# sotelo/parrot

Measured on AMD Instinct MI355X. Metric: acoustic feature frames/sec (train fwd+bwd+allreduce+clip/Adam), higher is better.
Workload: dtype f32; 1 GPU; BASELINE configs[1]: 2-layer attention-GRU decoder, h=1024, batch=64 per GPU, T_enc=200, T_dec=800, fp32; cell=gru, layers=2, hidden=1024, batch_per_gpu=64, global_batch=64, T_enc=200, T_dec=800, parallelism=dp1, params=13919212

## Files before the change

include/parrot_hip.h:

```cpp
#ifndef PARROT_HIP_H
#define PARROT_HIP_H

#include <stddef.h>
#include <stdint.h>

#ifdef __cplusplus
extern "C" {
#endif

#define PARROT_ERR_BADARG 10001
#define PARROT_ERR_UNSUPPORTED 10002

#define PARROT_NORM_EPS 1e-5f
#define PARROT_MAX_LAYERS 3

const char* parrot_hip_version(void);

int parrot_profile_begin(void);
long long parrot_profile_end(double* total_us, double* flops, double* bytes);
long long parrot_profile_end2(double* total_us, double* flops, double* bytes, double* plain4);

#define PARROT_PRECISION_F32 0
#define PARROT_PRECISION_BF16 1
#define PARROT_PRECISION_BF16X3 2
int parrot_set_gemm_precision(int mode);
int parrot_get_gemm_precision(void);
int parrot_gemm(const float* A, int lda, int transA, const float* B, int ldb, int transB, float* C, int ldc,
                int M, int N, int K, const float* bias, float alpha, int accumulate, int act, int nbatch,
                long long strideA, long long strideB, long long strideC, int split_k, void* stream);

int parrot_gemm_gated(const float* A, int lda, int transA, const float* B, int ldb, int transB, float* C, int ldc,
                      int M, int N, int K, const float* gate, int ldg, void* stream);

#define PARROT_GEMM_ROUTE_STEP 0
#define PARROT_GEMM_ROUTE_F32 1
#define PARROT_GEMM_ROUTE_BF16 2
#define PARROT_GEMM_ROUTE_BF16X3 3
int parrot_gemm_route(const float* A, int lda, int transA, const float* B, int ldb, int transB, int M, int N, int K,
                      float alpha, int act, int nbatch, long long strideA, long long strideB, int split_k, int has_gate,
                      int* kernel, int* slices);

int parrot_step_launch_mode(int njobs, const int* M, const int* N, const int* K, const int* lstm_H, int* info);

int parrot_to_bf16(const float* x, void* y, long long n, void* stream);
int parrot_gemm_bf16in(const void* A, int lda, const void* B, int ldb, float* C, int ldc, int M, int N, int K,
                       int accumulate, int split_k, void* stream);
int parrot_gemm_bf16in_ex(const void* A, int lda, int transA, const void* B, int ldb, int transB, float* C, int ldc, int M,
                          int N, int K, const float* bias, int accumulate, int split_k, void* stream);

int parrot_colsum(const float* x, long long M, int N, int ld, float* out, int accumulate, void* stream);
int parrot_colsum_route(const float* x, long long M, int N, int ld, const float* out, int* info2);

int parrot_gru_step_fwd(const float* h, const float* inputs, const float* gate_inputs, const float* mask,
                        const float* Wg, const float* Wc, float* h_out, float* z, float* r, float* rh,
                        float* c, int B, int H, void* stream);

int parrot_gru_step_bwd(const float* dh_out, const float* h, const float* mask, const float* Wg,
                        const float* Wc, const float* z, const float* r, const float* c, float* dh,
                        float* d_inputs, float* d_gate_inputs, int B, int H, void* stream);

typedef struct ParrotGruSeqDesc {
    int T, B, H, nchain, use_graph, reserved;
    int reverse[4];
    const float* Wg[4];
    const float* Wc[4];
    const float* inputs[4];
    const float* gate_inputs[4];
    const float* mask;
    float* h[4];
    float* z[4]; float* r[4]; float* rh[4]; float* c[4];
    float* dh[4];
    float* dG[4];
    float* dC[4];
} ParrotGruSeqDesc;

int parrot_gru_seq_create(const ParrotGruSeqDesc* desc, void** plan);
int parrot_gru_seq_fwd(void* plan, void* stream);
int parrot_gru_seq_bwd(void* plan, void* stream);
int parrot_gru_seq_destroy(void* plan);

#define PARROT_GRU_ROUTE_ROWWISE 0
#define PARROT_GRU_ROUTE_SHAPE 1
#define PARROT_GRU_ROUTE_SWITCH 2
#define PARROT_GRU_ROUTE_UNALIGNED 3
#define PARROT_GRU_ROUTE_ALLOC 4
int parrot_gru_seq_route(void* plan, int* info4);
int parrot_gru_seq_rowwise_supported(int T, int B, int H, int nchain);

typedef struct ParrotLstmSeqDesc {
    int T, B, H, use_graph;
    const float* W;
    const float* pre_in;
    float* s; float* c;
    float* gates;
    float* dS;
    float* dc;
    float* dP;
} ParrotLstmSeqDesc;

int parrot_lstm_seq_create(const ParrotLstmSeqDesc* desc, void** plan);
int parrot_lstm_seq_fwd(void* plan, void* stream);
int parrot_lstm_seq_bwd(void* plan, void* stream);
int parrot_lstm_seq_destroy(void* plan);

int parrot_gmm_attention_fwd(const float* h1, const float* WattT, const float* batt, const float* kappa_prev,
                             const float* ctx, float* a, float* b, float* kappa, float* phi, float* w, int B,
                             int H, int A, int U, int E, int att_type, float eps, float alignment,
                             float sharpening, float timing, void* stream);

int parrot_gmm_attention_bwd(const float* dw, const float* ctx, const float* a, const float* b,
                             const float* kappa, const float* kappa_prev, const float* WattT, float* dkappa,
                             float* dp, float* dh1, int B, int H, int A, int U, int E, int att_type, float eps,
                             void* stream);

typedef struct ParrotDecoderDesc {
    int T, B, H, E, A, U, L, att_type, use_graph;
    int reserved;
    float eps, alignment, sharpening, timing;
    const float* Wg[PARROT_MAX_LAYERS];
    const float* Wc[PARROT_MAX_LAYERS];
    const float* bg[PARROT_MAX_LAYERS];
    const float* bc[PARROT_MAX_LAYERS];
    const float* WattT;
    const float* batt;
    const float* ctx;
    float* seq_c[PARROT_MAX_LAYERS];
    float* seq_g[PARROT_MAX_LAYERS];
    float* h[PARROT_MAX_LAYERS];
    float* w;
    float* kappa;
    float* z[PARROT_MAX_LAYERS]; float* r[PARROT_MAX_LAYERS];
    float* rh[PARROT_MAX_LAYERS]; float* c[PARROT_MAX_LAYERS];
    float* a; float* b;
    float* phi;
    float* dh[PARROT_MAX_LAYERS];
    float* dw;
    float* dw0;
    float* dhup[PARROT_MAX_LAYERS];
    float* dkappa;
    float* dG[PARROT_MAX_LAYERS];
    float* dC[PARROT_MAX_LAYERS];
    float* dp;
    int cell;
    int seq_init;
    float* cst[PARROT_MAX_LAYERS];
    float* gate4[PARROT_MAX_LAYERS];
    float* dcell[PARROT_MAX_LAYERS];
    int layer_norm, bf16;
    const float* ln_bg[PARROT_MAX_LAYERS * PARROT_MAX_LAYERS];
    const float* ln_bc[PARROT_MAX_LAYERS * PARROT_MAX_LAYERS];
    float* ln_yg[PARROT_MAX_LAYERS * PARROT_MAX_LAYERS];
    float* ln_yc[PARROT_MAX_LAYERS * PARROT_MAX_LAYERS];
    float* ln_sg[PARROT_MAX_LAYERS * PARROT_MAX_LAYERS];
    float* ln_sc[PARROT_MAX_LAYERS * PARROT_MAX_LAYERS];
    const float* Wg_f[PARROT_MAX_LAYERS];
    const float* Wc_f[PARROT_MAX_LAYERS];
    const float* Wg_r[PARROT_MAX_LAYERS];
    const float* Wc_r[PARROT_MAX_LAYERS];
    int* att_sup;
    float* persist_ws;
    long long persist_ws_floats;
    float* dh_b[PARROT_MAX_LAYERS];
    float* dhup_b[PARROT_MAX_LAYERS];
    float* dw_b;
    float* dw0_b;
    float* dhup_c[PARROT_MAX_LAYERS];
    float* dw_c;
    float* dw0_c;
    void* dG16[PARROT_MAX_LAYERS];
} ParrotDecoderDesc;

long long parrot_decoder_persist_floats(const ParrotDecoderDesc* desc);
int parrot_decoder_is_persistent(void* plan);
int parrot_decoder_schedule(void* plan);
int parrot_decoder_backward_tick(void* plan);
long long parrot_decoder_trace(void* plan, int which, long long* out, long long cap);
long long parrot_decoder_trace_jobs(void* plan, int which, long long* out, long long cap);
int parrot_decoder_status(void* plan);

int parrot_decoder_create(const ParrotDecoderDesc* desc, void** plan);
int parrot_decoder_writes_bf16_grads(void* plan);
int parrot_decoder_seq_fwd(void* plan, void* stream);
int parrot_decoder_seq_bwd(void* plan, void* stream);
int parrot_decoder_destroy(void* plan);

#define PARROT_READOUT_MAX_SEG 4
typedef struct ParrotReadoutComposedDesc {
    long long M;
    long long ws_floats;
    int nseg, R, O, zero_rows;
    int slice_rows, nbias;
    int K[PARROT_READOUT_MAX_SEG];
    int ldx[PARROT_READOUT_MAX_SEG];
// ... 196 lines not shown
```

parrot_amd/_lib.py:

```python
from __future__ import annotations

import ctypes as C
import os

from .utils import env_str

_HERE = os.path.dirname(os.path.abspath(__file__))
LIB_PATH = os.path.join(_HERE, "libparrot_hip.so")

MAX_LAYERS = 3

c_float_p = C.c_void_p


class HipLibraryMissing(RuntimeError):
    pass


class HipCallError(RuntimeError):
    pass


class GruSeqDesc(C.Structure):
    _fields_ = [
        ("T", C.c_int), ("B", C.c_int), ("H", C.c_int), ("nchain", C.c_int),
        ("use_graph", C.c_int), ("reserved", C.c_int),
        ("reverse", C.c_int * 4),
        ("Wg", C.c_void_p * 4), ("Wc", C.c_void_p * 4),
        ("inputs", C.c_void_p * 4), ("gate_inputs", C.c_void_p * 4),
        ("mask", C.c_void_p),
        ("h", C.c_void_p * 4),
        ("z", C.c_void_p * 4), ("r", C.c_void_p * 4), ("rh", C.c_void_p * 4), ("c", C.c_void_p * 4),
        ("dh", C.c_void_p * 4), ("dG", C.c_void_p * 4), ("dC", C.c_void_p * 4),
    ]


class LabelTablesDesc(C.Structure):
    _fields_ = [
        ("N", C.c_longlong), ("Q", C.c_int), ("nseg", C.c_int),
        ("labels", C.c_void_p),
        ("tbl", C.c_void_p * 4), ("rows", C.c_void_p * 4), ("sums", C.c_void_p * 4),
        ("D", C.c_int * 4),
    ]


class LstmSeqDesc(C.Structure):
    _fields_ = [(n, C.c_int) for n in ("T", "B", "H", "use_graph")] + \
               [(n, C.c_void_p) for n in ("W", "pre_in", "s", "c", "gates", "dS", "dc", "dP")]


class DecoderDesc(C.Structure):
    _fields_ = [
        ("T", C.c_int), ("B", C.c_int), ("H", C.c_int), ("E", C.c_int), ("A", C.c_int),
        ("U", C.c_int), ("L", C.c_int), ("att_type", C.c_int), ("use_graph", C.c_int),
        ("reserved", C.c_int),
        ("eps", C.c_float), ("alignment", C.c_float), ("sharpening", C.c_float), ("timing", C.c_float),
        ("Wg", C.c_void_p * MAX_LAYERS), ("Wc", C.c_void_p * MAX_LAYERS),
        ("bg", C.c_void_p * MAX_LAYERS), ("bc", C.c_void_p * MAX_LAYERS),
        ("WattT", C.c_void_p), ("batt", C.c_void_p), ("ctx", C.c_void_p),
        ("seq_c", C.c_void_p * MAX_LAYERS), ("seq_g", C.c_void_p * MAX_LAYERS),
        ("h", C.c_void_p * MAX_LAYERS), ("w", C.c_void_p), ("kappa", C.c_void_p),
        ("z", C.c_void_p * MAX_LAYERS), ("r", C.c_void_p * MAX_LAYERS),
        ("rh", C.c_void_p * MAX_LAYERS), ("c", C.c_void_p * MAX_LAYERS),
        ("a", C.c_void_p), ("b", C.c_void_p), ("phi", C.c_void_p),
        ("dh", C.c_void_p * MAX_LAYERS), ("dw", C.c_void_p), ("dw0", C.c_void_p), ("dhup", C.c_void_p * MAX_LAYERS),
        ("dkappa", C.c_void_p),
        ("dG", C.c_void_p * MAX_LAYERS), ("dC", C.c_void_p * MAX_LAYERS), ("dp", C.c_void_p),
        ("cell", C.c_int), ("seq_init", C.c_int),
        ("cst", C.c_void_p * MAX_LAYERS), ("gate4", C.c_void_p * MAX_LAYERS), ("dcell", C.c_void_p * MAX_LAYERS),
        ("layer_norm", C.c_int), ("bf16", C.c_int),
        ("ln_bg", C.c_void_p * (MAX_LAYERS * MAX_LAYERS)), ("ln_bc", C.c_void_p * (MAX_LAYERS * MAX_LAYERS)),
        ("ln_yg", C.c_void_p * (MAX_LAYERS * MAX_LAYERS)), ("ln_yc", C.c_void_p * (MAX_LAYERS * MAX_LAYERS)),
        ("ln_sg", C.c_void_p * (MAX_LAYERS * MAX_LAYERS)), ("ln_sc", C.c_void_p * (MAX_LAYERS * MAX_LAYERS)),
        ("Wg_f", C.c_void_p * MAX_LAYERS), ("Wc_f", C.c_void_p * MAX_LAYERS),
        ("Wg_r", C.c_void_p * MAX_LAYERS), ("Wc_r", C.c_void_p * MAX_LAYERS),
        ("att_sup", C.c_void_p),
        ("persist_ws", C.c_void_p), ("persist_ws_floats", C.c_longlong),
        ("dh_b", C.c_void_p * MAX_LAYERS), ("dhup_b", C.c_void_p * MAX_LAYERS), ("dw_b", C.c_void_p), ("dw0_b", C.c_void_p),
        ("dhup_c", C.c_void_p * MAX_LAYERS), ("dw_c", C.c_void_p), ("dw0_c", C.c_void_p),
        ("dG16", C.c_void_p * MAX_LAYERS),
    ]


READOUT_MAX_SEG = 4


class ReadoutComposedDesc(C.Structure):
    _fields_ = [
        ("M", C.c_longlong), ("ws_floats", C.c_longlong),
        ("nseg", C.c_int), ("R", C.c_int), ("O", C.c_int), ("zero_rows", C.c_int),
        ("slice_rows", C.c_int), ("nbias", C.c_int),
        ("K", C.c_int * READOUT_MAX_SEG), ("ldx", C.c_int * READOUT_MAX_SEG), ("lddx", C.c_int * READOUT_MAX_SEG),
        ("ldwr", C.c_int), ("ldwo", C.c_int), ("ldp", C.c_int), ("lddp", C.c_int),
        ("ldgwr", C.c_int), ("ldgwo", C.c_int),
        ("x", C.c_void_p * READOUT_MAX_SEG),
        ("Wr", C.c_void_p), ("Wo", C.c_void_p),
        ("rb", C.c_void_p * READOUT_MAX_SEG), ("bo", C.c_void_p),
        ("pred", C.c_void_p), ("dp", C.c_void_p),
        ("dx", C.c_void_p * READOUT_MAX_SEG),
        ("gWr", C.c_void_p), ("gWo", C.c_void_p),
        ("grb", C.c_void_p * READOUT_MAX_SEG), ("gbo", C.c_void_p),
    ]


class SampleDesc(C.Structure):
    _fields_ = [
        ("S", C.c_int), ("B", C.c_int), ("H", C.c_int), ("E", C.c_int), ("A", C.c_int),
        ("U", C.c_int), ("L", C.c_int), ("O", C.c_int), ("R", C.c_int), ("ldx", C.c_int),
        ("att_type", C.c_int), ("use_graph", C.c_int),
        ("eps", C.c_float), ("alignment", C.c_float), ("sharpening", C.c_float), ("timing", C.c_float),
        ("Wg", C.c_void_p * MAX_LAYERS), ("Wc", C.c_void_p * MAX_LAYERS),
        ("bg", C.c_void_p * MAX_LAYERS), ("bc", C.c_void_p * MAX_LAYERS),
        ("Wfg", C.c_void_p * MAX_LAYERS), ("Wfc", C.c_void_p * MAX_LAYERS),
        ("seq_c", C.c_void_p * MAX_LAYERS), ("seq_g", C.c_void_p * MAX_LAYERS),
        ("WattT", C.c_void_p), ("batt", C.c_void_p),
        ("Wr", C.c_void_p), ("br", C.c_void_p), ("radd", C.c_void_p),
        ("Wo", C.c_void_p), ("bo", C.c_void_p), ("oadd", C.c_void_p),
        ("ctx", C.c_void_p),
        ("x", C.c_void_p), ("h", C.c_void_p * MAX_LAYERS), ("w", C.c_void_p), ("kappa", C.c_void_p),
        ("a", C.c_void_p), ("bwork", C.c_void_p), ("phi", C.c_void_p),
        ("zwork", C.c_void_p), ("rwork", C.c_void_p), ("rhwork", C.c_void_p), ("readout", C.c_void_p),
        ("gmm_K", C.c_int), ("reserved2", C.c_int), ("sampling_bias", C.c_float), ("reserved3", C.c_float),
        ("Wmu", C.c_void_p), ("bmu", C.c_void_p), ("Wsig", C.c_void_p), ("bsig", C.c_void_p),
        ("Wco", C.c_void_p), ("bco", C.c_void_p),
        ("add_mu", C.c_void_p), ("add_sig", C.c_void_p), ("add_co", C.c_void_p),
        ("unif", C.c_void_p), ("noise", C.c_void_p),
        ("gmm_mu", C.c_void_p), ("gmm_sig", C.c_void_p), ("gmm_co", C.c_void_p), ("pi_out", C.c_void_p),
        ("cell", C.c_int), ("reserved5", C.c_int),
        ("cwork", C.c_void_p * MAX_LAYERS), ("gwork", C.c_void_p),
        ("layer_norm", C.c_int), ("reserved7", C.c_int),
        ("bfg", C.c_void_p * MAX_LAYERS), ("bfc", C.c_void_p * MAX_LAYERS),
        ("ln_bg", C.c_void_p * (MAX_LAYERS * MAX_LAYERS)), ("ln_bc", C.c_void_p * (MAX_LAYERS * MAX_LAYERS)),
        ("br_l", C.c_void_p * MAX_LAYERS),
        ("ln_scratch", C.c_void_p), ("ln_scratch_floats", C.c_longlong),
        ("Wg_t", C.c_void_p * MAX_LAYERS), ("Wc_t", C.c_void_p * MAX_LAYERS),
        ("Wr_t", C.c_void_p), ("Wo_t", C.c_void_p), ("bo_pad", C.c_void_p), ("oadd_pad", C.c_void_p),
        ("persist_ws", C.c_void_p), ("persist_ws_floats", C.c_longlong),
        ("Wro_t", C.c_void_p), ("ro_const", C.c_void_p),
        ("Wgx_t", C.c_void_p * MAX_LAYERS), ("Wcx_t", C.c_void_p * MAX_LAYERS),
        ("Watt_t", C.c_void_p),
        ("bf16", C.c_int), ("reserved8", C.c_int),
        ("Wg_t16", C.c_void_p * MAX_LAYERS),
        ("eou_pos", C.c_void_p), ("eou_ncmp", C.c_void_p), ("eou_first", C.c_void_p),
        ("eou_extra", C.c_int), ("reserved9", C.c_int),
        ("Wrh_t", C.c_void_p), ("rh_const", C.c_void_p), ("rh_cols", C.c_int), ("reserved10", C.c_int),
    ]


class SampleRnnGenDesc(C.Structure):
    _fields_ = ([(n, C.c_int) for n in ("B", "D", "T", "Q", "FS", "BFS", "feat_dim", "use_graph")] +
                [("temperature", C.c_float), ("reserved", C.c_int), ("seed", C.c_ulonglong)] +
                [(n, C.c_void_p) for n in (
                    "big_Win_frames", "big_Win_feats", "big_bin", "big_U", "big_bU", "big_Wg", "big_Wc",
                    "big_Wout", "big_bout", "frm_Win", "frm_bin", "frm_U", "frm_bU", "frm_Wg", "frm_Wc",
                    "frm_Wout", "frm_bout", "emb_tbl", "W2", "b2", "W3", "b3", "W4", "b4", "features",
                    "samples", "big_h", "frm_h", "xf_big", "xf_frm", "feat_cur", "gru_in", "P", "z", "r", "rh",
                    "big_out", "frame_out", "o1", "o2", "o3", "logits", "tbase")] +
                [("n_rnn", C.c_int), ("lstm", C.c_int),
                 ("big_L", (C.c_void_p * 4) * 5), ("frm_L", (C.c_void_p * 4) * 5),
                 ("big_hs", C.c_void_p * 5), ("big_cs", C.c_void_p * 5),
                 ("frm_hs", C.c_void_p * 5), ("frm_cs", C.c_void_p * 5),
                 ("gate_ws", C.c_void_p), ("layer_tmp", C.c_void_p),
                 ("persist_ws", C.c_void_p), ("persist_ws_floats", C.c_longlong)])


_vp, _i, _f, _ll, _sz = C.c_void_p, C.c_int, C.c_float, C.c_longlong, C.c_size_t
SIGNATURES = {
    "parrot_hip_version": (C.c_char_p, []),
    "parrot_profile_begin": (_i, []),
    "parrot_profile_end": (C.c_longlong, [C.POINTER(C.c_double)] * 3),
    "parrot_profile_end2": (C.c_longlong, [C.POINTER(C.c_double)] * 4),
    "parrot_gemm": (_i, [_vp, _i, _i, _vp, _i, _i, _vp, _i, _i, _i, _i, _vp, _f, _i, _i, _i, _ll, _ll, _ll, _i, _vp]),
    "parrot_gemm_gated": (_i, [_vp, _i, _i, _vp, _i, _i, _vp, _i, _i, _i, _i, _vp, _i, _vp]),
    "parrot_gemm_route": (_i, [_vp, _i, _i, _vp, _i, _i, _i, _i, _i, _f, _i, _i, _ll, _ll, _i, _i,
                               C.POINTER(C.c_int), C.POINTER(C.c_int)]),
    "parrot_step_launch_mode": (_i, [_i] + [C.POINTER(C.c_int)] * 5),
    "parrot_gather_sum_fwd": (_i, [_vp, _vp, _vp, _i, _vp, _i, _ll, _i, _i, _i, _vp]),
    "parrot_gather_sum_bwd_ws_floats": (C.c_longlong, [_ll, _i, _i, _i]),
    "parrot_gather_sum_bwd": (_i, [_vp, _i, _vp, _vp, _vp, _vp, _ll, _ll, _i, _i, _i, _i, _vp]),
    "parrot_softmax_ce_fwd": (_i, [_vp, _i, _vp, _ll, _i, _vp, _vp, _vp]),
    "parrot_softmax_ce_bwd": (_i, [_vp, _i, _vp, _vp, _vp, _ll, _i, _vp, _i, _vp]),
    "parrot_relu_gate": (_i, [_vp, _vp, _vp, _ll, _vp]),
    "parrot_gmm_cost_fwd": (_i, [_vp, _i] * 4 + [_ll, _i, _i, _f, _vp, _vp, _i, _vp, _vp]),
    "parrot_gmm_cost_bwd": (_i, [_vp, _i] * 4 + [_vp, _vp, _ll, _i, _i, _f] + [_vp, _i] * 3 + [_vp]),
    "samplernn_weightnorm_ws_floats": (_ll, [_i]),
    "samplernn_weightnorm_fold": (_i, [_vp, _i, _vp, _vp, _i, _vp, _vp, _i, _i, _vp]),
    "samplernn_weightnorm_fold_bwd": (_i, [_vp, _i, _vp, _vp, _vp, _i, _vp, _i, _vp, _vp, _i, _i, _i, _i, _vp]),
    "parrot_colsum": (_i, [_vp, _ll, _i, _i, _vp, _i, _vp]),
    "parrot_colsum_route": (_i, [_vp, _ll, _i, _i, _vp, C.POINTER(C.c_int)]),
    "parrot_gru_step_fwd": (_i, [_vp] * 11 + [_i, _i, _vp]),
    "parrot_gru_step_bwd": (_i, [_vp] * 11 + [_i, _i, _vp]),
    "parrot_label_tables_supported": (_i, [_ll, _i]),
    "parrot_label_gather": (_i, [C.POINTER(LabelTablesDesc), _vp]),
    "parrot_label_segsum_ws_floats": (C.c_longlong, [_ll, _i, _i]),
    "parrot_label_segsum": (_i, [C.POINTER(LabelTablesDesc), _vp, _ll, _vp]),
    "parrot_gru_seq_create": (_i, [C.POINTER(GruSeqDesc), C.POINTER(C.c_void_p)]),
    "parrot_gru_seq_fwd": (_i, [_vp, _vp]),
    "parrot_gru_seq_bwd": (_i, [_vp, _vp]),
    "parrot_gru_seq_destroy": (_i, [_vp]),
    "parrot_gru_seq_route": (_i, [_vp, C.POINTER(C.c_int)]),
    "parrot_gru_seq_rowwise_supported": (_i, [_i, _i, _i, _i]),
    "parrot_lstm_seq_create": (_i, [C.POINTER(LstmSeqDesc), C.POINTER(C.c_void_p)]),
    "parrot_lstm_seq_fwd": (_i, [_vp, _vp]),
    "parrot_lstm_seq_bwd": (_i, [_vp, _vp]),
    "parrot_lstm_seq_destroy": (_i, [_vp]),
    "parrot_gmm_attention_fwd": (_i, [_vp] * 10 + [_i] * 6 + [_f] * 4 + [_vp]),
    "parrot_gmm_attention_bwd": (_i, [_vp] * 10 + [_i] * 6 + [_f, _vp]),
    "parrot_decoder_create": (_i, [C.POINTER(DecoderDesc), C.POINTER(C.c_void_p)]),
    "parrot_decoder_persist_floats": (C.c_longlong, [C.POINTER(DecoderDesc)]),
    "parrot_decoder_is_persistent": (_i, [_vp]),
    "parrot_decoder_schedule": (_i, [_vp]),
    "parrot_decoder_backward_tick": (_i, [_vp]),
    "parrot_decoder_writes_bf16_grads": (_i, [_vp]),
    "parrot_decoder_trace": (C.c_longlong, [_vp, _i, C.POINTER(C.c_longlong), C.c_longlong]),
    "parrot_decoder_trace_jobs": (C.c_longlong, [_vp, _i, C.POINTER(C.c_longlong), C.c_longlong]),
    "parrot_decoder_seq_fwd": (_i, [_vp, _vp]),
    "parrot_decoder_seq_bwd": (_i, [_vp, _vp]),
    "parrot_decoder_destroy": (_i, [_vp]),
    "parrot_readout_composed_ws_floats": (C.c_longlong, [C.POINTER(ReadoutComposedDesc)]),
    "parrot_readout_composed_fwd": (_i, [C.POINTER(ReadoutComposedDesc), _vp, _vp]),
    "parrot_readout_composed_bwd": (_i, [C.POINTER(ReadoutComposedDesc), _vp, _vp]),
    "parrot_sample_create": (_i, [C.POINTER(SampleDesc), C.POINTER(C.c_void_p)]),
    "parrot_sample_persist_floats": (C.c_longlong, [C.POINTER(SampleDesc)]),
    "parrot_sample_is_persistent": (_i, [_vp]),
    "parrot_sample_is_bf16": (_i, [_vp]),
    "parrot_sample_plan_pieces_dry": (_i, [C.POINTER(SampleDesc), _i, C.POINTER(C.c_int)]),
    "parrot_sample_plan_digest_dry": (_i, [C.POINTER(SampleDesc), _i, C.POINTER(C.c_ulonglong)]),
    "parrot_sample_status": (_i, [_vp]),
    "parrot_sample_stops_early": (_i, [_vp]),
    "parrot_sample_steps_run": (_i, [_vp, C.POINTER(C.c_int)]),
    "parrot_decoder_status": (_i, [_vp]),
    "parrot_sample_run": (_i, [_vp, _vp]),
    "parrot_sample_destroy": (_i, [_vp]),
    "parrot_plan_last_error": (_i, [_vp]),
    "parrot_sumsq": (_i, [_vp, _sz, _vp, _vp]),
    "parrot_tile_weights": (_i, [_vp, _i, _i, _i, _vp, _i, _i, _vp]),
    "parrot_tile_weights_bf16": (_i, [_vp, _i, _i, _i, _vp, _i, _i, _vp]),
    "parrot_set_gemm_precision": (_i, [_i]),
    "parrot_get_gemm_precision": (_i, []),
    "parrot_to_bf16": (_i, [_vp, _vp, _ll, _vp]),
    "parrot_gemm_bf16in": (_i, [_vp, _i, _vp, _i, _vp, _i, _i, _i, _i, _i, _i, _vp]),
    "parrot_gemm_bf16in_ex": (_i, [_vp, _i, _i, _vp, _i, _i, _vp, _i, _i, _i, _i, _vp, _i, _i, _vp]),
    "parrot_simple_norm_fwd": (_i, [_vp, _i, _vp, _i, _vp, _ll, _i, _f, _vp, _i, _vp]),
    "parrot_simple_norm_bwd": (_i, [_vp, _i, _vp, _i, _vp, _vp, _i, _ll, _i, _f, _i, _vp]),
    "parrot_adam_clip_step": (_i, [_vp, _vp, _vp, _vp, _sz, _vp, _f, _f, _f, _f, _f, _f, _i, _vp]),
    "parrot_batch_quantize": (_i, [_vp, _i, _i, _i, _vp, _vp, _i, _i, _i, _vp]),
    "parrot_mu2linear": (_i, [_vp, _sz, _vp, _vp]),
    "samplernn_generate_create": (_i, [C.POINTER(SampleRnnGenDesc), C.POINTER(C.c_void_p)]),
    "samplernn_generate_run": (_i, [_vp, _vp]),
    "samplernn_persist_floats": (C.c_longlong, [C.POINTER(SampleRnnGenDesc)]),
    "samplernn_generate_is_persistent": (_i, [_vp]),
    "samplernn_generate_status": (_i, [_vp]),
    "samplernn_generate_destroy": (_i, [_vp]),
}

_lib = None


def load():
    global _lib
    if _lib is not None:
        return _lib
    import torch
    path = env_str('PARROT_HIP_LIB', LIB_PATH)
    if not os.path.exists(path):
        raise HipLibraryMissing(
            f"{LIB_PATH} not found: build it with `python -m parrot_amd.build` "
            "(hipcc --offload-arch=gfx950).  There is no CPU fallback for the product path.")
    lib = C.CDLL(path)
    for name, (res, args) in SIGNATURES.items():
        fn = getattr(lib, name)
        fn.restype = res
        fn.argtypes = args
    _lib = lib
    return lib


def check(rc: int, what: str, plan=None):
    if rc != 0:
        raise HipCallError(f"{what} failed with code {rc}")


def call(name: str, *args):
    lib = load()
    rc = getattr(lib, name)(*args)
    check(rc, name)
    return rc
```

parrot_amd/csrc/biggemm.h:

```cpp
#pragma once
#include "common.h"

struct BgArgs {
    const float* A;
    const float* B;
    float* C;
    const float* bias;
    int M, N, K;
    long long sam, sak, sbk, sbn;
    int ldc;
    long long batchA, batchB, batchC;
    int nbatch;
    int splitk;
    float* ws;
    int accumulate;
    float alpha;
    int act;
    const float* gate;
    int ldg;
    int bf16;
};

int bg_launch(const BgArgs& a, hipStream_t stream);
void bg_tile_shape(int bf16, int& bm, int& bn);
int bg_to_bf16_launch(const float* x, void* y, long long n, hipStream_t stream);
int bg_reduce_launch(const BgArgs& a, hipStream_t stream);

struct BgPrecisionScope {
    explicit BgPrecisionScope(int bf16);
    ~BgPrecisionScope();
    int saved;
};
```

parrot_amd/csrc/biggemm.hip:

```cpp
#include "biggemm.h"

#include <atomic>

#include <hip/hip_runtime.h>
#include <stdlib.h>
#include <string.h>

namespace {

constexpr int BM = 128, BN = 128, BK = 16, PITCH = 132;

__device__ __forceinline__ void bg_tile_of_block(int bid, int tiles_m, int tiles_n, int& tm, int& tn) {
    const int nwg = tiles_m * tiles_n;
    const int q = nwg / 8, r = nwg % 8;
    const int xcd = bid % 8, idx = bid / 8;
    const int lin = (xcd < r ? xcd * (q + 1) : r * (q + 1) + (xcd - r) * q) + idx;
    constexpr int GW = 8;
    const int group = lin / (GW * tiles_m);
    const int first = group * GW;
    const int gsz = min(tiles_n - first, GW);
    const int rem = lin - group * GW * tiles_m;
    tm = rem / gsz;
    tn = first + rem % gsz;
}

template <bool XC>
__device__ __forceinline__ void bg_load8(const float* __restrict__ p, int x0, int X, int k0, int kend,
                                         long long sx, long long sk, bool vec, int t, f32x4& v) {
    v = (f32x4){0.f, 0.f, 0.f, 0.f};
    if (XC) {
        const int xq = t & 31, kr = t >> 5;
        const int k = k0 + kr, x = x0 + 4 * xq;
        if (k < kend) {
            const float* q = p + (long long)k * sk + x;
            if (vec && x + 3 < X) v = *reinterpret_cast<const f32x4*>(q);
            else {
#pragma unroll
                for (int u = 0; u < 4; ++u)
                    if (x + u < X) v[u] = q[u];
            }
        }
    } else {
        const int x = x0 + (t >> 2), k = k0 + 4 * (t & 3);
        if (x < X) {
            const float* q = p + (long long)x * sx + k;
            if (vec && k + 3 < kend) v = *reinterpret_cast<const f32x4*>(q);
            else {
#pragma unroll
                for (int u = 0; u < 4; ++u)
                    if (k + u < kend) v[u] = q[u];
            }
        }
    }
}

template <bool XC>
__device__ __forceinline__ void bg_store8(float* __restrict__ s, int t, const f32x4& v) {
    if (XC) {
        *reinterpret_cast<f32x4*>(s + (t >> 5) * PITCH + 4 * (t & 31)) = v;
    } else {
        const int x = t >> 2, kq = t & 3;
#pragma unroll
        for (int u = 0; u < 4; ++u) s[(4 * kq + u) * PITCH + x] = v[u];
    }
}

template <bool AXC, bool BXC>
__global__ __launch_bounds__(512) void bg_kernel8(const BgArgs a, int vecA, int vecB, int tiles_m, int tiles_n) {
    __shared__ __attribute__((aligned(16))) float As[2][BK * PITCH];
    __shared__ __attribute__((aligned(16))) float Bs[2][BK * PITCH];
    int tm, tn;
    bg_tile_of_block(blockIdx.x, tiles_m, tiles_n, tm, tn);
    const int m0 = tm * BM, n0 = tn * BN;
    const int z = blockIdx.y;
    const int batch = z / a.splitk, ks = z % a.splitk;
    int kchunk = (a.K + a.splitk - 1) / a.splitk;
    kchunk = (kchunk + BK - 1) / BK * BK;
    const int kbeg = ks * kchunk;
    const int kend = min(a.K, kbeg + kchunk);
    const float* A = a.A + (long long)batch * a.batchA;
    const float* B = a.B + (long long)batch * a.batchB;
    float* C = a.C + (long long)batch * a.batchC;
    const int t = threadIdx.x, lane = t & 63, wave = t >> 6;
    const int wm = wave >> 2, wn = wave & 3;
    const int kk = lane >> 5, li = lane & 31;
    f32x16 acc[2];
#pragma unroll
    for (int i = 0; i < 2; ++i)
#pragma unroll
        for (int q = 0; q < 16; ++q) acc[i][q] = 0.f;
    f32x4 ra, rb;
    const int nk = (kend - kbeg + BK - 1) / BK;
    if (nk > 0) {
        bg_load8<AXC>(A, m0, a.M, kbeg, kend, a.sam, a.sak, vecA, t, ra);
        bg_load8<BXC>(B, n0, a.N, kbeg, kend, a.sbn, a.sbk, vecB, t, rb);
        bg_store8<AXC>(As[0], t, ra);
        bg_store8<BXC>(Bs[0], t, rb);
    }
    __syncthreads();
    for (int kt = 0; kt < nk; ++kt) {
        const int cur = kt & 1;
        if (kt + 1 < nk) {
            bg_load8<AXC>(A, m0, a.M, kbeg + (kt + 1) * BK, kend, a.sam, a.sak, vecA, t, ra);
            bg_load8<BXC>(B, n0, a.N, kbeg + (kt + 1) * BK, kend, a.sbn, a.sbk, vecB, t, rb);
        }
        const float* as = As[cur] + wm * 64 + li;
        const float* bs = Bs[cur] + wn * 32 + li;
#pragma unroll
        for (int kp = 0; kp < BK / 2; ++kp) {
            const int row = (2 * kp + kk) * PITCH;
            const float a0 = as[row], a1 = as[row + 32];
            const float b0 = bs[row];
            acc[0] = __builtin_amdgcn_mfma_f32_32x32x2f32(a0, b0, acc[0], 0, 0, 0);
            acc[1] = __builtin_amdgcn_mfma_f32_32x32x2f32(a1, b0, acc[1], 0, 0, 0);
        }
        if (kt + 1 < nk) {
            bg_store8<AXC>(As[cur ^ 1], t, ra);
            bg_store8<BXC>(Bs[cur ^ 1], t, rb);
        }
        __syncthreads();
    }
#pragma unroll
    for (int i = 0; i < 2; ++i) {
        const int n = n0 + wn * 32 + li;
        if (n >= a.N) continue;
        const float bias = (a.bias && ks == 0) ? a.bias[n] : 0.f;
#pragma unroll
        for (int q = 0; q < 16; ++q) {
            const int m = m0 + wm * 64 + i * 32 + (q & 3) + 8 * (q >> 2) + 4 * kk;
            if (m >= a.M) continue;
            float v = a.alpha * acc[i][q] + bias;
            float* c = C + (long long)m * a.ldc + n;
            if (a.splitk > 1) {
                a.ws[((long long)z * a.M + m) * a.N + n] = a.alpha * acc[i][q];
            } else {
                if (a.accumulate) v += *c;
                if (a.act == 1) v = fmaxf(v, 0.f);
                else if (a.act == 2) v = tanhf(v);
                else if (a.act == 3) v = 1.f / (1.f + expf(-v));
                if (a.gate && !(a.gate[(long long)m * a.ldg + n] > 0.f)) v = 0.f;
                *c = v;
            }
        }
    }
}


constexpr int BK16 = 32, PITCH16 = 40, PITCHT = 144;

template <bool XC>
__device__ __forceinline__ void bg_load16(const float* __restrict__ p, int x0, int X, int k0, int kend,
                                          long long sx, long long sk, bool vec, int t, f32x4 (&v)[2]) {
    v[0] = (f32x4){0.f, 0.f, 0.f, 0.f};
    v[1] = (f32x4){0.f, 0.f, 0.f, 0.f};
    if (XC) {
        const int x = x0 + 4 * (t & 31);
#pragma unroll
        for (int ps = 0; ps < 2; ++ps) {
            const int k = k0 + (t >> 5) + 16 * ps;
            if (k < kend) {
                const float* q = p + (long long)k * sk + x;
                if (vec && x + 3 < X) {
                    v[ps] = *reinterpret_cast<const f32x4*>(q);
                } else {
#pragma unroll
                    for (int u = 0; u < 4; ++u)
                        if (x + u < X) v[ps][u] = q[u];
                }
            }
        }
    } else {
        const int x = x0 + (t >> 2), k = k0 + 8 * (t & 3);
        if (x < X) {
            const float* q = p + (long long)x * sx + k;
            if (vec && k + 7 < kend) {
                v[0] = *reinterpret_cast<const f32x4*>(q);
                v[1] = *reinterpret_cast<const f32x4*>(q + 4);
            } else {
#pragma unroll
                for (int u = 0; u < 8; ++u)
                    if (k + u < kend) v[u >> 2][u & 3] = q[u];
            }
        }
    }
}

template <bool XC>
__device__ __forceinline__ void bg_store16(__bf16* __restrict__ s, int t, const f32x4 (&v)[2]) {
    if (XC) {
        typedef __bf16 bf16x4 __attribute__((ext_vector_type(4)));
#pragma unroll
        for (int ps = 0; ps < 2; ++ps)
            *reinterpret_cast<bf16x4*>(s + ((t >> 5) + 16 * ps) * PITCHT + 4 * (t & 31)) = __builtin_convertvector(v[ps], bf16x4);
    } else {
        *reinterpret_cast<bf16x8*>(s + (t >> 2) * PITCH16 + 8 * (t & 3)) = ph_bf16x8(v[0], v[1]);
    }
}

template <bool XC>
__device__ __forceinline__ bf16x8 bg_frag16(const __bf16* __restrict__ img, int xb, int s, int lane) {
    const int kk = lane >> 5, li = lane & 31;
    if (XC) {
        typedef short s16x4 __attribute__((ext_vector_type(4)));
        typedef __attribute__((address_space(3))) s16x4* lds4;
        const int k0 = 16 * s + 8 * kk, q = (li >> 2) & 3, xg = xb + (li & 16) + 4 * (li & 3);
        const __bf16* p = img + (k0 + q) * PITCHT + xg;
        const s16x4 lo = __builtin_amdgcn_ds_read_tr16_b64_v4i16((lds4)(p));
        const s16x4 hi = __builtin_amdgcn_ds_read_tr16_b64_v4i16((lds4)(p + 4 * PITCHT));
        typedef short s16x8 __attribute__((ext_vector_type(8)));
        const s16x8 v = {lo[0], lo[1], lo[2], lo[3], hi[0], hi[1], hi[2], hi[3]};
        return __builtin_bit_cast(bf16x8, v);
    } else {
        return *reinterpret_cast<const bf16x8*>(img + (xb + li) * PITCH16 + 16 * s + 8 * kk);
    }
}

template <bool AXC, bool BXC>
__global__ __launch_bounds__(512) void bg_kernel_bf16(const BgArgs a, int vecA, int vecB, int tiles_m, int tiles_n) {
    constexpr int ASZ = AXC ? BK16 * PITCHT : BM * PITCH16, BSZ = BXC ? BK16 * PITCHT : BN * PITCH16;
    __shared__ __attribute__((aligned(16))) __bf16 As[2][ASZ];
    __shared__ __attribute__((aligned(16))) __bf16 Bs[2][BSZ];
    int tm, tn;
    bg_tile_of_block(blockIdx.x, tiles_m, tiles_n, tm, tn);
    const int m0 = tm * BM, n0 = tn * BN;
    const int z = blockIdx.y;
    const int batch = z / a.splitk, ks = z % a.splitk;
    int kchunk = (a.K + a.splitk - 1) / a.splitk;
    kchunk = (kchunk + BK16 - 1) / BK16 * BK16;
    const int kbeg = ks * kchunk;
    const int kend = min(a.K, kbeg + kchunk);
    const float* A = a.A + (long long)batch * a.batchA;
    const float* B = a.B + (long long)batch * a.batchB;
    float* C = a.C + (long long)batch * a.batchC;
    const int t = threadIdx.x, lane = t & 63, wave = t >> 6;
    const int wm = wave >> 2, wn = wave & 3;
    const int kk = lane >> 5, li = lane & 31;
    f32x16 acc[2];
#pragma unroll
    for (int i = 0; i < 2; ++i)
#pragma unroll
        for (int q = 0; q < 16; ++q) acc[i][q] = 0.f;
    f32x4 ra[2], rb[2];
    const int nk = (kend - kbeg + BK16 - 1) / BK16;
    if (nk > 0) {
        bg_load16<AXC>(A, m0, a.M, kbeg, kend, a.sam, a.sak, vecA, t, ra);
        bg_load16<BXC>(B, n0, a.N, kbeg, kend, a.sbn, a.sbk, vecB, t, rb);
        bg_store16<AXC>(As[0], t, ra);
        bg_store16<BXC>(Bs[0], t, rb);
    }
    __syncthreads();
    for (int kt = 0; kt < nk; ++kt) {
        const int cur = kt & 1;
        if (kt + 1 < nk) {
            bg_load16<AXC>(A, m0, a.M, kbeg + (kt + 1) * BK16, kend, a.sam, a.sak, vecA, t, ra);
            bg_load16<BXC>(B, n0, a.N, kbeg + (kt + 1) * BK16, kend, a.sbn, a.sbk, vecB, t, rb);
        }
#pragma unroll
        for (int s = 0; s < BK16 / 16; ++s) {
            const bf16x8 a0 = bg_frag16<AXC>(As[cur], wm * 64, s, lane);
            const bf16x8 a1 = bg_frag16<AXC>(As[cur], wm * 64 + 32, s, lane);
            const bf16x8 b0 = bg_frag16<BXC>(Bs[cur], wn * 32, s, lane);
            acc[0] = __builtin_amdgcn_mfma_f32_32x32x16_bf16(a0, b0, acc[0], 0, 0, 0);
            acc[1] = __builtin_amdgcn_mfma_f32_32x32x16_bf16(a1, b0, acc[1], 0, 0, 0);
        }
        if (kt + 1 < nk) {
            bg_store16<AXC>(As[cur ^ 1], t, ra);
            bg_store16<BXC>(Bs[cur ^ 1], t, rb);
        }
        __syncthreads();
    }
#pragma unroll
    for (int i = 0; i < 2; ++i) {
        const int n = n0 + wn * 32 + li;
        if (n >= a.N) continue;
        const float bias = (a.bias && ks == 0) ? a.bias[n] : 0.f;
#pragma unroll
        for (int q = 0; q < 16; ++q) {
            const int m = m0 + wm * 64 + i * 32 + (q & 3) + 8 * (q >> 2) + 4 * kk;
            if (m >= a.M) continue;
            float v = a.alpha * acc[i][q] + bias;
            float* c = C + (long long)m * a.ldc + n;
            if (a.splitk > 1) {
                a.ws[((long long)z * a.M + m) * a.N + n] = a.alpha * acc[i][q];
            } else {
                if (a.accumulate) v += *c;
                if (a.act == 1) v = fmaxf(v, 0.f);
                else if (a.act == 2) v = tanhf(v);
                else if (a.act == 3) v = 1.f / (1.f + expf(-v));
                if (a.gate && !(a.gate[(long long)m * a.ldg + n] > 0.f)) v = 0.f;
                *c = v;
            }
        }
    }
}

constexpr int HBMT = 256, HBNT = 256, HPITCH = 272;
template <int BKT, bool XC>
struct BghOperand {
    static constexpr int PK = BKT + 8;
    static constexpr int SZ = XC ? BKT * HPITCH : 256 * PK;
    static constexpr int NV = BKT / 16;
    static __device__ __forceinline__ void load(const __bf16* __restrict__ p, long long ld, int x0, int X, int k0, int kend,
                                                int t, bf16x8 (&v)[NV]) {
#pragma unroll
        for (int i = 0; i < NV; ++i) {
            bf16x8 r;
#pragma unroll
            for (int u = 0; u < 8; ++u) r[u] = (__bf16)0.f;
            if (XC) {
                const int k = k0 + (t >> 5) + 16 * i, x = x0 + 8 * (t & 31);
                if (k < kend && x < X) r = *reinterpret_cast<const bf16x8*>(p + (long long)k * ld + x);
            } else {
                const int id = t + 512 * i;
                const int x = x0 + id / (BKT / 8), k = k0 + 8 * (id % (BKT / 8));
                if (x < X && k < kend) r = *reinterpret_cast<const bf16x8*>(p + (long long)x * ld + k);
            }
            v[i] = r;
        }
    }
    static __device__ __forceinline__ void store(__bf16* __restrict__ s, int t, const bf16x8 (&v)[NV]) {
#pragma unroll
        for (int i = 0; i < NV; ++i) {
            if (XC) {
                *reinterpret_cast<bf16x8*>(s + ((t >> 5) + 16 * i) * HPITCH + 8 * (t & 31)) = v[i];
            } else {
                const int id = t + 512 * i;
                *reinterpret_cast<bf16x8*>(s + (id / (BKT / 8)) * PK + 8 * (id % (BKT / 8))) = v[i];
            }
        }
    }
    static __device__ __forceinline__ bf16x8 frag(const __bf16* __restrict__ img, int xb, int s_, int kk, int li) {
        if (XC) {
            typedef short s16x4 __attribute__((ext_vector_type(4)));
            typedef short s16x8 __attribute__((ext_vector_type(8)));
            typedef __attribute__((address_space(3))) s16x4* lds4;
            const int k0 = 16 * s_ + 8 * kk, q = (li >> 2) & 3, xg = xb + (li & 16) + 4 * (li & 3);
            const __bf16* p = img + (k0 + q) * HPITCH + xg;
            const s16x4 lo = __builtin_amdgcn_ds_read_tr16_b64_v4i16((lds4)(p));
            const s16x4 hi = __builtin_amdgcn_ds_read_tr16_b64_v4i16((lds4)(p + 4 * HPITCH));
            const s16x8 v = {lo[0], lo[1], lo[2], lo[3], hi[0], hi[1], hi[2], hi[3]};
            return __builtin_bit_cast(bf16x8, v);
        } else {
            return *reinterpret_cast<const bf16x8*>(img + (xb + li) * PK + 16 * s_ + 8 * kk);
        }
    }
};

template <int BKT, bool AXC, bool BXC>
__global__ __launch_bounds__(512) void bgh_kernel(const BgArgs a, int tiles_m, int tiles_n) {
    typedef BghOperand<BKT, AXC> OA;
    typedef BghOperand<BKT, BXC> OB;
    constexpr int NV = BKT / 16;
    extern __shared__ __attribute__((aligned(16))) __bf16 bgh_smem[];
    __bf16* As = bgh_smem;
    __bf16* Bs = bgh_smem + 2 * OA::SZ;
    int tm, tn;
    bg_tile_of_block(blockIdx.x, tiles_m, tiles_n, tm, tn);
    const int m0 = tm * HBMT, n0 = tn * HBNT;
    const int z = blockIdx.y;
    const int batch = z / a.splitk, ks = z % a.splitk;
    int kchunk = (a.K + a.splitk - 1) / a.splitk;
    kchunk = (kchunk + BKT - 1) / BKT * BKT;
    const int kbeg = ks * kchunk;
    const int kend = min(a.K, kbeg + kchunk);
    const __bf16* A = reinterpret_cast<const __bf16*>(a.A) + (long long)batch * a.batchA;
    const __bf16* B = reinterpret_cast<const __bf16*>(a.B) + (long long)batch * a.batchB;
    float* C = a.C + (long long)batch * a.batchC;
    const long long lda = AXC ? a.sak : a.sam, ldb = BXC ? a.sbk : a.sbn;
    const int t = threadIdx.x, lane = t & 63, wave = t >> 6;
    const int wm = wave >> 2, wn = wave & 3;
    const int kk = lane >> 5, li = lane & 31;
    f32x16 acc[4][2];
#pragma unroll
    for (int i = 0; i < 4; ++i)
#pragma unroll
        for (int j = 0; j < 2; ++j)
#pragma unroll
            for (int q = 0; q < 16; ++q) acc[i][j][q] = 0.f;
    bf16x8 ra[NV], rb[NV];
    const int nk = (kend - kbeg + BKT - 1) / BKT;
    if (nk > 0) {
        OA::load(A, lda, m0, a.M, kbeg, kend, t, ra);
        OB::load(B, ldb, n0, a.N, kbeg, kend, t, rb);
        OA::store(As, t, ra);
        OB::store(Bs, t, rb);
    }
    __syncthreads();
    for (int kt = 0; kt < nk; ++kt) {
        const int cur = kt & 1;
        if (kt + 1 < nk) {
            OA::load(A, lda, m0, a.M, kbeg + (kt + 1) * BKT, kend, t, ra);
            OB::load(B, ldb, n0, a.N, kbeg + (kt + 1) * BKT, kend, t, rb);
        }
        const __bf16* as = As + cur * OA::SZ;
        const __bf16* bs = Bs + cur * OB::SZ;
#pragma unroll
        for (int s_ = 0; s_ < BKT / 16; ++s_) {
            bf16x8 fa[4], fb[2];
#pragma unroll
            for (int j = 0; j < 2; ++j) fb[j] = OB::frag(bs, wn * 64 + 32 * j, s_, kk, li);
#pragma unroll
            for (int i = 0; i < 4; ++i) fa[i] = OA::frag(as, wm * 128 + 32 * i, s_, kk, li);
#pragma unroll
            for (int i = 0; i < 4; ++i)
#pragma unroll
                for (int j = 0; j < 2; ++j)
                    acc[i][j] = __builtin_amdgcn_mfma_f32_32x32x16_bf16(fa[i], fb[j], acc[i][j], 0, 0, 0);
        }
        if (kt + 1 < nk) {
            OA::store(As + (cur ^ 1) * OA::SZ, t, ra);
            OB::store(Bs + (cur ^ 1) * OB::SZ, t, rb);
        }
        __syncthreads();
    }
#pragma unroll
    for (int i = 0; i < 4; ++i)
#pragma unroll
        for (int j = 0; j < 2; ++j) {
            const int n = n0 + wn * 64 + j * 32 + li;
            if (n >= a.N) continue;
            const float bias = (a.bias && ks == 0) ? a.bias[n] : 0.f;
#pragma unroll
            for (int q = 0; q < 16; ++q) {
                const int m = m0 + wm * 128 + i * 32 + (q & 3) + 8 * (q >> 2) + 4 * kk;
                if (m >= a.M) continue;
                const float v = a.alpha * acc[i][j][q];
                if (a.splitk > 1) {
                    a.ws[((long long)z * a.M + m) * a.N + n] = v;
                } else {
                    float* c = C + (long long)m * a.ldc + n;
                    *c = a.accumulate ? *c + v + bias : v + bias;
                }
            }
        }
}

constexpr int SBK = 16;
typedef __bf16 bf16x4 __attribute__((ext_vector_type(4)));

__device__ __forceinline__ void bgs_split(const f32x4& v, bf16x4& p0, bf16x4& p1, bf16x4& p2) {
    p0 = __builtin_convertvector(v, bf16x4);
    const f32x4 r1 = v - __builtin_convertvector(p0, f32x4);
    p1 = __builtin_convertvector(r1, bf16x4);
    const f32x4 r2 = r1 - __builtin_convertvector(p1, f32x4);
    p2 = __builtin_convertvector(r2, bf16x4);
}

template <bool XC>
struct BgsOperand {
    static constexpr int PK = SBK + 8;
    static constexpr int PLANE = XC ? SBK * HPITCH : 256 * PK;
    static constexpr int SZ = 3 * PLANE;
    static __device__ __forceinline__ void load(const float* __restrict__ p, long long ld, int x0, int X, int k0, int kend,
                                                bool vec, int t, f32x4 (&v)[2]) {
#pragma unroll
        for (int i = 0; i < 2; ++i) {
            const int id = t + 512 * i;
            v[i] = (f32x4){0.f, 0.f, 0.f, 0.f};
            if (XC) {
                const int k = k0 + (id >> 6), x = x0 + 4 * (id & 63);
                if (k < kend && x < X) {
                    const float* q = p + (long long)k * ld + x;
                    if (vec && x + 3 < X) v[i] = *reinterpret_cast<const f32x4*>(q);
                    else {
#pragma unroll
                        for (int u = 0; u < 4; ++u)
                            if (x + u < X) v[i][u] = q[u];
                    }
                }
            } else {
                const int x = x0 + (id >> 2), k = k0 + 4 * (id & 3);
                if (x < X && k < kend) {
                    const float* q = p + (long long)x * ld + k;
                    if (vec && k + 3 < kend) v[i] = *reinterpret_cast<const f32x4*>(q);
                    else {
#pragma unroll
                        for (int u = 0; u < 4; ++u)
                            if (k + u < kend) v[i][u] = q[u];
                    }
                }
            }
        }
    }
    static __device__ __forceinline__ void store(__bf16* __restrict__ s, int t, const f32x4 (&v)[2]) {
#pragma unroll
        for (int i = 0; i < 2; ++i) {
            const int id = t + 512 * i;
            bf16x4 p0, p1, p2;
            bgs_split(v[i], p0, p1, p2);
            __bf16* d = XC ? s + (id >> 6) * HPITCH + 4 * (id & 63) : s + (id >> 2) * PK + 4 * (id & 3);
            *reinterpret_cast<bf16x4*>(d) = p0;
            *reinterpret_cast<bf16x4*>(d + PLANE) = p1;
            *reinterpret_cast<bf16x4*>(d + 2 * PLANE) = p2;
        }
    }
    static __device__ __forceinline__ bf16x8 frag(const __bf16* __restrict__ img, int xb, int kk, int li) {
        if (XC) {
            typedef short s16x4 __attribute__((ext_vector_type(4)));
            typedef short s16x8 __attribute__((ext_vector_type(8)));
            typedef __attribute__((address_space(3))) s16x4* lds4;
            const int q = (li >> 2) & 3, xg = xb + (li & 16) + 4 * (li & 3);
            const __bf16* p = img + (8 * kk + q) * HPITCH + xg;
            const s16x4 lo = __builtin_amdgcn_ds_read_tr16_b64_v4i16((lds4)(p));
            const s16x4 hi = __builtin_amdgcn_ds_read_tr16_b64_v4i16((lds4)(p + 4 * HPITCH));
            const s16x8 v = {lo[0], lo[1], lo[2], lo[3], hi[0], hi[1], hi[2], hi[3]};
            return __builtin_bit_cast(bf16x8, v);
        } else {
            return *reinterpret_cast<const bf16x8*>(img + (xb + li) * PK + 8 * kk);
        }
    }
};

template <bool AXC, bool BXC>
__global__ __launch_bounds__(512) void bgs_kernel(const BgArgs a, int vecA, int vecB, int tiles_m, int tiles_n, int zmap) {
    typedef BgsOperand<AXC> OA;
    typedef BgsOperand<BXC> OB;
    extern __shared__ __attribute__((aligned(16))) __bf16 bgs_smem[];
    __bf16* As = bgs_smem;
    __bf16* Bs = bgs_smem + 2 * OA::SZ;
    int tm, tn, z;
    if (zmap) {
        const int tiles = tiles_m * tiles_n, idx = blockIdx.x >> 3;
        z = 8 * (idx / tiles) + (blockIdx.x & 7);
        const int tl = idx % tiles;
        tm = tl / tiles_n;
        tn = tl % tiles_n;
    } else {
        bg_tile_of_block(blockIdx.x, tiles_m, tiles_n, tm, tn);
        z = blockIdx.y;
    }
    const int m0 = tm * HBMT, n0 = tn * HBNT;
    const int batch = z / a.splitk, ks = z % a.splitk;
    int kchunk = (a.K + a.splitk - 1) / a.splitk;
    kchunk = (kchunk + SBK - 1) / SBK * SBK;
    const int kbeg = ks * kchunk;
    const int kend = min(a.K, kbeg + kchunk);
    const float* A = a.A + (long long)batch * a.batchA;
    const float* B = a.B + (long long)batch * a.batchB;
    float* C = a.C + (long long)batch * a.batchC;
    const long long lda = AXC ? a.sak : a.sam, ldb = BXC ? a.sbk : a.sbn;
    const int t = threadIdx.x, lane = t & 63, wave = t >> 6;
    const int wm = wave >> 2, wn = wave & 3;
    const int kk = lane >> 5, li = lane & 31;
    f32x16 acc[4][2];
#pragma unroll
    for (int i = 0; i < 4; ++i)
#pragma unroll
        for (int j = 0; j < 2; ++j)
#pragma unroll
            for (int q = 0; q < 16; ++q) acc[i][j][q] = 0.f;
    f32x4 ra[2], rb[2];
    const int nk = (kend - kbeg + SBK - 1) / SBK;
    if (nk > 0) {
        OA::load(A, lda, m0, a.M, kbeg, kend, vecA, t, ra);
        OB::load(B, ldb, n0, a.N, kbeg, kend, vecB, t, rb);
        OA::store(As, t, ra);
        OB::store(Bs, t, rb);
        if (nk > 1) {
            OA::load(A, lda, m0, a.M, kbeg + SBK, kend, vecA, t, ra);
            OB::load(B, ldb, n0, a.N, kbeg + SBK, kend, vecB, t, rb);
        }
    }
    __syncthreads();
    const bool early = wave >= 4;
    for (int kt = 0; kt < nk; ++kt) {
        const int cur = kt & 1;
        const __bf16* as = As + cur * OA::SZ;
        const __bf16* bs = Bs + cur * OB::SZ;
        if (early && kt + 1 < nk) {
            OA::store(As + (cur ^ 1) * OA::SZ, t, ra);
            OB::store(Bs + (cur ^ 1) * OB::SZ, t, rb);
            if (kt + 2 < nk) {
                OA::load(A, lda, m0, a.M, kbeg + (kt + 2) * SBK, kend, vecA, t, ra);
                OB::load(B, ldb, n0, a.N, kbeg + (kt + 2) * SBK, kend, vecB, t, rb);
            }
        }
        bf16x8 fb[2][3];
#pragma unroll
        for (int j = 0; j < 2; ++j)
#pragma unroll
            for (int p = 0; p < 3; ++p) fb[j][p] = OB::frag(bs + p * OB::PLANE, wn * 64 + 32 * j, kk, li);
#pragma unroll
        for (int i = 0; i < 4; ++i) {
            bf16x8 fa[3];
#pragma unroll
            for (int p = 0; p < 3; ++p) fa[p] = OA::frag(as + p * OA::PLANE, wm * 128 + 32 * i, kk, li);
#define BGS_MM(pa, pb)                                                                                    \
    acc[i][0] = __builtin_amdgcn_mfma_f32_32x32x16_bf16(fa[pa], fb[0][pb], acc[i][0], 0, 0, 0);          \
    acc[i][1] = __builtin_amdgcn_mfma_f32_32x32x16_bf16(fa[pa], fb[1][pb], acc[i][1], 0, 0, 0)
            BGS_MM(2, 0);
            BGS_MM(0, 2);
            BGS_MM(1, 1);
            BGS_MM(1, 0);
            BGS_MM(0, 1);
            BGS_MM(0, 0);
#undef BGS_MM
        }
        if (!early && kt + 1 < nk) {
            OA::store(As + (cur ^ 1) * OA::SZ, t, ra);
            OB::store(Bs + (cur ^ 1) * OB::SZ, t, rb);
            if (kt + 2 < nk) {
                OA::load(A, lda, m0, a.M, kbeg + (kt + 2) * SBK, kend, vecA, t, ra);
                OB::load(B, ldb, n0, a.N, kbeg + (kt + 2) * SBK, kend, vecB, t, rb);
            }
        }
        __syncthreads();
    }
#pragma unroll
    for (int i = 0; i < 4; ++i)
#pragma unroll
        for (int j = 0; j < 2; ++j) {
            const int n = n0 + wn * 64 + j * 32 + li;
            if (n >= a.N) continue;
            const float bias = (a.bias && ks == 0) ? a.bias[n] : 0.f;
#pragma unroll
            for (int q = 0; q < 16; ++q) {
                const int m = m0 + wm * 128 + i * 32 + (q & 3) + 8 * (q >> 2) + 4 * kk;
                if (m >= a.M) continue;
                const float v = a.alpha * acc[i][j][q];
                if (a.splitk > 1) {
                    a.ws[((long long)z * a.M + m) * a.N + n] = v;
                } else {
                    float* c = C + (long long)m * a.ldc + n;
                    float r = a.accumulate ? *c + v + bias : v + bias;
                    if (a.act == 1) r = fmaxf(r, 0.f);
                    if (a.gate && !(a.gate[(long long)m * a.ldg + n] > 0.f)) r = 0.f;
                    *c = r;
                }
            }
        }
}

__global__ __launch_bounds__(256) void bg_to_bf16_kernel(const float* __restrict__ x, __bf16* __restrict__ y, long long n8) {
    for (long long i = (long long)blockIdx.x * 256 + threadIdx.x; i < n8; i += (long long)gridDim.x * 256) {
        const f32x4 lo = *reinterpret_cast<const f32x4*>(x + 8 * i);
        const f32x4 hi = *reinterpret_cast<const f32x4*>(x + 8 * i + 4);
        *reinterpret_cast<bf16x8*>(y + 8 * i) = ph_bf16x8(lo, hi);
    }
}

__global__ __launch_bounds__(256) void bg_reduce_kernel(const BgArgs a) {
    const long long mn = (long long)a.M * a.N;
    const long long total = mn * a.nbatch;
    for (long long i = (long long)blockIdx.x * 256 + threadIdx.x; i < total; i += (long long)gridDim.x * 256) {
        const int batch = (int)(i / mn);
        const long long r = i % mn;
        const int m = (int)(r / a.N), n = (int)(r % a.N);
        float* c = a.C + (long long)batch * a.batchC + (long long)m * a.ldc + n;
        float v = a.accumulate ? *c : 0.f;
        if (a.bias) v += a.bias[n];
        const float* w = a.ws + ((long long)batch * a.splitk) * mn + r;
        int ks = 0;
        for (; ks + 8 <= a.splitk; ks += 8) {
            float p[8];
#pragma unroll
            for (int q = 0; q < 8; ++q) p[q] = w[(long long)(ks + q) * mn];
#pragma unroll
            for (int q = 0; q < 8; ++q) v += p[q];
        }
        for (; ks < a.splitk; ++ks) v += w[(long long)ks * mn];
        if (a.gate && !(a.gate[(long long)m * a.ldg + n] > 0.f)) v = 0.f;
        *c = v;
    }
}

}

int bg_reduce_launch(const BgArgs& a, hipStream_t stream) {
    const long long total = (long long)a.M * a.N * a.nbatch;
    int blocks = (int)((total + 255) / 256);
    if (blocks > 4096) blocks = 4096;
    hipLaunchKernelGGL(bg_reduce_kernel, dim3(blocks), dim3(256), 0, stream, a);
    return (int)hipGetLastError();
}

void bg_tile_shape(int bf16, int& bm, int& bn) {
    bm = bn = 128;
    if (bf16 == 2 || bf16 == 3) { bm = HBMT; bn = HBNT; return; }
}

template <typename K>
static void bg_big_lds_once(K kern, bool& done) {
    if (!done) {
        (void)hipFuncSetAttribute((const void*)kern, hipFuncAttributeMaxDynamicSharedMemorySize, 160 * 1024);
        done = true;
    }
}

template <int BKT, bool AX, bool BX>
static void bgh_go(const BgArgs& a, dim3 grid, int tm, int tn, hipStream_t stream) {
    static bool done = false;
    bg_big_lds_once(bgh_kernel<BKT, AX, BX>, done);
    const size_t lds = (size_t)4 * (BghOperand<BKT, AX>::SZ + BghOperand<BKT, BX>::SZ);
    hipLaunchKernelGGL((bgh_kernel<BKT, AX, BX>), grid, dim3(512), lds, stream, a, tm, tn);
}

template <bool AX, bool BX>
static void bgs_go(const BgArgs& a, dim3 grid, int vecA, int vecB, int tm, int tn, int zmap, hipStream_t stream) {
    static bool done = false;
    bg_big_lds_once(bgs_kernel<AX, BX>, done);
    const size_t lds = (size_t)4 * (BgsOperand<AX>::SZ + BgsOperand<BX>::SZ);
    hipLaunchKernelGGL((bgs_kernel<AX, BX>), grid, dim3(512), lds, stream, a, vecA, vecB, tm, tn, zmap);
}

int bg_to_bf16_launch(const float* x, void* y, long long n, hipStream_t stream) {
    if (n <= 0) return 0;
    if ((n & 7) || ((uintptr_t)x & 15) || ((uintptr_t)y & 15)) return PH_ERR_BADARG;
    const long long n8 = n / 8;
    int blocks = (int)((n8 + 255) / 256);
    if (blocks > 8192) blocks = 8192;
    hipLaunchKernelGGL(bg_to_bf16_kernel, dim3(blocks), dim3(256), 0, stream, x, reinterpret_cast<__bf16*>(y), n8);
    return (int)hipGetLastError();
}

int bg_launch(const BgArgs& a, hipStream_t stream) {
    const size_t pad = 0;
    if (a.M <= 0 || a.N <= 0 || a.K < 0 || a.nbatch < 1 || a.splitk < 1 || (a.splitk > 1 && !a.ws)) return PH_ERR_BADARG;
    const bool axc = (a.sam == 1), bxc = (a.sbn == 1);
    if (!axc && a.sak != 1) return PH_ERR_BADARG;
    if (!bxc && a.sbk != 1) return PH_ERR_BADARG;
    auto al = [](const float* p, long long stride, long long batch) {
        return (((uintptr_t)p & 15) == 0) && (stride % 4 == 0) && (batch % 4 == 0);
    };
    const int vecA = axc ? al(a.A, a.sak, a.batchA) : al(a.A, a.sam, a.batchA);
    const int vecB = bxc ? al(a.B, a.sbk, a.batchB) : al(a.B, a.sbn, a.batchB);
    const int tiles_m = ceil_div(a.M, BM), tiles_n = ceil_div(a.N, BN);
    dim3 grid(tiles_m * tiles_n, a.nbatch * a.splitk);
    if (a.bf16 == 2) {
        if (a.act || a.gate || ((uintptr_t)a.A & 15) || ((uintptr_t)a.B & 15) || (a.batchA & 7) || (a.batchB & 7))
            return PH_ERR_UNSUPPORTED;
        if (axc ? ((a.M & 7) || (a.sak & 7)) : ((a.K & 7) || (a.sam & 7))) return PH_ERR_UNSUPPORTED;
        if (bxc ? ((a.N & 7) || (a.sbk & 7)) : ((a.K & 7) || (a.sbn & 7))) return PH_ERR_UNSUPPORTED;
        const int tm = ceil_div(a.M, HBMT), tn = ceil_div(a.N, HBNT);
        const int bkt = (axc && bxc) ? 32 : 64;
        const dim3 g2(tm * tn, a.nbatch * a.splitk);
        if (bkt == 64) {
            if (axc && bxc) bgh_go<64, true, true>(a, g2, tm, tn, stream);
            else if (axc) bgh_go<64, true, false>(a, g2, tm, tn, stream);
            else if (bxc) bgh_go<64, false, true>(a, g2, tm, tn, stream);
            else bgh_go<64, false, false>(a, g2, tm, tn, stream);
        } else {
            bgh_go<32, true, true>(a, g2, tm, tn, stream);
        }
        return (int)hipGetLastError();
    }
    if (a.bf16 == 3) {
        if (a.act > 1) return PH_ERR_UNSUPPORTED;
        const int tm = ceil_div(a.M, HBMT), tn = ceil_div(a.N, HBNT);
        const int Z = a.nbatch * a.splitk;
        const int zmap = (Z % 8 == 0) ? 1 : 0;
        const dim3 g = zmap ? dim3(tm * tn * Z) : dim3(tm * tn, Z);
        if (axc && bxc) bgs_go<true, true>(a, g, vecA, vecB, tm, tn, zmap, stream);
        else if (axc) bgs_go<true, false>(a, g, vecA, vecB, tm, tn, zmap, stream);
        else if (bxc) bgs_go<false, true>(a, g, vecA, vecB, tm, tn, zmap, stream);
        else bgs_go<false, false>(a, g, vecA, vecB, tm, tn, zmap, stream);
        return (int)hipGetLastError();
    }
    if (a.bf16) {
        dim3 b8(512);
        if (axc && bxc) hipLaunchKernelGGL((bg_kernel_bf16<true, true>), grid, b8, pad, stream, a, vecA, vecB, tiles_m, tiles_n);
        else if (axc && !bxc) hipLaunchKernelGGL((bg_kernel_bf16<true, false>), grid, b8, pad, stream, a, vecA, vecB, tiles_m, tiles_n);
        else if (!axc && bxc) hipLaunchKernelGGL((bg_kernel_bf16<false, true>), grid, b8, pad, stream, a, vecA, vecB, tiles_m, tiles_n);
        else hipLaunchKernelGGL((bg_kernel_bf16<false, false>), grid, b8, pad, stream, a, vecA, vecB, tiles_m, tiles_n);
        return (int)hipGetLastError();
    }
    const dim3 b8(512);
    if (axc && bxc) hipLaunchKernelGGL((bg_kernel8<true, true>), grid, b8, pad, stream, a, vecA, vecB, tiles_m, tiles_n);
    else if (axc && !bxc) hipLaunchKernelGGL((bg_kernel8<true, false>), grid, b8, pad, stream, a, vecA, vecB, tiles_m, tiles_n);
    else if (!axc && bxc) hipLaunchKernelGGL((bg_kernel8<false, true>), grid, b8, pad, stream, a, vecA, vecB, tiles_m, tiles_n);
    else hipLaunchKernelGGL((bg_kernel8<false, false>), grid, b8, pad, stream, a, vecA, vecB, tiles_m, tiles_n);
    return (int)hipGetLastError();
}
```

parrot_amd/csrc/capi.hip:

```cpp
#include "../../include/parrot_hip.h"
#include "attention.h"
#include "biggemm.h"
#include "elementwise.h"
#include "quantize.h"
#include "skinny.h"
#include "switches.h"

#include <math.h>
#include <stdlib.h>
#include <string.h>

#include <atomic>

static int gemm_target_wgs() {
    return 1024;
}

static int gemm_default_mode() {
    const char* e = env_str("PARROT_GEMM_PRECISION");
    if (e && (!strcmp(e, "f32") || !strcmp(e, "0"))) return PARROT_PRECISION_F32;
    if (e && (!strcmp(e, "bf16") || !strcmp(e, "1"))) return PARROT_PRECISION_BF16;
    return PARROT_PRECISION_BF16X3;
}
static std::atomic<int> g_gemm_bf16{gemm_default_mode()};
static thread_local int t_gemm_bf16 = -1;
BgPrecisionScope::BgPrecisionScope(int bf16) : saved(t_gemm_bf16) { t_gemm_bf16 = bf16 < 0 ? saved : (bf16 ? 1 : 0); }
BgPrecisionScope::~BgPrecisionScope() { t_gemm_bf16 = saved; }

extern "C" {

int parrot_set_gemm_precision(int mode) { PH_ENTRY();
    if (mode != PARROT_PRECISION_F32 && mode != PARROT_PRECISION_BF16 && mode != PARROT_PRECISION_BF16X3) return PARROT_ERR_BADARG;
    g_gemm_bf16.store(mode, std::memory_order_relaxed);
    return 0;
}

int parrot_get_gemm_precision(void) { PH_ENTRY(); return g_gemm_bf16.load(std::memory_order_relaxed); }

const char* parrot_hip_version(void) { PH_ENTRY(); return "parrot_hip 0.5.0 gfx950"; }

int parrot_profile_begin(void) { PH_ENTRY();
    sk_profile_begin();
    return 0;
}

long long parrot_profile_end(double* total_us, double* flops, double* bytes) { PH_ENTRY();
    return sk_profile_end(total_us, flops, bytes);
}

long long parrot_profile_end2(double* total_us, double* flops, double* bytes, double* plain4) { PH_ENTRY();
    return sk_profile_end2(total_us, flops, bytes, plain4);
}

static StreamScratch bg_workspace(0);

static int bg_auto_split(int bf16, int M, int N, int K, int act, int nbatch) {
    int bm, bn;
    bg_tile_shape(bf16, bm, bn);
    const long long tiles = (long long)ceil_div(M, bm) * ceil_div(N, bn) * nbatch;
    int split = 1;
    if (bf16 == 3) {
        if (act == 0 && tiles < 256 && K >= 4096) {
            double best = -1.0;
            for (int sp = 8; sp <= 64 && K / sp >= 512; sp += 8) {
                const long long wgs = tiles * sp;
                const double eff = (double)wgs / (double)((wgs + 255) / 256 * 256);
                const double score = eff - 0.001 * sp;
                if (score > best) { best = score; split = sp; }
            }
        }
    } else if (bf16 == 2 && K >= 512 && tiles < 256) {
        double best = -1.0;
        for (int sp = 1; sp <= 16 && K / sp >= 1024; ++sp) {
            const long long wgs = tiles * sp;
            const double eff = (double)wgs / (double)((wgs + 255) / 256 * 256);
            const double score = eff - (wgs < 512 ? 0.25 : 0.0) - 0.002 * sp;
            if (score > best) { best = score; split = sp; }
        }
    } else if (act == 0 && tiles < 512 && K >= 512) {
        split = (int)((gemm_target_wgs() + tiles - 1) / tiles);
        const int maxs = K / 256 > 0 ? K / 256 : 1;
        if (split > maxs) split = maxs;
        if (split > 64) split = 64;
    }
    return split;
}

static int bg_run(BgArgs a, int split_k, hipStream_t st) {
    const int M = a.M, N = a.N, nbatch = a.nbatch, act = a.act;
    const float* bias = a.bias;
    const int split = split_k > 0 ? split_k : bg_auto_split(a.bf16, M, N, a.K, act, nbatch);
    a.splitk = split;
    a.ws = nullptr;
    if (a.splitk > 1) {
        if (act != 0) return PARROT_ERR_BADARG;
        float* ws = bg_workspace.get(st, (size_t)nbatch * a.splitk * M * N);
        if (ws) {
            a.ws = ws;
            a.bias = nullptr;
            int rc = bg_launch(a, st);
            if (rc) return rc;
            a.bias = bias;
            return bg_reduce_launch(a, st);
        }
        a.splitk = 1;
    }
    return bg_launch(a, st);
}

static int gemm_pick_kernel(const float* A, int lda, int transA, const float* B, int ldb, int transB, int M, int N, int K,
                            float alpha, int act, int nbatch, long long strideA, long long strideB, int split_k,
                            bool has_gate, int mode) {
    if (M <= 64 && !transA && nbatch == 1 && split_k <= 1 && alpha == 1.0f && !has_gate) return PARROT_GEMM_ROUTE_STEP;
    if (mode == PARROT_PRECISION_BF16) return PARROT_GEMM_ROUTE_BF16;
    if (mode == PARROT_PRECISION_BF16X3) {
        auto al = [](const float* p, long long ld) { return (((uintptr_t)p & 15) == 0) && (ld % 4 == 0); };
        const bool ok = act <= 1 && al(A, lda) && al(B, ldb) && (strideA % 4 == 0) && (strideB % 4 == 0) && M >= 128 && N >= 128 &&
                        K >= 64 && (!transA || M % 4 == 0) && (transA || K % 4 == 0) && (transB || N % 4 == 0) && (!transB || K % 4 == 0);
        if (ok) return PARROT_GEMM_ROUTE_BF16X3;
    }
    return PARROT_GEMM_ROUTE_F32;
}

static int gemm_mode_in_force() { return t_gemm_bf16 >= 0 ? t_gemm_bf16 : g_gemm_bf16.load(std::memory_order_relaxed); }

static int gemm_route_bf16(int route) {
    return route == PARROT_GEMM_ROUTE_BF16X3 ? 3 : route == PARROT_GEMM_ROUTE_BF16 ? 1 : 0;
}

static int gemm_impl(const float* A, int lda, int transA, const float* B, int ldb, int transB, float* C, int ldc,
                     int M, int N, int K, const float* bias, float alpha, int accumulate, int act, int nbatch,
                     long long strideA, long long strideB, long long strideC, int split_k, const float* gate, int ldg,
                     void* stream) {
    if (!A || !B || !C || M < 1 || N < 1 || K < 1 || nbatch < 1) return PARROT_ERR_BADARG;
    if (gate && (nbatch != 1 || ldg < N)) return PARROT_ERR_BADARG;
    if (act != 0 && accumulate) return PARROT_ERR_BADARG;
    hipStream_t st = (hipStream_t)stream;
    const int route = gemm_pick_kernel(A, lda, transA, B, ldb, transB, M, N, K, alpha, act, nbatch, strideA, strideB, split_k,
                                       gate != nullptr, gemm_mode_in_force());
    if (route == PARROT_GEMM_ROUTE_STEP) {
        SkJob j;
        sk_job_init(j);
        j.nseg = 1;
        j.seg[0] = sk_seg(A, lda, B, ldb, K, transB ? 1 : 0);
        j.M = M; j.N = N; j.H = N; j.epi = SK_EPI_LINEAR; j.act = act; j.accumulate = accumulate;
        j.bias = bias;
        j.out = C; j.ldo = ldc;
        SkLaunch L;
        int rc = sk_make_launch(L, &j, 1);
        if (rc) return rc;
        return sk_launch(L, st);
    }
    BgArgs a;
    a.A = A; a.B = B; a.C = C; a.bias = bias;
    a.M = M; a.N = N; a.K = K;
    a.sam = transA ? 1 : lda; a.sak = transA ? lda : 1;
    a.sbk = transB ? 1 : ldb; a.sbn = transB ? ldb : 1;
    a.ldc = ldc;
    a.batchA = strideA; a.batchB = strideB; a.batchC = strideC;
    a.nbatch = nbatch;
    a.accumulate = accumulate; a.alpha = alpha; a.act = act;
    a.gate = gate; a.ldg = ldg;
    a.bf16 = gemm_route_bf16(route);
    return bg_run(a, split_k, st);
}

int parrot_gemm(const float* A, int lda, int transA, const float* B, int ldb, int transB, float* C, int ldc,
                int M, int N, int K, const float* bias, float alpha, int accumulate, int act, int nbatch,
                long long strideA, long long strideB, long long strideC, int split_k, void* stream) { PH_ENTRY();
    return gemm_impl(A, lda, transA, B, ldb, transB, C, ldc, M, N, K, bias, alpha, accumulate, act, nbatch, strideA, strideB,
                     strideC, split_k, nullptr, 0, stream);
}

int parrot_gemm_gated(const float* A, int lda, int transA, const float* B, int ldb, int transB, float* C, int ldc,
                      int M, int N, int K, const float* gate, int ldg, void* stream) { PH_ENTRY();
    if (!gate) return PARROT_ERR_BADARG;
    return gemm_impl(A, lda, transA, B, ldb, transB, C, ldc, M, N, K, nullptr, 1.0f, 0, 0, 1, 0, 0, 0, 0, gate, ldg, stream);
}

int parrot_gemm_route(const float* A, int lda, int transA, const float* B, int ldb, int transB, int M, int N, int K,
                      float alpha, int act, int nbatch, long long strideA, long long strideB, int split_k, int has_gate,
                      int* kernel, int* slices) {
    if (!A || !B || !kernel || !slices || M < 1 || N < 1 || K < 1 || nbatch < 1) return PARROT_ERR_BADARG;
    if (has_gate && nbatch != 1) return PARROT_ERR_BADARG;
    const int route = gemm_pick_kernel(A, lda, transA, B, ldb, transB, M, N, K, alpha, act, nbatch, strideA, strideB, split_k,
                                       has_gate != 0, gemm_mode_in_force());
    int split = 1;
    if (route != PARROT_GEMM_ROUTE_STEP) {
        split = split_k > 0 ? split_k : bg_auto_split(gemm_route_bf16(route), M, N, K, act, nbatch);
        if (split > 1 && act != 0) return PARROT_ERR_BADARG;
    }
    *kernel = route;
    *slices = split;
    return 0;
}

int parrot_step_launch_mode(int njobs, const int* M, const int* N, const int* K, const int* lstm_H, int* info) {
    if (!M || !N || !K || !info || njobs < 1 || njobs > SK_MAXJOB) return PARROT_ERR_BADARG;
    SkJob jobs[SK_MAXJOB];
    for (int q = 0; q < njobs; ++q) {
        if (M[q] < 1 || N[q] < 1 || K[q] < 1) return PARROT_ERR_BADARG;
        SkJob& j = jobs[q];
        sk_job_init(j);
        const float* aligned_base = reinterpret_cast<const float*>(uintptr_t(4096));
        j.nseg = 1;
        j.seg[0] = sk_seg(aligned_base, (K[q] + 3) & ~3, aligned_base, (N[q] + 3) & ~3, K[q], 0);
        j.M = M[q]; j.N = N[q];
        j.H = lstm_H && lstm_H[q] > 0 ? lstm_H[q] : N[q];
        j.epi = lstm_H && lstm_H[q] > 0 ? SK_EPI_LSTM : SK_EPI_LINEAR;
    }
    SkLaunch Lin, L;
    const int rc = sk_make_launch(Lin, jobs, njobs);
    if (rc) return rc;
    dim3 grid;
    size_t lds;
    int mbnb;
    sk_prepare(Lin, L, grid, lds, mbnb);
    info[0] = L.zmode; info[1] = mbnb; info[2] = (int)grid.x; info[3] = (int)grid.y; info[4] = (int)grid.z;
    for (int q = 0; q < njobs; ++q) info[5 + q] = L.tile_end[q];
    return 0;
}

int parrot_to_bf16(const float* x, void* y, long long n, void* stream) { PH_ENTRY();
    if (!x || !y || n < 0) return PARROT_ERR_BADARG;
    return bg_to_bf16_launch(x, y, n, (hipStream_t)stream);
}

int parrot_gemm_bf16in_ex(const void* A, int lda, int transA, const void* B, int ldb, int transB, float* C, int ldc, int M,
                          int N, int K, const float* bias, int accumulate, int split_k, void* stream) { PH_ENTRY();
    if (!A || !B || !C || M < 1 || N < 1 || K < 1) return PARROT_ERR_BADARG;
    BgArgs a;
    a.A = reinterpret_cast<const float*>(A); a.B = reinterpret_cast<const float*>(B); a.C = C; a.bias = bias;
    a.M = M; a.N = N; a.K = K;
    a.sam = transA ? 1 : lda; a.sak = transA ? lda : 1;
    a.sbk = transB ? 1 : ldb; a.sbn = transB ? ldb : 1;
    a.ldc = ldc;
    a.batchA = a.batchB = a.batchC = 0;
    a.nbatch = 1;
    a.accumulate = accumulate; a.alpha = 1.0f; a.act = 0;
    a.gate = nullptr; a.ldg = 0;
    a.bf16 = 2;
    return bg_run(a, split_k, (hipStream_t)stream);
}

int parrot_gemm_bf16in(const void* A, int lda, const void* B, int ldb, float* C, int ldc, int M, int N, int K,
                       int accumulate, int split_k, void* stream) {
    return parrot_gemm_bf16in_ex(A, lda, 1, B, ldb, 0, C, ldc, M, N, K, nullptr, accumulate, split_k, stream);
}

int parrot_tile_weights(const float* W, int rows, int cols, int ld, float* out, int mode, int lstm_H, void* stream) { PH_ENTRY();
    if (mode != 0 && mode != 1) return PARROT_ERR_BADARG;
    return sk_tile_weights_launch(W, rows, cols, ld, out, mode, lstm_H, (hipStream_t)stream);
}

int parrot_tile_weights_bf16(const float* W, int rows, int cols, int ld, void* out, int mode, int lstm_H, void* stream) { PH_ENTRY();
    if (mode != 0 && mode != 1 && mode != 2) return PARROT_ERR_BADARG;
    return sk_tile_weights_bf16_launch(W, rows, cols, ld, out, mode, lstm_H, (hipStream_t)stream);
}

int parrot_simple_norm_fwd(const float* x, int ldx, float* y, int ldy, float* sigma, long long R, int N, float eps,
                           float* add_dst, int ld_add, void* stream) { PH_ENTRY();
    if (!x || !y || !sigma) return PARROT_ERR_BADARG;
    return simple_norm_fwd_launch(x, ldx, y, ldy, sigma, R, N, eps, add_dst, ld_add, (hipStream_t)stream);
}

int parrot_simple_norm_bwd(const float* dy, int lddy, const float* y, int ldy, const float* sigma, float* dx,
                           int lddx, long long R, int N, float eps, int accumulate, void* stream) { PH_ENTRY();
    if (!dy || !y || !sigma || !dx) return PARROT_ERR_BADARG;
    return simple_norm_bwd_launch(dy, lddy, y, ldy, sigma, dx, lddx, R, N, eps, accumulate, (hipStream_t)stream);
}

int parrot_colsum(const float* x, long long M, int N, int ld, float* out, int accumulate, void* stream) { PH_ENTRY();
    return colsum_launch(x, M, N, ld, out, accumulate, (hipStream_t)stream);
}

int parrot_colsum_route(const float* x, long long M, int N, int ld, const float* out, int* info2) {
    if (!x || !info2 || M < 0 || N < 1) return PARROT_ERR_BADARG;
    const ColsumRoute r = colsum_route(x, M, N, ld, out);
    info2[0] = r.vec4;
    info2[1] = r.ysplit;
    return 0;
}

int parrot_gru_step_fwd(const float* h, const float* inputs, const float* gate_inputs, const float* mask,
                        const float* Wg, const float* Wc, float* h_out, float* z, float* r, float* rh,
                        float* c, int B, int H, void* stream) { PH_ENTRY();
    if (!h || !Wg || !Wc || !h_out || !z || !r || !rh || B < 1 || H < 1) return PARROT_ERR_BADARG;
    hipStream_t st = (hipStream_t)stream;
    SkJob j;
    SkLaunch L;
    sk_job_init(j);
    j.nseg = 1;
    j.seg[0] = sk_seg(h, H, Wg, 2 * H, H, 0);
    j.M = B; j.N = 2 * H; j.H = H; j.epi = SK_EPI_GRU_GATES;
    j.add = gate_inputs; j.ld_add = 2 * H;
    j.e0 = h; j.lde0 = H;
    j.o1 = z; j.ldo1 = H; j.o2 = r; j.ldo2 = H; j.out = rh; j.ldo = H;
    int rc = sk_make_launch(L, &j, 1);
    if (rc) return rc;
    rc = sk_launch(L, st);
    if (rc) return rc;
    sk_job_init(j);
    j.nseg = 1;
    j.seg[0] = sk_seg(rh, H, Wc, H, H, 0);
    j.M = B; j.N = H; j.H = H; j.epi = SK_EPI_GRU_CAND;
    j.add = inputs; j.ld_add = H;
    j.e0 = h; j.lde0 = H; j.e1 = z; j.lde1 = H;
    j.o1 = c; j.ldo1 = H; j.out = h_out; j.ldo = H; j.mask = mask;
    rc = sk_make_launch(L, &j, 1);
    if (rc) return rc;
    return sk_launch(L, st);
}

int parrot_gru_step_bwd(const float* dh_out, const float* h, const float* mask, const float* Wg,
                        const float* Wc, const float* z, const float* r, const float* c, float* dh,
                        float* d_inputs, float* d_gate_inputs, int B, int H, void* stream) { PH_ENTRY();
    if (!dh_out || !h || !Wg || !Wc || !z || !r || !c || !dh || !d_inputs || !d_gate_inputs)
        return PARROT_ERR_BADARG;
    hipStream_t st = (hipStream_t)stream;
    hipError_t e = hipMemsetAsync(dh, 0, sizeof(float) * (size_t)B * H, st);
    if (e != hipSuccess) return (int)e;
    GruStateBwdArgs ga;
    ga.nchain = 1; ga.B = B; ga.H = H;
    ga.chain[0].dh = dh_out; ga.chain[0].dh2 = nullptr; ga.chain[0].hprev = h; ga.chain[0].z = z; ga.chain[0].c = c;
    ga.chain[0].mask = mask; ga.chain[0].dC = d_inputs; ga.chain[0].dG = d_gate_inputs; ga.chain[0].dhprev = dh;
    int rc = gru_state_bwd_launch(ga, st);
    if (rc) return rc;
    SkJob j;
    SkLaunch L;
    sk_job_init(j);
    j.nseg = 1;
    j.seg[0] = sk_seg(d_inputs, H, Wc, H, H, 1);
    j.M = B; j.N = H; j.H = H; j.epi = SK_EPI_BWD_RH;
    j.e0 = h; j.lde0 = H; j.e1 = r; j.lde1 = H;
    j.out = d_gate_inputs + H; j.ldo = 2 * H; j.o1 = dh; j.ldo1 = H;
    rc = sk_make_launch(L, &j, 1);
    if (rc) return rc;
    rc = sk_launch(L, st);
    if (rc) return rc;
    sk_job_init(j);
    j.nseg = 1;
    j.seg[0] = sk_seg(d_gate_inputs, 2 * H, Wg, 2 * H, 2 * H, 1);
    j.M = B; j.N = H; j.H = H; j.epi = SK_EPI_LINEAR; j.accumulate = 1;
    j.out = dh; j.ldo = H;
    rc = sk_make_launch(L, &j, 1);
    if (rc) return rc;
    return sk_launch(L, st);
}

int parrot_gmm_attention_fwd(const float* h1, const float* WattT, const float* batt, const float* kappa_prev,
                             const float* ctx, float* a, float* b, float* kappa, float* phi, float* w, int B,
                             int H, int A, int U, int E, int att_type, float eps, float alignment,
                             float sharpening, float timing, void* stream) { PH_ENTRY();
    if (!h1 || !WattT || !kappa_prev || !ctx || !a || !b || !kappa || !phi || !w) return PARROT_ERR_BADARG;
    AttFwdArgs g{};
    g.h1 = h1; g.ldh = H; g.WattT = WattT; g.batt = batt; g.kappa_prev = kappa_prev; g.ctx = ctx;
    g.a_out = a; g.b_out = b; g.kappa_out = kappa; g.phi_out = phi; g.w_out = w; g.ldw = E;
    g.B = B; g.H = H; g.A = A; g.U = U; g.E = E; g.esplit = att_default_esplit(B, E);
    g.att_type = att_type; g.eps = eps; g.alignment = alignment; g.sharpening = sharpening; g.timing = timing;
    return att_fwd_launch(g, (hipStream_t)stream);
}

int parrot_gmm_attention_bwd(const float* dw, const float* ctx, const float* a, const float* b,
                             const float* kappa, const float* kappa_prev, const float* WattT, float* dkappa,
                             float* dp, float* dh1, int B, int H, int A, int U, int E, int att_type, float eps,
                             void* stream) { PH_ENTRY();
    if (!dw || !ctx || !a || !b || !kappa || !kappa_prev || !WattT || !dkappa || !dp || !dh1)
        return PARROT_ERR_BADARG;
    AttBwdArgs g{};
    g.dw = const_cast<float*>(dw); g.dw2 = nullptr; g.lddw = E; g.ctx = ctx; g.a = a; g.b = b; g.kappa = kappa; g.kappa_prev = kappa_prev;
    g.WattT = WattT; g.dkappa = dkappa; g.dp_out = dp; g.dh1 = dh1; g.lddh = H;
    g.B = B; g.H = H; g.A = A; g.U = U; g.E = E; g.att_type = att_type; g.eps = eps;
    return att_bwd_launch(g, (hipStream_t)stream);
}

int parrot_sumsq(const float* x, size_t n, float* out, void* stream) { PH_ENTRY();
    return sumsq_launch(x, n, out, (hipStream_t)stream);
}

int parrot_adam_clip_step(float* param, const float* grad, float* m, float* v, size_t n,
                          const float* gnorm_sq, float grad_scale, float clip_threshold, float lr,
                          float beta1, float beta2, float eps, int step, void* stream) { PH_ENTRY();
    if (!param || !grad || !m || !v || step < 1) return PARROT_ERR_BADARG;
    if (clip_threshold > 0.f && !gnorm_sq) return PARROT_ERR_BADARG;
    const double lr_t = (double)lr * sqrt(1.0 - pow((double)beta2, step)) / (1.0 - pow((double)beta1, step));
    return adam_clip_launch(param, grad, m, v, n, gnorm_sq, grad_scale, clip_threshold, (float)lr_t, beta1,
                            beta2, eps, (hipStream_t)stream);
}

int parrot_batch_quantize(const float* x, int rows, int n, int ld, double* ws, void* out, int ldo, int mode,
                          int q_levels, void* stream) { PH_ENTRY();
    if (!x || !ws || !out) return PARROT_ERR_BADARG;
    return quantize_launch(x, rows, n, ld, ws, out, ldo, mode, q_levels, (hipStream_t)stream);
}

int parrot_mu2linear(const int32_t* q, size_t n, float* out, void* stream) { PH_ENTRY();
    if (!q || !out) return PARROT_ERR_BADARG;
    return mu2linear_launch(q, n, out, (hipStream_t)stream);
}

}
```

parrot_amd/csrc/elementwise.h:

```cpp
#pragma once
#include "common.h"

#include <map>
#include <mutex>

namespace {
class StreamScratch {
  public:
    explicit StreamScratch(size_t min_floats) : min_floats_(min_floats) {}
    float* get(hipStream_t stream, size_t floats) {
        hipStreamCaptureStatus cs = hipStreamCaptureStatusNone;
        (void)hipStreamIsCapturing(stream, &cs);
        if (cs != hipStreamCaptureStatusNone) return nullptr;
        std::lock_guard<std::mutex> lock(mu_);
        Buf& b = bufs_[stream];
        if (floats > b.cap) {
            if (b.p) {
                (void)hipStreamSynchronize(stream);
                (void)hipFree(b.p);
                b.p = nullptr;
                b.cap = 0;
            }
            const size_t want = floats < min_floats_ ? min_floats_ : floats;
            if (hipMalloc(&b.p, want * sizeof(float)) != hipSuccess) {
                b.p = nullptr;
                return nullptr;
            }
            b.cap = want;
        }
        return b.p;
    }

  private:
    struct Buf { float* p = nullptr; size_t cap = 0; };
    const size_t min_floats_;
    std::mutex mu_;
    std::map<hipStream_t, Buf> bufs_;
};
}

struct GruStateBwdChain {
    const float* dh;
    const float* dh2;
    const float* dhx[3] = {nullptr, nullptr, nullptr};
    const float* hprev;
    const float* z;
    const float* c;
    const float* mask;
    float* dC;
    float* dG;
    float* dhprev;
};
struct GruStateBwdArgs {
    GruStateBwdChain chain[4];
    int nchain, B, H;
};

__device__ __forceinline__ void gru_state_bwd_row(const GruStateBwdChain& c, int m, int H, int tid, int nthr) {
    const unsigned long long a1 = (unsigned long long)c.dh, a2 = (unsigned long long)c.dh2, a3 = (unsigned long long)c.dhx[0],
                             a4 = (unsigned long long)c.dhx[1], a5 = (unsigned long long)c.dhx[2];
    const bool on2 = a2 != 0, on3 = a3 != 0, on4 = a4 != 0, on5 = a5 != 0;
    const float* p2 = reinterpret_cast<const float*>(on2 ? a2 : a1);
    const float* p3 = reinterpret_cast<const float*>(on3 ? a3 : a1);
    const float* p4 = reinterpret_cast<const float*>(on4 ? a4 : a1);
    const float* p5 = reinterpret_cast<const float*>(on5 ? a5 : a1);
    const unsigned long long am = (unsigned long long)c.mask;
    const float* pm = reinterpret_cast<const float*>(am ? am + 4ull * (unsigned)m : (unsigned long long)c.z);
    for (int k = tid; k < H; k += nthr) {
        const size_t i = (size_t)m * H + k;
        const float x1 = c.dh[i], x2 = p2[i], x3 = p3[i], x4 = p4[i], x5 = p5[i];
        const float hp = c.hprev[i], z = c.z[i], cc = c.c[i], dhp = c.dhprev[i], mkv = *pm;
        float dh = x1;
        dh += on2 ? x2 : 0.f;
        dh += on3 ? x3 : 0.f;
        dh += on4 ? x4 : 0.f;
        dh += on5 ? x5 : 0.f;
        float dhp_direct = 0.f;
        if (c.mask) {
            dhp_direct = dh * (1.f - mkv);
            dh *= mkv;
        }
        c.dC[i] = dh * z * (1.f - cc * cc);
        c.dG[(size_t)m * 2 * H + k] = dh * (cc - hp) * z * (1.f - z);
        c.dhprev[i] = dhp + (dh * (1.f - z) + dhp_direct);
    }
}

__device__ __forceinline__ void gru_state_bwd_rows4(const GruStateBwdChain& c, int m0, int nrows, int H, int tid, int nthr) {
    const unsigned long long a1 = (unsigned long long)c.dh, a2 = (unsigned long long)c.dh2, a3 = (unsigned long long)c.dhx[0],
                             a4 = (unsigned long long)c.dhx[1], a5 = (unsigned long long)c.dhx[2];
    const bool on2 = a2 != 0, on3 = a3 != 0, on4 = a4 != 0, on5 = a5 != 0;
    const float* p2 = reinterpret_cast<const float*>(on2 ? a2 : a1);
    const float* p3 = reinterpret_cast<const float*>(on3 ? a3 : a1);
    const float* p4 = reinterpret_cast<const float*>(on4 ? a4 : a1);
    const float* p5 = reinterpret_cast<const float*>(on5 ? a5 : a1);
    for (int k = tid; k < H; k += nthr) {
        float x1[4], x2[4], x3[4], x4[4], x5[4], hp[4], z[4], cc[4], dhp[4], mkv[4];
#pragma unroll
        for (int r = 0; r < 4; ++r) {
            const int m = m0 + (r < nrows ? r : 0);
            const unsigned i = (unsigned)m * (unsigned)H + (unsigned)k;
            x1[r] = c.dh[i]; x2[r] = p2[i]; x3[r] = p3[i]; x4[r] = p4[i]; x5[r] = p5[i];
            hp[r] = c.hprev[i]; z[r] = c.z[i]; cc[r] = c.c[i]; dhp[r] = c.dhprev[i];
            mkv[r] = c.mask ? c.mask[m] : 1.f;
        }
#pragma unroll
        for (int r = 0; r < 4; ++r) {
            if (r >= nrows) break;
            const int m = m0 + r;
            const unsigned i = (unsigned)m * (unsigned)H + (unsigned)k;
            float dh = x1[r];
            dh += on2 ? x2[r] : 0.f;
            dh += on3 ? x3[r] : 0.f;
            dh += on4 ? x4[r] : 0.f;
            dh += on5 ? x5[r] : 0.f;
            float dhp_direct = 0.f;
            if (c.mask) {
                dhp_direct = dh * (1.f - mkv[r]);
                dh *= mkv[r];
            }
            c.dC[i] = dh * z[r] * (1.f - cc[r] * cc[r]);
            c.dG[2u * (unsigned)m * (unsigned)H + (unsigned)k] = dh * (cc[r] - hp[r]) * z[r] * (1.f - z[r]);
            c.dhprev[i] = dhp[r] + (dh * (1.f - z[r]) + dhp_direct);
        }
    }
}

int gru_state_bwd_launch(const GruStateBwdArgs& g, hipStream_t stream);
int colsum_launch(const float* x, long long M, int N, int ld, float* out, int accumulate, hipStream_t stream);
struct ColsumRoute { int vec4, ysplit; };
ColsumRoute colsum_route(const float* x, long long M, int N, int ld, const float* out);
int sumsq_launch(const float* x, size_t n, float* out, hipStream_t stream);
int adam_clip_launch(float* p, const float* g, float* m, float* v, size_t n, const float* gnorm_sq,
                     float grad_scale, float threshold, float lr_t, float b1, float b2, float eps,
                     hipStream_t stream);

int gmm_sample_launch(const float* mu, const float* sig_hat, const float* co_hat, int B, int O, int K, float bias,
                      float eps, const float* unif, const float* noise, float* x, int ldx, float* pi_out,
                      hipStream_t stream);

struct LstmStateBwdChain {
    const float* dh;
    const float* dh2;
    const float* dh3 = nullptr;
    const float* dh4 = nullptr;
    const float* dh5 = nullptr;
    const float* dh6 = nullptr;
    float* dc;
    const float* gates;
    const float* c_prev;
    const float* c_new;
    float* dP;
    void* dP16 = nullptr;
};
struct LstmStateBwdArgs {
    LstmStateBwdChain chain[4];
    int nchain, B, H;
};

struct LstmSbVals { float gi, gf, go, gg, cn, cp, dc, x1, x2, x3, x4, x5, x6; };
__device__ __forceinline__ LstmSbVals lstm_sb_load(const LstmStateBwdChain& c, int m, int H, int k) {
    const size_t idx = (size_t)m * H + k;
    const float* g = c.gates + (size_t)m * 4 * H;
    const float* p2 = c.dh2 ? c.dh2 : c.dh;
    const float* p3 = c.dh3 ? c.dh3 : c.dh;
    const float* p4 = c.dh4 ? c.dh4 : c.dh;
    const float* p5 = c.dh5 ? c.dh5 : c.dh;
    const float* p6 = c.dh6 ? c.dh6 : c.dh;
    LstmSbVals v;
    v.gi = g[k]; v.gf = g[H + k]; v.go = g[2 * H + k]; v.gg = g[3 * H + k];
    v.cn = c.c_new[idx]; v.cp = c.c_prev[idx]; v.dc = c.dc[idx];
    v.x1 = c.dh[idx]; v.x2 = p2[idx]; v.x3 = p3[idx]; v.x4 = p4[idx]; v.x5 = p5[idx]; v.x6 = p6[idx];
    return v;
}
__device__ __forceinline__ float lstm_sb_math(const LstmStateBwdChain& c, const LstmSbVals& v, float (&out)[4]) {
    const float tc = tanhf(v.cn);
    const float dhv = v.x1 + (c.dh2 ? v.x2 : 0.f) + (c.dh3 ? v.x3 : 0.f) + (c.dh4 ? v.x4 : 0.f) + (c.dh5 ? v.x5 : 0.f) +
                      (c.dh6 ? v.x6 : 0.f);
    const float dcv = dhv * v.go * (1.f - tc * tc) + v.dc;
    out[0] = dcv * v.gg * v.gi * (1.f - v.gi);
    out[1] = dcv * v.cp * v.gf * (1.f - v.gf);
    out[2] = dhv * tc * v.go * (1.f - v.go);
    out[3] = dcv * v.gi * (1.f - v.gg * v.gg);
    return dcv * v.gf;
}

__device__ __forceinline__ void lstm_state_bwd_row(const LstmStateBwdChain& c, int m, int H, int tid, int nthr) {
    float* o = c.dP + (size_t)m * 4 * H;
    for (int k = tid; k < H; k += 2 * nthr) {
        const int k2 = k + nthr < H ? k + nthr : k;
        const LstmSbVals va = lstm_sb_load(c, m, H, k), vb = lstm_sb_load(c, m, H, k2);
        float ra[4], rb[4];
        const float da = lstm_sb_math(c, va, ra), db = lstm_sb_math(c, vb, rb);
        o[k] = ra[0]; o[H + k] = ra[1]; o[2 * H + k] = ra[2]; o[3 * H + k] = ra[3];
        c.dc[(size_t)m * H + k] = da;
        if (k2 != k) {
            o[k2] = rb[0]; o[H + k2] = rb[1]; o[2 * H + k2] = rb[2]; o[3 * H + k2] = rb[3];
            c.dc[(size_t)m * H + k2] = db;
        }
    }
}

__device__ __forceinline__ void lstm_state_bwd_row_pub(const LstmStateBwdChain& c, int m, int H, int tid, int nthr, float* row) {
    for (int k = tid; k < H; k += 2 * nthr) {
        const int k2 = k + nthr < H ? k + nthr : k;
        const LstmSbVals va = lstm_sb_load(c, m, H, k), vb = lstm_sb_load(c, m, H, k2);
        float ra[4], rb[4];
        const float da = lstm_sb_math(c, va, ra), db = lstm_sb_math(c, vb, rb);
        row[k] = ra[0]; row[H + k] = ra[1]; row[2 * H + k] = ra[2]; row[3 * H + k] = ra[3];
        c.dc[(size_t)m * H + k] = da;
        if (k2 != k) {
            row[k2] = rb[0]; row[H + k2] = rb[1]; row[2 * H + k2] = rb[2]; row[3 * H + k2] = rb[3];
            c.dc[(size_t)m * H + k2] = db;
        }
    }
    __syncthreads();
    float* o = c.dP + (size_t)m * 4 * H;
    for (int i = tid; i < H; i += nthr) {
        const f32x4 v = *reinterpret_cast<const f32x4*>(row + 4 * i);
        float* q = o + 4 * i;
        asm volatile("global_store_dwordx4 %0, %1, off sc1" ::"v"(q), "v"(v) : "memory");
    }
}

__device__ __forceinline__ void lstm_state_bwd_row_copy16(const LstmStateBwdChain& c, int m, int H, int tid, int nthr, const float* row) {
    if (!c.dP16) return;
    __bf16* o16 = reinterpret_cast<__bf16*>(c.dP16) + (size_t)m * 4 * H;
    for (int i = tid; i < (H >> 1); i += nthr)
        *reinterpret_cast<bf16x8*>(o16 + 8 * i) = ph_bf16x8(*reinterpret_cast<const f32x4*>(row + 8 * i),
                                                            *reinterpret_cast<const f32x4*>(row + 8 * i + 4));
}

int lstm_state_bwd_launch(const float* dh, const float* dh2, float* dc, const float* gates, const float* c_prev, const float* c_new,
                          float* dP, int B, int H, hipStream_t stream);

int simple_norm_fwd_launch(const float* x, int ldx, float* y, int ldy, float* sigma, long long R, int N, float eps,
                           float* add_dst, int ld_add, hipStream_t stream);
int simple_norm_bwd_launch(const float* dy, int lddy, const float* y, int ldy, const float* sigma, float* dx, int lddx,
                           long long R, int N, float eps, int accumulate, hipStream_t stream);

struct NormSumGroup {
    const float* src[4];
    int nsrc, N;
    const float* base;
    float* dst;
};
int norm_sum_launch(const NormSumGroup* groups, int ngroups, int R, float eps, hipStream_t stream);
```

parrot_amd/csrc/elementwise.hip:

```cpp
#include "elementwise.h"

namespace {

__global__ __launch_bounds__(256) void gru_state_bwd_kernel(const GruStateBwdArgs g) {
    const GruStateBwdChain& c = g.chain[blockIdx.y];
    for (int m = blockIdx.x; m < g.B; m += gridDim.x) gru_state_bwd_row(c, m, g.H, threadIdx.x, 256);
}

__global__ __launch_bounds__(256) void colsum_kernel(const float* __restrict__ x, long long M, int N, int ld,
                                                     float* __restrict__ out, int accumulate) {
    __shared__ float red[4][64];
    const int n = blockIdx.x * 64 + (threadIdx.x & 63);
    const int rg = threadIdx.x >> 6;
    float acc = 0.f;
    if (n < N) {
        const long long per = (M + gridDim.y - 1) / gridDim.y;
        const long long mb = (long long)blockIdx.y * per, me = min(M, mb + per);
        for (long long m = mb + rg; m < me; m += 4) acc += x[m * ld + n];
    }
    red[rg][threadIdx.x & 63] = acc;
    __syncthreads();
    if (rg == 0 && n < N) {
        const float s = red[0][threadIdx.x] + red[1][threadIdx.x] + red[2][threadIdx.x] + red[3][threadIdx.x];
        if (gridDim.y > 1) out[(size_t)blockIdx.y * N + n] = s;
        else if (accumulate) out[n] += s;
        else out[n] = s;
    }
}

__global__ __launch_bounds__(256) void colsum4_kernel(const float* __restrict__ x, long long M, int N, int ld,
                                                      float* __restrict__ out, int accumulate) {
    __shared__ f32x4 red[4][64];
    const int lane = threadIdx.x & 63, rg = threadIdx.x >> 6;
    const int n = blockIdx.x * 256 + 4 * lane;
    f32x4 acc = {0.f, 0.f, 0.f, 0.f};
    if (n < N) {
        const long long per = (M + gridDim.y - 1) / gridDim.y;
        const long long mb = (long long)blockIdx.y * per, me = min(M, mb + per);
        const float* p = x + n;
        long long m = mb + rg;
        for (; m + 28 < me; m += 32) {
            f32x4 v[8];
#pragma unroll
            for (int q = 0; q < 8; ++q) v[q] = *reinterpret_cast<const f32x4*>(p + (m + 4 * q) * ld);
#pragma unroll
            for (int q = 0; q < 8; ++q) acc += v[q];
        }
        for (; m < me; m += 4) acc += *reinterpret_cast<const f32x4*>(p + m * ld);
    }
    red[rg][lane] = acc;
    __syncthreads();
    if (rg == 0 && n < N) {
        const f32x4 s = red[0][lane] + red[1][lane] + red[2][lane] + red[3][lane];
        float* o = gridDim.y > 1 ? out + (size_t)blockIdx.y * N + n : out + n;
        f32x4 r = s;
        if (gridDim.y == 1 && accumulate) r += *reinterpret_cast<const f32x4*>(o);
        *reinterpret_cast<f32x4*>(o) = r;
    }
}

__global__ __launch_bounds__(256) void sumsq_kernel(const float* __restrict__ x, size_t n, float* __restrict__ out) {
    __shared__ float red[4];
    float acc = 0.f;
    const size_t n4 = n / 4;
    const f32x4* x4 = reinterpret_cast<const f32x4*>(x);
    for (size_t i = (size_t)blockIdx.x * 256 + threadIdx.x; i < n4; i += (size_t)gridDim.x * 256) {
        const f32x4 v = x4[i];
        acc += v[0] * v[0] + v[1] * v[1] + v[2] * v[2] + v[3] * v[3];
    }
    if (blockIdx.x == 0)
        for (size_t i = n4 * 4 + threadIdx.x; i < n; i += 256) acc += x[i] * x[i];
    acc = wave_sum(acc);
    if ((threadIdx.x & 63) == 0) red[threadIdx.x >> 6] = acc;
    __syncthreads();
    if (threadIdx.x == 0) out[blockIdx.x] = red[0] + red[1] + red[2] + red[3];
}

__global__ __launch_bounds__(256) void sum_partials_kernel(const float* __restrict__ part, int n, float* __restrict__ out) {
    __shared__ float red[4];
    float acc = 0.f;
    for (int i = threadIdx.x; i < n; i += 256) acc += part[i];
    acc = wave_sum(acc);
    if ((threadIdx.x & 63) == 0) red[threadIdx.x >> 6] = acc;
    __syncthreads();
    if (threadIdx.x == 0) out[0] = red[0] + red[1] + red[2] + red[3];
}

__global__ __launch_bounds__(256) void colsum_finish_kernel(const float* __restrict__ part, int N, int ysplit,
                                                            float* __restrict__ out, int accumulate) {
    const int n = blockIdx.x * 256 + threadIdx.x;
    if (n >= N) return;
    float v = accumulate ? out[n] : 0.f;
    int y = 0;
    for (; y + 8 <= ysplit; y += 8) {
        float p[8];
#pragma unroll
        for (int q = 0; q < 8; ++q) p[q] = part[(size_t)(y + q) * N + n];
#pragma unroll
        for (int q = 0; q < 8; ++q) v += p[q];
    }
    for (; y < ysplit; ++y) v += part[(size_t)y * N + n];
    out[n] = v;
}

__global__ __launch_bounds__(256) void adam_clip_kernel(float* __restrict__ p, const float* __restrict__ g,
                                                        float* __restrict__ m, float* __restrict__ v, size_t n,
                                                        const float* __restrict__ gnorm_sq, float grad_scale,
                                                        float threshold, float lr_t, float b1, float b2, float eps) {
    float scale = grad_scale;
    if (threshold > 0.f) {
        const float nrm = sqrtf(*gnorm_sq) * grad_scale;
        if (nrm > threshold) scale *= threshold / nrm;
        if (!(nrm == nrm) || nrm > 3.0e38f) return;
    }
    for (size_t i = (size_t)blockIdx.x * 256 + threadIdx.x; i < n; i += (size_t)gridDim.x * 256) {
        const float gi = g[i] * scale;
        const float mi = b1 * m[i] + (1.f - b1) * gi;
        const float vi = b2 * v[i] + (1.f - b2) * gi * gi;
        m[i] = mi;
        v[i] = vi;
        p[i] -= lr_t * mi / (sqrtf(vi) + eps);
    }
}

__global__ __launch_bounds__(64) void gmm_sample_kernel(const float* __restrict__ mu, const float* __restrict__ sig_hat,
                                                        const float* __restrict__ co_hat, int O, int K, float bias,
                                                        float eps, const float* __restrict__ unif,
                                                        const float* __restrict__ noise, float* __restrict__ x, int ldx,
                                                        float* __restrict__ pi_out) {
    __shared__ int s_pick;
    const int b = blockIdx.x, t = threadIdx.x;
    if (t == 0) {
        const float* c = co_hat + (size_t)b * K;
        const float sc = 1.f + bias;
        float mx = -INFINITY;
        for (int k = 0; k < K; ++k) mx = fmaxf(mx, c[k] * sc);
        float tot = 0.f;
        for (int k = 0; k < K; ++k) tot += expf(c[k] * sc - mx);
        const float u = unif[b];
        float cum = 0.f;
        int pick = K - 1;
        bool found = false;
        for (int k = 0; k < K; ++k) {
            const float pk = expf(c[k] * sc - mx) / tot + eps;
            if (pi_out) pi_out[(size_t)b * K + k] = pk;
            cum += pk;
            if (!found && cum > u) { pick = k; found = true; }
        }
        s_pick = pick;
    }
    __syncthreads();
    const int k = s_pick;
    for (int o = t; o < O; o += 64) {
        const size_t i = (size_t)b * O * K + (size_t)o * K + k;
        x[(size_t)b * ldx + o] = mu[i] + (expf(sig_hat[i] - bias) + eps) * noise[(size_t)b * O + o];
    }
}

__global__ __launch_bounds__(256) void lstm_state_bwd_kernel(const float* __restrict__ dh,
                                                             const float* __restrict__ dh2, float* __restrict__ dc,
                                                             const float* __restrict__ gates,
                                                             const float* __restrict__ c_prev,
                                                             const float* __restrict__ c_new, float* __restrict__ dP,
                                                             int B, int H) {
    const size_t n = (size_t)B * H;
    for (size_t idx = (size_t)blockIdx.x * 256 + threadIdx.x; idx < n; idx += (size_t)gridDim.x * 256) {
        const int m = (int)(idx / H), k = (int)(idx % H);
        const float* g = gates + (size_t)m * 4 * H;
        const float gi = g[k], gf = g[H + k], go = g[2 * H + k], gg = g[3 * H + k];
        const float tc = tanhf(c_new[idx]);
        const float dhv = dh[idx] + (dh2 ? dh2[idx] : 0.f);
        const float dcv = dhv * go * (1.f - tc * tc) + dc[idx];
        float* o = dP + (size_t)m * 4 * H;
        o[k] = dcv * gg * gi * (1.f - gi);
        o[H + k] = dcv * c_prev[idx] * gf * (1.f - gf);
        o[2 * H + k] = dhv * tc * go * (1.f - go);
        o[3 * H + k] = dcv * gi * (1.f - gg * gg);
        dc[idx] = dcv * gf;
    }
}

__device__ __forceinline__ float block_sum256(float v, float* red) {
    v = wave_sum(v);
    __syncthreads();
    if ((threadIdx.x & 63) == 0) red[threadIdx.x >> 6] = v;
    __syncthreads();
    return red[0] + red[1] + red[2] + red[3];
}

__global__ __launch_bounds__(256) void simple_norm_fwd_kernel(const float* x, int ldx, float* y, int ldy,
                                                              float* __restrict__ sigma, int N, float eps,
                                                              float* add_dst, int ld_add) {
    __shared__ float red[4];
    const size_t r = blockIdx.x;
    const float* xr = x + r * ldx;
    float s = 0.f;
    for (int n = threadIdx.x; n < N; n += 256) s += xr[n];
    const float mean = block_sum256(s, red) / (float)N;
    float q = 0.f;
    for (int n = threadIdx.x; n < N; n += 256) {
        const float d = xr[n] - mean;
        q += d * d;
    }
    const float sd = sqrtf(block_sum256(q, red) / (float)N);
    const float inv = 1.f / (eps + sd);
    for (int n = threadIdx.x; n < N; n += 256) {
        const float v = (xr[n] - mean) * inv;
        y[r * ldy + n] = v;
        if (add_dst) add_dst[r * ld_add + n] += v;
    }
    if (threadIdx.x == 0) sigma[r] = sd;
}

__global__ __launch_bounds__(256) void simple_norm_bwd_kernel(const float* dy, int lddy, const float* y, int ldy,
                                                              const float* __restrict__ sigma, float* dx, int lddx,
                                                              int N, float eps, int accumulate) {
    __shared__ float red[4];
    const size_t r = blockIdx.x;
    const float* dyr = dy + r * lddy;
    const float* yr = y + r * ldy;
    float a = 0.f, b = 0.f;
    for (int n = threadIdx.x; n < N; n += 256) {
        a += dyr[n];
        b += dyr[n] * yr[n];
    }
    const float mdy = block_sum256(a, red) / (float)N;
    const float dot = block_sum256(b, red);
    const float sd = sigma[r];
    const float inv = 1.f / (eps + sd);
    const float k = sd > 0.f ? dot / ((float)N * sd) : 0.f;
    for (int n = threadIdx.x; n < N; n += 256) {
        const float v = (dyr[n] - mdy) * inv - yr[n] * k;
        if (accumulate) dx[r * lddx + n] += v;
        else dx[r * lddx + n] = v;
    }
}

struct NormSumArgs {
    NormSumGroup g[2];
};

__global__ __launch_bounds__(256) void norm_sum_kernel(const NormSumArgs a, float eps) {
    __shared__ float red[4];
    const NormSumGroup& g = a.g[blockIdx.y];
    const size_t r = blockIdx.x;
    const int N = g.N;
    float* dst = g.dst + r * N;
    for (int n = threadIdx.x; n < N; n += 256) dst[n] = g.base ? g.base[r * N + n] : 0.f;
    for (int s = 0; s < g.nsrc; ++s) {
        const float* xr = g.src[s] + r * N;
        float sum = 0.f;
        for (int n = threadIdx.x; n < N; n += 256) sum += xr[n];
        const float mean = block_sum256(sum, red) / (float)N;
        float q = 0.f;
        for (int n = threadIdx.x; n < N; n += 256) {
            const float dlt = xr[n] - mean;
            q += dlt * dlt;
        }
        const float inv = 1.f / (eps + sqrtf(block_sum256(q, red) / (float)N));
        for (int n = threadIdx.x; n < N; n += 256) dst[n] += (xr[n] - mean) * inv;
    }
}

}

static StreamScratch ew_scratch(1u << 20);


int norm_sum_launch(const NormSumGroup* groups, int ngroups, int R, float eps, hipStream_t stream) {
    if (ngroups < 1 || ngroups > 2 || R < 1) return PH_ERR_BADARG;
    NormSumArgs a;
    for (int i = 0; i < ngroups; ++i) a.g[i] = groups[i];
    hipLaunchKernelGGL(norm_sum_kernel, dim3((unsigned)R, (unsigned)ngroups), dim3(256), 0, stream, a, eps);
    return (int)hipGetLastError();
}

int simple_norm_fwd_launch(const float* x, int ldx, float* y, int ldy, float* sigma, long long R, int N, float eps,
                           float* add_dst, int ld_add, hipStream_t stream) {
    if (R < 1 || N < 1) return PH_ERR_BADARG;
    hipLaunchKernelGGL(simple_norm_fwd_kernel, dim3((unsigned)R), dim3(256), 0, stream, x, ldx, y, ldy, sigma, N, eps,
                       add_dst, ld_add);
    return (int)hipGetLastError();
}

int simple_norm_bwd_launch(const float* dy, int lddy, const float* y, int ldy, const float* sigma, float* dx, int lddx,
                           long long R, int N, float eps, int accumulate, hipStream_t stream) {
    if (R < 1 || N < 1) return PH_ERR_BADARG;
    hipLaunchKernelGGL(simple_norm_bwd_kernel, dim3((unsigned)R), dim3(256), 0, stream, dy, lddy, y, ldy, sigma, dx,
                       lddx, N, eps, accumulate);
    return (int)hipGetLastError();
}


int lstm_state_bwd_launch(const float* dh, const float* dh2, float* dc, const float* gates, const float* c_prev,
                          const float* c_new, float* dP, int B, int H, hipStream_t stream) {
    const size_t n = (size_t)B * H;
    int bx = (int)((n + 255) / 256);
    if (bx > 1024) bx = 1024;
    hipLaunchKernelGGL(lstm_state_bwd_kernel, dim3(bx), dim3(256), 0, stream, dh, dh2, dc, gates, c_prev, c_new, dP, B,
                       H);
    return (int)hipGetLastError();
}

int gmm_sample_launch(const float* mu, const float* sig_hat, const float* co_hat, int B, int O, int K, float bias,
                      float eps, const float* unif, const float* noise, float* x, int ldx, float* pi_out,
                      hipStream_t stream) {
    hipLaunchKernelGGL(gmm_sample_kernel, dim3(B), dim3(64), 0, stream, mu, sig_hat, co_hat, O, K, bias, eps, unif, noise,
                       x, ldx, pi_out);
    return (int)hipGetLastError();
}

int gru_state_bwd_launch(const GruStateBwdArgs& g, hipStream_t stream) {
    if (g.nchain < 1 || g.nchain > 4) return PH_ERR_BADARG;
    const int bx = g.B < 1024 ? g.B : 1024;
    hipLaunchKernelGGL(gru_state_bwd_kernel, dim3(bx, g.nchain), dim3(256), 0, stream, g);
    return (int)hipGetLastError();
}

static int colsum_scalar_ysplit(long long M, int N) {
    int ysplit = 1;
    const int bx = ceil_div(N, 64);
    while (bx * ysplit < 512 && M / (ysplit * 2) >= 256) ysplit *= 2;
    return ysplit;
}

ColsumRoute colsum_route(const float* x, long long M, int N, int ld, const float* out) {
    ColsumRoute r;
    if (!(N & 3) && !(ld & 3) && !((uintptr_t)x & 15) && !((uintptr_t)out & 15) && M >= 64) {
        const int bx = ceil_div(N, 256);
        int ysplit = 1;
        while (bx * ysplit < 256 && M / (ysplit * 2) >= 64) ysplit *= 2;
        r.vec4 = 1;
        r.ysplit = ysplit;
        return r;
    }
    r.vec4 = 0;
    r.ysplit = colsum_scalar_ysplit(M, N);
    return r;
}

int colsum_launch(const float* x, long long M, int N, int ld, float* out, int accumulate, hipStream_t stream) {
    if (M < 0 || N < 1) return PH_ERR_BADARG;
    ColsumRoute r = colsum_route(x, M, N, ld, out);
    if (r.vec4) {
        const int bx = ceil_div(N, 256), ysplit = r.ysplit;
        float* part = ysplit > 1 ? ew_scratch.get(stream, (size_t)ysplit * N) : nullptr;
        if (ysplit == 1 || part) {
            hipLaunchKernelGGL(colsum4_kernel, dim3(bx, ysplit), dim3(256), 0, stream, x, M, N, ld, ysplit > 1 ? part : out,
                               accumulate);
            if (ysplit > 1)
                hipLaunchKernelGGL(colsum_finish_kernel, dim3(ceil_div(N, 256)), dim3(256), 0, stream, part, N, ysplit, out,
                                   accumulate);
            return (int)hipGetLastError();
        }
        r.ysplit = colsum_scalar_ysplit(M, N);
    }
    int ysplit = r.ysplit;
    const int bx = ceil_div(N, 64);
    if (ysplit > 1) {
        float* part = ew_scratch.get(stream, (size_t)ysplit * N);
        if (!part) ysplit = 1;
        else {
            hipLaunchKernelGGL(colsum_kernel, dim3(bx, ysplit), dim3(256), 0, stream, x, M, N, ld, part, 0);
            hipLaunchKernelGGL(colsum_finish_kernel, dim3(ceil_div(N, 256)), dim3(256), 0, stream, part, N, ysplit, out,
                               accumulate);
            return (int)hipGetLastError();
        }
    }
    hipLaunchKernelGGL(colsum_kernel, dim3(bx, ysplit), dim3(256), 0, stream, x, M, N, ld, out, accumulate);
    return (int)hipGetLastError();
}

int sumsq_launch(const float* x, size_t n, float* out, hipStream_t stream) {
    if (((uintptr_t)x & 15) != 0) return PH_ERR_BADARG;
    int bx = (int)((n / 4 + 255) / 256);
    if (bx < 1) bx = 1;
    if (bx > 2048) bx = 2048;
    float* part = ew_scratch.get(stream, (size_t)bx);
    if (!part) return PH_ERR_UNSUPPORTED;
    hipLaunchKernelGGL(sumsq_kernel, dim3(bx), dim3(256), 0, stream, x, n, part);
    hipLaunchKernelGGL(sum_partials_kernel, dim3(1), dim3(256), 0, stream, part, bx, out);
    return (int)hipGetLastError();
}

int adam_clip_launch(float* p, const float* g, float* m, float* v, size_t n, const float* gnorm_sq,
                     float grad_scale, float threshold, float lr_t, float b1, float b2, float eps,
                     hipStream_t stream) {
    int bx = (int)((n + 255) / 256);
    if (bx < 1) bx = 1;
    if (bx > 4096) bx = 4096;
    hipLaunchKernelGGL(adam_clip_kernel, dim3(bx), dim3(256), 0, stream, p, g, m, v, n, gnorm_sq, grad_scale,
                       threshold, lr_t, b1, b2, eps);
    return (int)hipGetLastError();
}
```

parrot_amd/csrc/switches.h:

```cpp
#pragma once
#include <stdlib.h>

static inline int env_int(const char* name, int dflt) {
    const char* e = getenv(name);
    return e ? atoi(e) : dflt;
}
static inline bool env_set(const char* name) { return getenv(name) != nullptr; }
static inline const char* env_str(const char* name) { return getenv(name); }

static inline int sw_att_dense() { return env_int("PARROT_ATT_DENSE", 0); }
static inline int sw_pm_dataflow(int dflt) { return env_int("PARROT_PM_DATAFLOW", dflt); }
static inline int sw_rg_waves() { return env_int("PARROT_RG_WAVES", 8); }
static inline int sw_wk() { return env_int("PARROT_WK", 1); }
static inline bool sw_pm_dump_plan() { return env_set("PARROT_PM_DUMP_PLAN"); }
```

parrot_amd/model.py:

```python
from __future__ import annotations

import collections
import ctypes as C
from collections import OrderedDict

import numpy
import torch

from . import _lib, ops
from .bricks import Brick, Constant, IsotropicGaussian
from .params import ParamStore
from .utils import env_int

floatX = "float32"


def _simple_norm(x, eps=1e-5):
    return (x - x.mean(-1, keepdim=True)) / (eps + x.std(-1, unbiased=False, keepdim=True))


def logsumexp(x, axis=None):
    x_max = x.max(axis, keepdim=True)[0]
    z = torch.log(torch.exp(x - x_max).sum(axis, keepdim=True)) + x_max
    return z.sum(axis)
# ... 834 lines not shown
        for l in range(1, L + 1):
            rb.add_(self._p(f'/h{l}_to_readout.b'))
        if self.layer_norm:
            ops.gemm(ws['w'][1:].view(T * B, E), Wr[L * H:], bias=self._p('/att_to_readout.b'), out=readouts)
            for l in range(L):
                y, sig = ops.simple_norm_fwd(
                    ops.gemm(ws['h'][l][1:].view(T * B, H), Wr[l * H:(l + 1) * H],
                             bias=self._p(f'/h{l + 1}_to_readout.b')), add_into=readouts)
                save[('ln_ro', l)] = (y, sig)
        elif self._bf16_readouts(T, R):
            cp = self._bf16_copies(ws, T, B, convert=('h', 'w'))
            save['bf16_hw_done'] = True
            Wr16 = save['Wr16'] = ops.to_bf16(Wr)
            ops.gemm16(cp['h'][0][1:T + 1].view(T * B, H), Wr16[0:H], out=readouts, bias=rb)
            for l in range(1, L):
                ops.gemm16(cp['h'][l][1:T + 1].view(T * B, H), Wr16[l * H:(l + 1) * H], out=readouts, accumulate=True)
            ops.gemm16(cp['w'][1:T + 1].view(T * B, E), Wr16[L * H:], out=readouts, accumulate=True)
        else:
            ops.gemm(ws['h'][0][1:].view(T * B, H), Wr[0:H], bias=rb, out=readouts)
            for l in range(1, L):
                ops.gemm(ws['h'][l][1:].view(T * B, H), Wr[l * H:(l + 1) * H], out=readouts, accumulate=True)
            ops.gemm(ws['w'][1:].view(T * B, E), Wr[L * H:], out=readouts, accumulate=True)
        if self.use_speaker:
            spr = ops.gemm(emb_spk, self._p('/speaker_to_readout.W'), bias=self._p('/speaker_to_readout.b'))
            readouts.view(T, B, R).add_(spr.unsqueeze(0))
        preds = []
        for i, (wn, bn, dim) in enumerate(self._out_names):
            pr = ops.gemm(readouts, self.store.param(wn), bias=self.store.param(bn)).view(T, B, dim)
            if self.use_speaker:
                swn, sbn, _ = self._spk_out_names[i]
                pr.add_(ops.gemm(emb_spk, self.store.param(swn), bias=self.store.param(sbn)).unsqueeze(0))
            preds.append(pr)
        return preds

    @property
    def readout_path(self):
        return getattr(self, '_readout_path', None)

    def _readout_composed(self):
        H, E = self.rnn_h_dim, self.encoded_input_dim
        return (not self.layer_norm and not self.use_speaker and not self.compute_bf16
                and len(self._out_names) == 1 and sum(d for _, _, d in self._out_names) <= 64
                and self.readouts_dim >= 256 and H % 16 == 0 and E % 16 == 0
                and env_int('PARROT_READOUT_COMPOSED', 1) != 0)

    @property
    def gmm_cost_path(self):
        return getattr(self, '_gmm_cost_path', None)

    def _gmm_cost_fused(self):
        return (self.which_cost == 'GMM' and not self.raw_output and self.k_gmm <= 64
                and env_int('PARROT_GMM_COST_FUSED', 1) != 0)

    def _gmm_grad_buffers(self, ws, T, B):
        if 'gmm_grads' not in ws:
            ws['gmm_grads'] = tuple(torch.empty(T * B, d, device=self._dev(), dtype=torch.float32)
                                    for _, _, d in self._out_names)
        return ws['gmm_grads']

    def _readouts_buffer(self, ws, T, B):
        if 'readouts' not in ws:
            ws['readouts'] = torch.empty(T * B, self.readouts_dim, device=self._dev(), dtype=torch.float32)
        return ws['readouts']

    def _readout_desc(self, ws, T, B):
        if 'ro_desc' in ws:
            return ws['ro_desc']
        H, E, L, R, O = self.rnn_h_dim, self.encoded_input_dim, self.num_layers, self.readouts_dim, self.output_dim
        d = _lib.ReadoutComposedDesc()
        d.M, d.nseg, d.R, d.O, d.zero_rows, d.slice_rows = T * B, L + 1, R, O, B, 0
        for l in range(L):
            d.K[l], d.ldx[l], d.lddx[l] = H, H, H
            d.x[l], d.dx[l] = ws['h'][l][1:].data_ptr(), ws['dh'][l].data_ptr()
        d.K[L], d.ldx[L], d.lddx[L] = E, E, E
        d.x[L], d.dx[L] = ws['w'][1:].data_ptr(), ws['dw'].data_ptr()
        Wr, gWr = self.store.storage['dec.Wr'], self.store.storage_grad['dec.Wr']
        wn, bn, _ = self._out_names[0]
        Wo, gWo = self.store.param(wn), self.store.grad(wn)
        d.Wr, d.ldwr, d.gWr, d.ldgwr = Wr.data_ptr(), Wr.stride(0), gWr.data_ptr(), gWr.stride(0)
        d.Wo, d.ldwo, d.gWo, d.ldgwo = Wo.data_ptr(), Wo.stride(0), gWo.data_ptr(), gWo.stride(0)
        d.bo, d.gbo = self.store.param(bn).data_ptr(), self.store.grad(bn).data_ptr()
        names = [f'/h{l}_to_readout.b' for l in range(1, L + 1)] + ['/att_to_readout.b']
        d.nbias = len(names)
        for i, n in enumerate(names):
            d.rb[i], d.grb[i] = self._p(n).data_ptr(), self._g(n).data_ptr()
        d.ldp, d.lddp = O, O
        n = int(_lib.load().parrot_readout_composed_ws_floats(C.byref(d)))
        if n <= 0:
            raise _lib.HipCallError(f"parrot_readout_composed_ws_floats failed with code {-n}")
        ws['ro_ws'] = torch.empty(n, device=self._dev(), dtype=torch.float32)
        d.ws_floats = n
        ws['ro_desc'] = d
        return d

    def _backward_f(self, token, gscale):
        if self._saved is None or self._saved[0] != token:
            raise RuntimeError("backward() must follow the compute_cost() call that produced this cost "
                               "(workspaces are reused between calls)")
        save = self._saved[1]
        ws, T, B, U = save['ws'], save['T'], save['B'], save['U']
        H, E, L, R, O, A = (self.rnn_h_dim, self.encoded_input_dim, self.num_layers, self.readouts_dim,
                            self.output_dim, self.attention_size)
        emb_spk = save.get('emb_spk')
        demb_spk = torch.zeros_like(emb_spk) if emb_spk is not None else None

        if 'torch_cost' in save:
            leafs = save['leafs']
            srn = [p_ for p_ in self.sampleRnn.parameters if p_.requires_grad]
            torch.autograd.backward(save['torch_cost'], grad_tensors=gscale.to(save['torch_cost'].dtype),
                                    inputs=list(leafs) + srn)
            save['dpreds'] = [(l.grad if l.grad is not None else torch.zeros_like(l)).reshape(T * B, -1).contiguous()
                              for l in leafs]
            gscale = torch.ones((), device=gscale.device)
        if 'gmm' in save:
            tgt, heads, logr, mrow = save['gmm']
            save['dpreds'] = ops.gmm_cost_bwd(tgt, *heads, logr, (mrow * gscale.to(torch.float32)).contiguous(),
                                              self.epsilon, out=self._gmm_grad_buffers(ws, T, B))
            gscale = None
        if save['readout_composed']:
            rd = self._readout_desc(ws, T, B)
            dp = (save['dpreds'][0] * gscale).contiguous()
            rd.dp = dp.data_ptr()
            _lib.call('parrot_readout_composed_bwd', C.byref(rd), ws['ro_ws'].data_ptr(), ops._stream())
            readout_weight_grads = None
        else:
            readout_weight_grads = self._readouts_factored_bwd(ws, save, T, B, gscale, emb_spk, demb_spk)
        ws['dkappa'].zero_()
        ws['dw0'].zero_()
        for t_ in (ws['dhup'] + ws.get('dcell', []) + ws.get('dhup_b', []) + ws.get('dhup_c', []) +
                   [ws[n] for n in ('dw_b', 'dw_c') if n in ws]):
            if t_ is not None:
                t_.zero_()

        self._scan_bwd_and_weight_grads(ws, save, T, B, before=readout_weight_grads)
        if 'dh_b' in ws:
            for l in range(L):
                ws['dh'][l][0].add_(ws['dh_b'][l][0])
            ws['dw'][0].add_(ws['dw_b'][0])
            ws['dw0'][0].add_(ws['dw0_b'][0])
            if 'dw_c' in ws:
                ws['dw'][0].add_(ws['dw_c'][0])
            if 'dw0_c' in ws:
                ws['dw0'][0].add_(ws['dw0_c'][0])

        sg_, sc_ = self.store.storage_grad, self.store.storage
        for l in range(L):
            ll = l + 1
            for key, wd, suf, mat, rec in self._groups:
                dP = ws['d' + key.upper()][l].view(T * B, wd)
                if self.layer_norm:
                    for j in range(l):
                        self._g(f'/h{j + 1}_to_h{ll}/fork_rnn{ll}_{suf}.b').add_(
                            ops.colsum(ws['ln_y' + key][(l, j)].view(T * B, wd)))
                db = ops.colsum(dP)
                for n in self._layer_bias_names(ll, suf):
                    self._g(n).add_(db)
                if ll in self._fb_layers:
                    dPf, dbf = dP, db
                    if self.layer_norm:
                        dPf = ops.simple_norm_bwd(dP, *save[('ln_fb', ll, key)])
                        dbf = ops.colsum(dPf)
                    ops.gemm(save['fb_inp'].t(), dPf, out=self._g(f'/out_to_h{ll}/fork_rnn{ll}_{suf}.W'),
                             accumulate=True)
                    self._g(f'/out_to_h{ll}/fork_rnn{ll}_{suf}.b').add_(dbf)
                if self.use_speaker:
                    dPs = dP.view(T, B, wd).sum(0)
                    if self.layer_norm:
                        dPs = ops.simple_norm_bwd(dPs, *save[('ln_spk', ll, key)])
                        db = ops.colsum(dPs)
                    ops.gemm(emb_spk.t(), dPs, out=self._g(f'/speaker_to_h{ll}/fork_rnn{ll}_{suf}.W'),
                             accumulate=True)
                    self._g(f'/speaker_to_h{ll}/fork_rnn{ll}_{suf}.b').add_(db)
                    ops.gemm(dPs, self._p(f'/speaker_to_h{ll}/fork_rnn{ll}_{suf}.W').t(), out=demb_spk,
                             accumulate=True)
            if save['start_flag']:
                ops.colsum(ws['dh'][l][0], out=self._g(f'/rnn{ll}.initial_state'), accumulate=True)
                if self.cell_type == 'lstm':
                    ops.colsum(ws['dcell'][l], out=self._g(f'/rnn{ll}.initial_cells'), accumulate=True)
        if save['start_flag']:
            ops.colsum(ws['dw'][0], out=self._g('.initial_w'), accumulate=True)
            ops.colsum(ws['dw0'][0], out=self._g('.initial_w'), accumulate=True)
        ops.colsum(ws['dp'].view(T * B, 3 * A), out=sg_['dec.batt'], accumulate=True)
        dctx = torch.empty(B, U, E, device=ws['ctx'].device, dtype=torch.float32)
        with ops.gemm_precision(ops.PRECISION_F32):
            _lib.call('parrot_gemm', ws['phi'].data_ptr(), B * U, 1, ws['dw'][1:].data_ptr(), B * E, 0,
                      dctx.data_ptr(), E, U, E, T, None, 1.0, 0, 0, B, U, E, U * E, 1, ops._stream())
            if self.use_speaker:
                self._scatter_rows_add(self._g('/lookuptable.W'), save['spk_idx'], demb_spk)
            self._encoder_backward(dctx, save)
        self._saved = None

    def _readouts_factored_bwd(self, ws, save, T, B, gscale, emb_spk, demb_spk):
        H, E, L, R = self.rnn_h_dim, self.encoded_input_dim, self.num_layers, self.readouts_dim
        readouts = ws['readouts']
        dread = torch.empty(T * B, R, device=readouts.device, dtype=torch.float32)
        for i, (wn, bn, dim) in enumerate(self._out_names):
            dp = save['dpreds'][i] if gscale is None else save['dpreds'][i] * gscale
            ops.gemm(readouts.t(), dp, out=self.store.grad(wn), accumulate=True)
            ops.colsum(dp, out=self.store.grad(bn), accumulate=True)
            ops.gemm(dp, self.store.param(wn).t(), out=dread, accumulate=i > 0)
            if self.use_speaker:
                swn, sbn, _ = self._spk_out_names[i]
                dsum = dp.view(T, B, dim).sum(0)
                ops.gemm(emb_spk.t(), dsum, out=self.store.grad(swn), accumulate=True)
                ops.colsum(dsum, out=self.store.grad(sbn), accumulate=True)
                ops.gemm(dsum, self.store.param(swn).t(), out=demb_spk, accumulate=True)
        gWr = self.store.storage_grad['dec.Wr']
        Wr = self.store.storage['dec.Wr']
        db = ops.colsum(dread)
        dro = [dread] * L
        if self.layer_norm:
            dro = [ops.simple_norm_bwd(dread, *save[('ln_ro', l)]) for l in range(L)]
        def readout_weight_grads():
            if self._bf16_weight_grads(0, T, T) and R % 8 == 0 and not self.layer_norm:
                cp = self._bf16_copies(ws, T, B, convert=() if save.get('bf16_hw_done') else ('h', 'w'))
                ws['bf16_hw_fresh'] = True
                d16 = save['d16'] if 'd16' in save else ops.to_bf16(dread)
                for l in range(L):
                    ops.gemm_bf16in(cp['h'][l][1:T + 1].view(T * B, H), d16, gWr[l * H:(l + 1) * H], accumulate=True)
                ops.gemm_bf16in(cp['w'][1:T + 1].view(T * B, E), d16, gWr[L * H:], accumulate=True)
                return
            for l in range(L):
                ops.gemm(ws['h'][l][1:].view(T * B, H).t(), dro[l], out=gWr[l * H:(l + 1) * H], accumulate=True)
            ops.gemm(ws['w'][1:].view(T * B, E).t(), dread, out=gWr[L * H:], accumulate=True)
        for l in range(L):
            self._g(f'/h{l + 1}_to_readout.b').add_(ops.colsum(dro[l]) if self.layer_norm else db)
        self._g('/att_to_readout.b').add_(db)
        if self.use_speaker:
            dsum = dread.view(T, B, R).sum(0)
            ops.gemm(emb_spk.t(), dsum, out=self._g('/speaker_to_readout.W'), accumulate=True)
            ops.colsum(dsum, out=self._g('/speaker_to_readout.b'), accumulate=True)
            ops.gemm(dsum, self._p('/speaker_to_readout.W').t(), out=demb_spk, accumulate=True)
        if 'Wr16' in save:
            Wr16 = save['Wr16']
            d16 = save['d16'] = ops.to_bf16(dread)
            for l in range(L):
                ws['dh'][l][0].zero_()
                ops.gemm16(d16, Wr16[l * H:(l + 1) * H].t(), out=ws['dh'][l][1:].view(T * B, H))
            ws['dw'][0].zero_()
            ops.gemm16(d16, Wr16[L * H:].t(), out=ws['dw'][1:].view(T * B, E))
        else:
            for l in range(L):
                ws['dh'][l][0].zero_()
                ops.gemm(dro[l], Wr[l * H:(l + 1) * H].t(), out=ws['dh'][l][1:].view(T * B, H))
            ws['dw'][0].zero_()
            ops.gemm(dread, Wr[L * H:].t(), out=ws['dw'][1:].view(T * B, E))
        return readout_weight_grads

    def _weight_grad_rows(self, ws, save, T, B, t0, t1):
        if t1 <= t0:
            return
        H, E, L = self.rnn_h_dim, self.encoded_input_dim, self.num_layers
        sg_ = self.store.storage_grad
        R = (t1 - t0) * B
        if self._bf16_weight_grads(t0, t1, T):
            return self._weight_grad_rows_bf16(ws, T, B)
        for l in range(L):
            ll = l + 1
            hprev = ws['h'][l][t0:t1].view(R, H)
            wsrc = (ws['w'][t0:t1] if l == 0 else ws['w'][t0 + 1:t1 + 1]).view(R, E)
            for key, wd, suf, mat, rec in self._groups:
                dP = ws['d' + key.upper()][l][t0:t1].view(R, wd)
                gW = sg_[f'{mat}{ll}']
                rec_in = ws['rh'][l][t0:t1].view(R, H) if key == 'c' else hprev
                ops.gemm(rec_in.t(), dP, out=gW[0:H], accumulate=True)
                ops.gemm(wsrc.t(), dP, out=gW[H:H + E], accumulate=True)
                for j in range(l):
                    r0 = H + E + j * H
                    dPj = dP
                    if self.layer_norm:
                        dPj = ws['ln_y' + key][(l, j)][t0:t1].view(R, wd)
                    ops.gemm(ws['h'][j][t0 + 1:t1 + 1].view(R, H).t(), dPj, out=gW[r0:r0 + H], accumulate=True)
                if t0 == 0 and t1 == T:
                    self._gradient_ready(f'{mat}{ll}')
        A = self.attention_size
        with ops.gemm_precision(ops.PRECISION_F32):
            ops.gemm(ws['dp'][t0:t1].view(R, 3 * A).t(), ws['h'][0][t0 + 1:t1 + 1].view(R, H),
                     out=sg_['dec.WattT'], accumulate=True)

    def _gradient_ready(self, storage_name):
        hook = getattr(self, 'on_gradient_ready', None)
        if hook is not None:
            o, n = self.store.offsets[storage_name]
            hook(o, o + (n + 3) // 4 * 4)

    def _bf16_weight_grads(self, t0, t1, T):
        H, E = self.rnn_h_dim, self.encoded_input_dim
        return (self.compute_bf16 and not self.layer_norm and t0 == 0 and t1 == T and H % 8 == 0 and E % 8 == 0
                and env_int('PARROT_BF16_DW', 1) != 0)

    def _bf16_readouts(self, T, R):
        return (self._bf16_weight_grads(0, T, T) and R % 8 == 0 and not self.use_speaker
                and env_int('PARROT_BF16_READOUT', 1) != 0)

    def _bf16_copies(self, ws, T, B, convert=()):
        H, E, L = self.rnn_h_dim, self.encoded_input_dim, self.num_layers
        cp = ws.get('bf16_copies')
        if cp is None:
            bf = dict(device=self._dev(), dtype=torch.bfloat16)
            cp = ws['bf16_copies'] = dict(
                h=[torch.empty(T + 1, B, H, **bf) for _ in range(L)], w=torch.empty(T + 1, B, E, **bf),
                rh=[torch.empty(T, B, H, **bf) for _ in range(L)] if self.cell_type != 'lstm' else None,
                d={key: [torch.empty(T, B, wd, **bf) for _ in range(L)] for key, wd, _, _, _ in self._groups})
        if 'w' in convert:
            ops.to_bf16(ws['w'], out=cp['w'])
        for l in range(L):
            if 'h' in convert:
                ops.to_bf16(ws['h'][l], out=cp['h'][l])
            if 'd' in convert:
                if cp['rh'] is not None:
                    ops.to_bf16(ws['rh'][l], out=cp['rh'][l])
                for key, wd, _, _, _ in self._groups:
                    ops.to_bf16(ws['d' + key.upper()][l], out=cp['d'][key][l])
        return cp

    def _weight_grad_rows_bf16(self, ws, T, B):
        H, E, L = self.rnn_h_dim, self.encoded_input_dim, self.num_layers
        sg_ = self.store.storage_grad
        R = T * B
        fresh = ('d',) if ws.pop('bf16_hw_fresh', False) else ('h', 'w', 'd')
        if ws.get('plan_writes_d16'):
            fresh = tuple(x for x in fresh if x != 'd')
        cp = self._bf16_copies(ws, T, B, convert=fresh)
        for l in range(L):
            ll = l + 1
            hprev = cp['h'][l][0:T].view(R, H)
            wsrc = (cp['w'][0:T] if l == 0 else cp['w'][1:T + 1]).view(R, E)
            for key, wd, suf, mat, rec in self._groups:
                dP = cp['d'][key][l].view(R, wd)
                gW = sg_[f'{mat}{ll}']
                rec_in = cp['rh'][l].view(R, H) if key == 'c' else hprev
                ops.gemm_bf16in(rec_in, dP, gW[0:H], accumulate=True)
                ops.gemm_bf16in(wsrc, dP, gW[H:H + E], accumulate=True)
                for j in range(l):
                    r0 = H + E + j * H
                    ops.gemm_bf16in(cp['h'][j][1:T + 1].view(R, H), dP, gW[r0:r0 + H], accumulate=True)
        A = self.attention_size
        with ops.gemm_precision(ops.PRECISION_F32):
            ops.gemm(ws['dp'].view(R, 3 * A).t(), ws['h'][0][1:T + 1].view(R, H), out=sg_['dec.WattT'], accumulate=True)

    def _scan_bwd_and_weight_grads(self, ws, save, T, B, before=None):
        if before is not None:
            before()
        hook = getattr(self, 'on_early_gradients', None)
        if hook is not None:
            hook()
        _lib.call('parrot_decoder_seq_bwd', ws['plan'], ops._stream())
        self._weight_grad_rows(ws, save, T, B, 0, T)

    def _sample_workspace(self, S, N, U, stop_extra=0):
        ws_key = ('stop', S, N, U, stop_extra) if stop_extra else (S, N, U)
        ws = self._sample_ws.get(ws_key)
        if ws is not None:
            return ws
        H, E, A, L, R, O = (self.rnn_h_dim, self.encoded_input_dim, self.attention_size, self.num_layers,
                            self.readouts_dim, self.output_dim)
        if self.decode_bf16:
            why = self._decode_bf16_refusal(N)
            if why:
                raise ValueError("decode_dtype='bf16' " + why)
        ldx = (O + 3) // 4 * 4
        f = dict(device=self._dev(), dtype=torch.float32)
        ws = dict(
            x=torch.zeros(S + 1, N, ldx, **f), h=[torch.zeros(2, N, H, **f) for _ in range(L)],
            w=torch.zeros(S + 1, N, E, **f), kappa=torch.zeros(S + 1, N, A, **f),
            a=torch.empty(S, N, A, **f), bwork=torch.empty(N, A, **f), phi=torch.empty(S, N, U, **f),
            zwork=torch.empty(N, H, **f), rwork=torch.empty(N, H, **f), rhwork=torch.empty(N, H, **f),
            readout=torch.empty(N, R, **f), ctx=torch.zeros(N, U, E, **f),
            br=torch.zeros(R, **f), ldx=ldx,
            radd=torch.zeros(N, R, **f) if self.use_speaker else None,
            oadd=torch.zeros(N, O, **f) if (self.use_speaker and self.which_cost == 'MSE') else None,
        )
        lstm = self.cell_type == 'lstm'
        for key, wd, suf, mat, rec in self._groups:
            ws['b' + key] = [torch.zeros(wd, **f) for _ in range(L)]
            ws['seq_' + key] = [torch.zeros(N, wd, **f) if self.use_speaker else None for _ in range(L)]
        if lstm:
            ws.update(cwork=[torch.zeros(2, N, H, **f) for _ in range(L)], gwork=torch.empty(N, 4 * H, **f))
        gmm = self.which_cost == 'GMM'
        if gmm:
            K = self.k_gmm
            ws.update(unif=torch.zeros(S, N, **f), noise=torch.zeros(S, N, O, **f),
                      gmm_mu=torch.empty(N, O * K, **f), gmm_sig=torch.empty(N, O * K, **f),
                      gmm_co=torch.empty(N, K, **f), pi_out=torch.empty(S, N, K, **f),
                      add_mu=torch.zeros(N, O * K, **f) if self.use_speaker else None,
                      add_sig=torch.zeros(N, O * K, **f) if self.use_speaker else None,
                      add_co=torch.zeros(N, K, **f) if self.use_speaker else None)
        d = _lib.SampleDesc()
        d.S, d.B, d.H, d.E, d.A, d.U, d.L, d.O, d.R, d.ldx = S, N, H, E, A, U, L, O, R, ldx
        d.att_type = 1 if self.attention_type == 'softmax' else 0
        d.use_graph = int(self.use_graph)
        d.eps, d.alignment = self.epsilon, self.attention_alignment
        d.sharpening, d.timing = self.sharpening_coeff, self.timing_coeff
        st = self.store.storage
        d.cell = 1 if lstm else 0
        for l in range(L):
            for key, wd, suf, mat, rec in self._groups:
                getattr(d, 'W' + key)[l] = st[f'{mat}{l + 1}'].data_ptr()
                getattr(d, 'b' + key)[l] = ws['b' + key][l].data_ptr()
                if (l + 1) in self._fb_layers:
                    getattr(d, 'Wf' + key)[l] = self._p(f'/out_to_h{l + 1}/fork_rnn{l + 1}_{suf}.W').data_ptr()
                if self.use_speaker:
                    getattr(d, 'seq_' + key)[l] = ws['seq_' + key][l].data_ptr()
            d.h[l] = ws['h'][l].data_ptr()
            if lstm:
                d.cwork[l] = ws['cwork'][l].data_ptr()
        if lstm:
            d.gwork = ws['gwork'].data_ptr()
        if self.layer_norm:
            widths = sum(wd for key, wd, suf, mat, rec in self._groups)
            ws['ln_scratch'] = torch.empty(N * (5 * widths + (L + 1) * R), **f)
            d.layer_norm = 1
            d.ln_scratch, d.ln_scratch_floats = ws['ln_scratch'].data_ptr(), ws['ln_scratch'].numel()
            for l in range(L):
                d.br_l[l] = self._p(f'/h{l + 1}_to_readout.b').data_ptr()
                for key, wd, suf, mat, rec in self._groups:
                    if (l + 1) in self._fb_layers:
                        getattr(d, 'bf' + key)[l] = self._p(f'/out_to_h{l + 1}/fork_rnn{l + 1}_{suf}.b').data_ptr()
# ... 364 lines not shown
```

parrot_amd/ops.py:

```python
from __future__ import annotations

import torch

from . import _lib
from .utils import env_int, env_str

ACT_NONE, ACT_RELU, ACT_TANH, ACT_SIGMOID = 0, 1, 2, 3


def _stream() -> int:
    return torch.cuda.current_stream().cuda_stream


def _chk(t: torch.Tensor, name: str, dtype=torch.float32):
    if not isinstance(t, torch.Tensor) or not t.is_cuda:
        raise _lib.HipCallError(
            f"{name}: the parrot_amd product path needs a GPU tensor (got {type(t).__name__}"
            f"{'' if not isinstance(t, torch.Tensor) else ' on ' + str(t.device)}); there is no CPU fallback")
    if t.dtype != dtype:
        raise TypeError(f"{name}: expected {dtype}, got {t.dtype}")


def ptr(t, name="tensor", dtype=torch.float32) -> int:
    if t is None:
        return None
    _chk(t, name, dtype)
    if not t.is_contiguous():
        raise ValueError(f"{name}: tensor must be contiguous")
    return t.data_ptr()


def _mat(t: torch.Tensor, name: str):
    _chk(t, name)
    if t.dim() != 2:
        raise ValueError(f"{name}: expected a 2-D tensor")
    if t.stride(1) == 1 and t.stride(0) >= max(1, t.shape[1]):
        return t.data_ptr(), t.shape[0], t.shape[1], t.stride(0), 0
    if t.stride(0) == 1 and t.stride(1) >= max(1, t.shape[0]):
        return t.data_ptr(), t.shape[0], t.shape[1], t.stride(1), 1
    if t.shape[0] == 1 or t.shape[1] == 1:
        t = t.contiguous()
        return t.data_ptr(), t.shape[0], t.shape[1], t.stride(0), 0
    raise ValueError(f"{name}: unsupported strides {t.stride()}")


def gemm(a: torch.Tensor, b: torch.Tensor, bias=None, out=None, accumulate=False, act=ACT_NONE,
         alpha=1.0, split_k=0) -> torch.Tensor:
    if accumulate and int(act) != ACT_NONE:
        raise ValueError("gemm: accumulate together with an activation is not defined")
    pa, M, K, lda, ta = _mat(a, "a")
    pb, K2, N, ldb, tb = _mat(b, "b")
    if K != K2:
        raise ValueError(f"gemm: inner dimensions differ ({K} vs {K2})")
    if out is None:
        if accumulate:
            out = torch.zeros((M, N), device=a.device, dtype=torch.float32)
        else:
            out = torch.empty((M, N), device=a.device, dtype=torch.float32)
    _chk(out, "out")
    if out.shape != (M, N) or out.stride(1) != 1:
        raise ValueError("gemm: bad output tensor")
    if M == 0 or N == 0:
        return out
    if K == 0:
        if not accumulate:
            out.zero_()
        return out
    _lib.call("parrot_gemm", pa, lda, ta, pb, ldb, tb, out.data_ptr(), out.stride(0), M, N, K,
              ptr(bias, "bias"), float(alpha), int(bool(accumulate)), int(act), 1, 0, 0, 0, int(split_k),
              _stream())
    return out


ROUTE_STEP, ROUTE_F32, ROUTE_BF16, ROUTE_BF16X3 = 0, 1, 2, 3


def gemm_route(a: torch.Tensor, b: torch.Tensor, bias=None, out=None, accumulate=False, act=ACT_NONE, alpha=1.0,
               split_k=0, gate=None, nbatch=None, transA=False, transB=False):
    import ctypes as C
    if nbatch is not None:
        _chk(a, "a"); _chk(b, "b")
        if a.shape[0] != nbatch or b.shape[0] != nbatch:
            raise ValueError("gemm_route: nbatch does not match the operands")
        M, K = (a.shape[2], a.shape[1]) if transA else (a.shape[1], a.shape[2])
        N = b.shape[1] if transB else b.shape[2]
        args = (a.data_ptr(), a.stride(1), int(transA), b.data_ptr(), b.stride(1), int(transB), M, N, K, 1.0, 0,
                int(nbatch), a.stride(0), b.stride(0), 1, 0)
    else:
        pa, M, K, lda, ta = _mat(a, "a")
        pb, K2, N, ldb, tb = _mat(b, "b")
        if K != K2:
            raise ValueError(f"gemm_route: inner dimensions differ ({K} vs {K2})")
        if gate is not None:
            args = (pa, lda, ta, pb, ldb, tb, M, N, K, 1.0, 0, 1, 0, 0, 0, 1)
        else:
            args = (pa, lda, ta, pb, ldb, tb, M, N, K, float(alpha), int(act), 1, 0, 0, int(split_k), 0)
    kernel, slices = C.c_int(-1), C.c_int(-1)
    _lib.call("parrot_gemm_route", *args, C.byref(kernel), C.byref(slices))
    return kernel.value, slices.value


def to_bf16(x: torch.Tensor, out=None) -> torch.Tensor:
    _chk(x, "x")
    if not x.is_contiguous() or x.numel() % 8:
        raise ValueError("to_bf16: contiguous tensor with a multiple of 8 elements expected")
    if out is None:
        out = torch.empty(x.shape, device=x.device, dtype=torch.bfloat16)
    if out.dtype != torch.bfloat16 or out.numel() != x.numel() or not out.is_contiguous() or not out.is_cuda:
        raise ValueError("to_bf16: bad output tensor")
    _lib.call("parrot_to_bf16", x.data_ptr(), out.data_ptr(), x.numel(), _stream())
    return out


def gemm_bf16in(a_t: torch.Tensor, b: torch.Tensor, out: torch.Tensor, accumulate=False, split_k=0) -> torch.Tensor:
    for x_, n_ in ((a_t, "a_t"), (b, "b")):
        if not (x_.is_cuda and x_.dtype == torch.bfloat16 and x_.dim() == 2 and x_.stride(1) == 1):
            raise ValueError(f"gemm_bf16in: {n_} must be a 2-d bf16 GPU tensor with unit inner stride")
    _chk(out, "out")
    K, M = a_t.shape
    K2, N = b.shape
    if K != K2 or out.shape != (M, N) or out.stride(1) != 1:
        raise ValueError("gemm_bf16in: shapes do not match")
    _lib.call("parrot_gemm_bf16in", a_t.data_ptr(), a_t.stride(0), b.data_ptr(), b.stride(0), out.data_ptr(),
              out.stride(0), M, N, K, int(bool(accumulate)), int(split_k), _stream())
    return out


def gemm16(a: torch.Tensor, b: torch.Tensor, out=None, bias=None, accumulate=False, split_k=0) -> torch.Tensor:
    pa, M, K, lda, ta = _mat16(a, "a")
    pb, K2, N, ldb, tb = _mat16(b, "b")
    if K != K2:
        raise ValueError(f"gemm16: inner dimensions differ ({K} vs {K2})")
    if out is None:
        out = (torch.zeros if accumulate else torch.empty)((M, N), device=a.device, dtype=torch.float32)
    _chk(out, "out")
    if out.shape != (M, N) or out.stride(1) != 1:
        raise ValueError("gemm16: bad output tensor")
    _lib.call("parrot_gemm_bf16in_ex", pa, lda, ta, pb, ldb, tb, out.data_ptr(), out.stride(0), M, N, K,
              ptr(bias, "bias"), int(bool(accumulate)), int(split_k), _stream())
    return out


def _mat16(t: torch.Tensor, name: str):
    _chk(t, name, torch.bfloat16)
    if t.dim() != 2:
        raise ValueError(f"{name}: expected a 2-D tensor")
    if t.stride(1) == 1 and t.stride(0) >= max(1, t.shape[1]):
        return t.data_ptr(), t.shape[0], t.shape[1], t.stride(0), 0
    if t.stride(0) == 1 and t.stride(1) >= max(1, t.shape[0]):
        return t.data_ptr(), t.shape[0], t.shape[1], t.stride(1), 1
    raise ValueError(f"{name}: unsupported strides {t.stride()}")


PRECISION_F32, PRECISION_BF16, PRECISION_BF16X3 = 0, 1, 2


def _default_full_precision() -> int:
    return PRECISION_F32 if env_str("PARROT_GEMM_PRECISION", "") in ("f32", "0") else PRECISION_BF16X3


_FULL_PRECISION = _default_full_precision()


def full_precision() -> int:
    return _FULL_PRECISION


def set_full_precision(mode: int) -> int:
    global _FULL_PRECISION
    if mode not in (PRECISION_F32, PRECISION_BF16X3):
        raise ValueError("set_full_precision: PRECISION_F32 or PRECISION_BF16X3")
    prev, _FULL_PRECISION = _FULL_PRECISION, int(mode)
    _lib.call("parrot_set_gemm_precision", int(mode))
    return prev


class gemm_precision:

    def __init__(self, mode):
        self.mode = int(mode)

    def __enter__(self):
        self.prev = int(_lib.load().parrot_get_gemm_precision())
        _lib.call("parrot_set_gemm_precision", self.mode)
        return self

    def __exit__(self, *exc):
        _lib.call("parrot_set_gemm_precision", self.prev)
        return False


def gemm_batched(a, b, out, transA=False, transB=False, accumulate=False):
    _chk(a, "a"); _chk(b, "b"); _chk(out, "out")
    nb = a.shape[0]
    M, K = (a.shape[2], a.shape[1]) if transA else (a.shape[1], a.shape[2])
    N = b.shape[1] if transB else b.shape[2]
    assert a.stride(2) == 1 and b.stride(2) == 1 and out.stride(2) == 1
    _lib.call("parrot_gemm", a.data_ptr(), a.stride(1), int(transA), b.data_ptr(), b.stride(1), int(transB),
              out.data_ptr(), out.stride(1), M, N, K, None, 1.0, int(bool(accumulate)), 0, nb,
              a.stride(0), b.stride(0), out.stride(0), 1, _stream())
    return out


def colsum(x: torch.Tensor, out=None, accumulate=False) -> torch.Tensor:
    _chk(x, "x")
    x2 = x.reshape(-1, x.shape[-1])
    if x2.stride(1) != 1:
        x2 = x2.contiguous()
    M, N = x2.shape
    if out is None:
        out = torch.empty((N,), device=x.device, dtype=torch.float32)
        accumulate = False
    if M == 0:
        if not accumulate:
            out.zero_()
        return out
    _lib.call("parrot_colsum", x2.data_ptr(), M, N, x2.stride(0), out.data_ptr(), int(bool(accumulate)), _stream())
    return out


def colsum_route(x: torch.Tensor, out=None):
    import ctypes as C
    _chk(x, "x")
    N = x.shape[-1]
    M = x.numel() // N if N else 0
    if x.dim() == 2 and x.stride(1) == 1:
        px, ld = x.data_ptr(), x.stride(0)
    elif x.is_contiguous():
        px, ld = x.data_ptr(), N
    else:
        px, ld = 4096, N
    info = (C.c_int * 2)(-1, -1)
    _lib.call("parrot_colsum_route", px, M, N, ld, None if out is None else out.data_ptr(), info)
    return info[0], info[1]


class _LinearFn(torch.autograd.Function):

    @staticmethod
    def forward(ctx, x, W, b, act):
        x2 = x.reshape(-1, x.shape[-1])
        if x2.stride(-1) != 1:
            x2 = x2.contiguous()
        y = gemm(x2, W, bias=b, act=act)
        ctx.save_for_backward(x2, W, y if act != ACT_NONE else None)
        ctx.act = act
        ctx.has_b = b is not None
        ctx.xshape = x.shape
        return y.reshape(*x.shape[:-1], W.shape[1])

    @staticmethod
    def backward(ctx, dy):
        x2, W, y = ctx.saved_tensors
        dy2 = dy.reshape(-1, dy.shape[-1])
        if ctx.act == ACT_RELU:
            dy2 = dy2 * (y > 0).to(dy2.dtype)
        elif ctx.act == ACT_TANH:
            dy2 = dy2 * (1 - y * y)
        elif ctx.act == ACT_SIGMOID:
            dy2 = dy2 * y * (1 - y)
        if not dy2.is_contiguous():
            dy2 = dy2.contiguous()
        dx = dW = db = None
        if ctx.needs_input_grad[0]:
            dx = gemm(dy2, W.t()).reshape(ctx.xshape)
        if ctx.needs_input_grad[1]:
            dW = gemm(x2.t(), dy2)
        if ctx.has_b and ctx.needs_input_grad[2]:
            db = colsum(dy2)
        return dx, dW, db, None


def linear(x, W, b=None, act=ACT_NONE):
    return _LinearFn.apply(x, W, b, act)


def gemm_gated(a: torch.Tensor, b: torch.Tensor, gate: torch.Tensor, out=None) -> torch.Tensor:
    pa, M, K, lda, ta = _mat(a, "a")
    pb, K2, N, ldb, tb = _mat(b, "b")
    _chk(gate, "gate")
    if K != K2 or gate.shape != (M, N) or gate.stride(1) != 1:
        raise ValueError("gemm_gated: shapes do not match")
    if out is None:
        out = torch.empty((M, N), device=a.device, dtype=torch.float32)
    _chk(out, "out")
    if out.shape != (M, N) or out.stride(1) != 1:
        raise ValueError("gemm_gated: bad output tensor")
    _lib.call("parrot_gemm_gated", pa, lda, ta, pb, ldb, tb, out.data_ptr(), out.stride(0), M, N, K,
              gate.data_ptr(), gate.stride(0), _stream())
    return out


def _int32(t: torch.Tensor, name: str, bound=None) -> torch.Tensor:
    if not isinstance(t, torch.Tensor) or not t.is_cuda:
        raise _lib.HipCallError(f"{name}: the parrot_amd product path needs a GPU tensor; there is no CPU fallback")
    t32 = t.to(torch.int32).contiguous()
    if bound is not None and t32.numel() and not _SKIP_INDEX_CHECK:
        lo, hi = int(t32.min()), int(t32.max())
        if lo < 0 or hi >= bound:
            raise IndexError(f"{name}: values in [{lo}, {hi}] outside [0, {bound})")
    return t32


_SKIP_INDEX_CHECK = env_int("PARROT_SKIP_INDEX_CHECK", 0) != 0


class _EmbedSumFn(torch.autograd.Function):

    @staticmethod
    def forward(ctx, E, W1, idx, add):
        Q, EMB = E.shape
        N, J = idx.shape
        D = W1.shape[1]
        if W1.shape[0] != J * EMB:
            raise ValueError("embed_sum: W1 must be [J * EMB, D]")
        E_, W1_ = E.contiguous(), W1.contiguous()
        idx32 = _int32(idx, "idx", bound=Q)
        tbl = torch.empty(J, Q, D, device=E.device, dtype=torch.float32)
        with gemm_precision(PRECISION_F32):
            gemm_batched(E_.unsqueeze(0).expand(J, -1, -1), W1_.view(J, EMB, D), tbl)
        y = torch.empty(N, D, device=E.device, dtype=torch.float32)
        if add is not None:
            _chk(add, "add")
            add = add.reshape(N, D)
            if add.stride(1) != 1:
                add = add.contiguous()
        _lib.call("parrot_gather_sum_fwd", tbl.data_ptr(), idx32.data_ptr(), add.data_ptr() if add is not None else None,
                  add.stride(0) if add is not None else 0, y.data_ptr(), y.stride(0), N, J, Q, D, _stream())
        ctx.save_for_backward(E_, W1_, idx32)
        ctx.has_add = add is not None
        return y

    @staticmethod
    def backward(ctx, dy):
        E, W1, idx32 = ctx.saved_tensors
        Q, EMB = E.shape
        N, J = idx32.shape
        D = W1.shape[1]
        dy = dy.reshape(N, D)
        if dy.stride(1) != 1:
            dy = dy.contiguous()
        vals, perm = torch.sort(idx32.t().contiguous(), dim=1, stable=True)
        bins = torch.arange(Q + 1, device=E.device, dtype=torch.int32).unsqueeze(0).expand(J, -1).contiguous()
        offs = torch.searchsorted(vals, bins).to(torch.int32).contiguous()
        perm = perm.to(torch.int32).contiguous()
        n_ws = int(_lib.load().parrot_gather_sum_bwd_ws_floats(N, J, Q, D))
        ws = torch.empty(n_ws, device=E.device, dtype=torch.float32)
        dtbl = torch.empty(J, Q, D, device=E.device, dtype=torch.float32)
        _lib.call("parrot_gather_sum_bwd", dy.data_ptr(), dy.stride(0), perm.data_ptr(), offs.data_ptr(), dtbl.data_ptr(),
                  ws.data_ptr(), n_ws, N, J, Q, D, 0, _stream())
        dE = dW1 = None
        with gemm_precision(PRECISION_F32):
            if ctx.needs_input_grad[0]:
                t = torch.empty(J, Q, EMB, device=E.device, dtype=torch.float32)
                gemm_batched(dtbl, W1.view(J, EMB, D), t, transB=True)
                dE = t.sum(0)
            if ctx.needs_input_grad[1]:
                dW1 = torch.empty(J, EMB, D, device=E.device, dtype=torch.float32)
                gemm_batched(E.unsqueeze(0).expand(J, -1, -1), dtbl, dW1, transA=True)
                dW1 = dW1.view(J * EMB, D)
        return dE, dW1, None, (dy if ctx.has_add and ctx.needs_input_grad[3] else None)


def embed_sum(E, W1, idx, add=None):
    return _EmbedSumFn.apply(E, W1, idx, add)


def _label_desc(labels32, Q, mats, field):
    import ctypes as C
    d = _lib.LabelTablesDesc()
    d.N, d.Q, d.nseg = labels32.numel(), int(Q), len(mats)
    d.labels = ptr(labels32, "labels", torch.int32)
    for s, (m, rows) in enumerate(mats):
        if rows.shape != (labels32.numel(), m.shape[1]) or m.shape[0] != Q:
            raise ValueError("label tables: expected [Q, D] tables / sums and [N, D] row matrices")
        getattr(d, field)[s], d.rows[s], d.D[s] = ptr(m, field), ptr(rows, "rows"), m.shape[1]
    return d, C.byref(d)


def label_tables_supported(N, Q) -> bool:
    return bool(_lib.load().parrot_label_tables_supported(int(N), int(Q)))


def label_gather(labels32, tables, rows):
    d, ref = _label_desc(labels32, tables[0].shape[0], list(zip(tables, rows)), "tbl")
    _lib.call("parrot_label_gather", ref, _stream())


def label_segsum(labels32, rows, sums, ws=None):
    Q = sums[0].shape[0]
    d, ref = _label_desc(labels32, Q, list(zip(sums, rows)), "sums")
    n_ws = int(_lib.load().parrot_label_segsum_ws_floats(d.N, Q, sum(m.shape[1] for m in sums)))
    if ws is None or ws.numel() < n_ws:
        ws = torch.empty(n_ws, device=labels32.device, dtype=torch.float32)
    _lib.call("parrot_label_segsum", ref, ws.data_ptr(), ws.numel(), _stream())
    return ws


class _ReluMlpFn(torch.autograd.Function):

    @staticmethod
    def forward(ctx, x, W2, b2, W3, b3, W4, b4):
        x = x.reshape(-1, x.shape[-1])
        if x.stride(1) != 1:
            x = x.contiguous()
        y2 = gemm(x, W2, bias=b2, act=ACT_RELU)
        y3 = gemm(y2, W3, bias=b3, act=ACT_RELU)
        out = gemm(y3, W4, bias=b4)
        ctx.save_for_backward(x, y2, y3, W2, W3, W4)
        return out

    @staticmethod
    def backward(ctx, dl):
        x, y2, y3, W2, W3, W4 = ctx.saved_tensors
        if not dl.is_contiguous():
            dl = dl.contiguous()
        need = ctx.needs_input_grad
        d3 = gemm_gated(dl, W4.t(), y3)
        dW4 = gemm(y3.t(), dl) if need[5] else None
        db4 = colsum(dl) if need[6] else None
        d2 = gemm_gated(d3, W3.t(), y2)
        dW3 = gemm(y2.t(), d3) if need[3] else None
        db3 = colsum(d3) if need[4] else None
        dW2 = gemm(x.t(), d2) if need[1] else None
        db2 = colsum(d2) if need[2] else None
        dx = gemm(d2, W2.t()) if need[0] else None
        return dx, dW2, db2, dW3, db3, dW4, db4


def relu_mlp(x, W2, b2, W3, b3, W4, b4):
    return _ReluMlpFn.apply(x, W2, b2, W3, b3, W4, b4)


class _SoftmaxCeFn(torch.autograd.Function):

    @staticmethod
    def forward(ctx, logits, target):
        _chk(logits, "logits")
        x = logits.reshape(-1, logits.shape[-1])
        if x.stride(1) != 1:
            x = x.contiguous()
        rows, Q = x.shape
# ... 446 lines not shown
```

Baseline: 916,300 frames/s.

## Fuse bias-gradient column sums into weight-gradient GEMM and fan out bias adds

Computes the column sum of dP (the bias gradient) inside the bf16x3 split GEMM that already streams dP for the recurrent weight gradient. Only the tm==0 tiles accumulate the sums, with split-K partials reduced in the reduce kernel. This removes a separate colsum pass over dP for each layer and gate. Several per-name bias add_ calls are also replaced by one fan-out kernel, and LDS pitches are changed for two other GEMM variants. The cost is extra adds and an LDS reduction in one row of tiles, plus a larger split-K workspace.

After: 923,100 frames/s (median of 6 runs). Within noise of the previous version (+0.7%).

```diff
diff --git a/include/parrot_hip.h b/include/parrot_hip.h
--- a/include/parrot_hip.h
+++ b/include/parrot_hip.h
@@ -39,6 +39,15 @@
 int parrot_gemm_route(const float* A, int lda, int transA, const float* B, int ldb, int transB, int M, int N, int K,
                       float alpha, int act, int nbatch, long long strideA, long long strideB, int split_k, int has_gate,
                       int* kernel, int* slices);
+
+int parrot_gemm_colsum(const float* A, int lda, int transA, const float* B, int ldb, int transB, float* C, int ldc,
+                       int M, int N, int K, float alpha, int accumulate, int split_k, float* colsum, int colsum_accumulate,
+                       void* stream);
+int parrot_gemm_colsum_fused(const float* A, int lda, int transA, const float* B, int ldb, int transB, int M, int N, int K,
+                             float alpha, int act, int nbatch, long long strideA, long long strideB, int split_k,
+                             int has_gate, int* fused);
+
+int parrot_add_fanout(const float* src, float* const* dst, int ndst, size_t n, void* stream);
 
 int parrot_step_launch_mode(int njobs, const int* M, const int* N, const int* K, const int* lstm_H, int* info);
 
diff --git a/parrot_amd/_lib.py b/parrot_amd/_lib.py
--- a/parrot_amd/_lib.py
+++ b/parrot_amd/_lib.py
@@ -174,7 +174,11 @@
     "parrot_gemm_gated": (_i, [_vp, _i, _i, _vp, _i, _i, _vp, _i, _i, _i, _i, _vp, _i, _vp]),
     "parrot_gemm_route": (_i, [_vp, _i, _i, _vp, _i, _i, _i, _i, _i, _f, _i, _i, _ll, _ll, _i, _i,
                                C.POINTER(C.c_int), C.POINTER(C.c_int)]),
-    "parrot_step_launch_mode": (_i, [_i] + [C.POINTER(C.c_int)] * 5),
+    "parrot_gemm_colsum": (_i, [_vp, _i, _i, _vp, _i, _i, _vp, _i, _i, _i, _i, _f, _i, _i, _vp, _i, _vp]),
+    "parrot_gemm_colsum_fused": (_i, [_vp, _i, _i, _vp, _i, _i, _i, _i, _i, _f, _i, _i, _ll, _ll, _i, _i,
+                                      C.POINTER(C.c_int)]),
+    "parrot_add_fanout": (_i, [_vp, C.POINTER(C.c_void_p), _i, _sz, _vp]),
+    "parrot_step_launch_mode":(_i, [_i] + [C.POINTER(C.c_int)] * 5),
     "parrot_gather_sum_fwd": (_i, [_vp, _vp, _vp, _i, _vp, _i, _ll, _i, _i, _i, _vp]),
     "parrot_gather_sum_bwd_ws_floats": (C.c_longlong, [_ll, _i, _i, _i]),
     "parrot_gather_sum_bwd": (_i, [_vp, _i, _vp, _vp, _vp, _vp, _ll, _ll, _i, _i, _i, _i, _vp]),
diff --git a/parrot_amd/csrc/biggemm.h b/parrot_amd/csrc/biggemm.h
--- a/parrot_amd/csrc/biggemm.h
+++ b/parrot_amd/csrc/biggemm.h
@@ -19,7 +19,12 @@
     const float* gate;
     int ldg;
     int bf16;
+    float* colsum = nullptr;
+    int colsum_accumulate = 0;
 };
+
+bool bg_colsum_supported(const BgArgs& a);
+size_t bg_ws_floats(const BgArgs& a);
 
 int bg_launch(const BgArgs& a, hipStream_t stream);
 void bg_tile_shape(int bf16, int& bm, int& bn);
diff --git a/parrot_amd/csrc/biggemm.hip b/parrot_amd/csrc/biggemm.hip
--- a/parrot_amd/csrc/biggemm.hip
+++ b/parrot_amd/csrc/biggemm.hip
@@ -146,7 +146,7 @@
 }
 
 
-constexpr int BK16 = 32, PITCH16 = 40, PITCHT = 144;
+constexpr int BK16 = 32, PITCH16 = 40, PITCHT = 160;
 
 template <bool XC>
 __device__ __forceinline__ void bg_load16(const float* __restrict__ p, int x0, int X, int k0, int kend,
@@ -294,7 +294,7 @@
     }
 }
 
-constexpr int HBMT = 256, HBNT = 256, HPITCH = 272;
+constexpr int HBMT = 256, HBNT = 256, HPITCH = 288;
 template <int BKT, bool XC>
 struct BghOperand {
     static constexpr int PK = BKT + 8;
@@ -446,6 +446,15 @@
     p2 = __builtin_convertvector(r2, bf16x4);
 }
 
+__device__ __forceinline__ void bgs_colsum_add(f32x4& cs, const f32x4& v) {
+#pragma unroll
+    for (int u = 0; u < 4; ++u) {
+        float r;
+        asm("v_add_f32 %0, %1, %2" : "=v"(r) : "v"(cs[u]), "v"(v[u]));
+        cs[u] = r;
+    }
+}
+
 template <bool XC>
 struct BgsOperand {
     static constexpr int PK = SBK + 8;
@@ -511,8 +520,9 @@
     }
 };
 
-template <bool AXC, bool BXC>
+template <bool AXC, bool BXC, bool CS = false>
 __global__ __launch_bounds__(512) void bgs_kernel(const BgArgs a, int vecA, int vecB, int tiles_m, int tiles_n, int zmap) {
+    static_assert(!CS || BXC, "column sums ride on an x-contiguous B");
     typedef BgsOperand<AXC> OA;
     typedef BgsOperand<BXC> OB;
     extern __shared__ __attribute__((aligned(16))) __bf16 bgs_smem[];
@@ -550,12 +560,15 @@
 #pragma unroll
             for (int q = 0; q < 16; ++q) acc[i][j][q] = 0.f;
     f32x4 ra[2], rb[2];
+    const bool sums = CS && tm == 0;
+    f32x4 cs = {0.f, 0.f, 0.f, 0.f};
     const int nk = (kend - kbeg + SBK - 1) / SBK;
     if (nk > 0) {
         OA::load(A, lda, m0, a.M, kbeg, kend, vecA, t, ra);
         OB::load(B, ldb, n0, a.N, kbeg, kend, vecB, t, rb);
         OA::store(As, t, ra);
         OB::store(Bs, t, rb);
+        if (sums) { bgs_colsum_add(cs, rb[0]); bgs_colsum_add(cs, rb[1]); }
         if (nk > 1) {
             OA::load(A, lda, m0, a.M, kbeg + SBK, kend, vecA, t, ra);
             OB::load(B, ldb, n0, a.N, kbeg + SBK, kend, vecB, t, rb);
@@ -570,6 +583,7 @@
         if (early && kt + 1 < nk) {
             OA::store(As + (cur ^ 1) * OA::SZ, t, ra);
             OB::store(Bs + (cur ^ 1) * OB::SZ, t, rb);
+            if (sums) { bgs_colsum_add(cs, rb[0]); bgs_colsum_add(cs, rb[1]); }
             if (kt + 2 < nk) {
                 OA::load(A, lda, m0, a.M, kbeg + (kt + 2) * SBK, kend, vecA, t, ra);
                 OB::load(B, ldb, n0, a.N, kbeg + (kt + 2) * SBK, kend, vecB, t, rb);
@@ -599,12 +613,26 @@
         if (!early && kt + 1 < nk) {
             OA::store(As + (cur ^ 1) * OA::SZ, t, ra);
             OB::store(Bs + (cur ^ 1) * OB::SZ, t, rb);
+            if (sums) { bgs_colsum_add(cs, rb[0]); bgs_colsum_add(cs, rb[1]); }
             if (kt + 2 < nk) {
                 OA::load(A, lda, m0, a.M, kbeg + (kt + 2) * SBK, kend, vecA, t, ra);
                 OB::load(B, ldb, n0, a.N, kbeg + (kt + 2) * SBK, kend, vecB, t, rb);
             }
         }
         __syncthreads();
+    }
+    if (sums) {
+        float* red = reinterpret_cast<float*>(bgs_smem);
+        *reinterpret_cast<f32x4*>(red + wave * 256 + 4 * lane) = cs;
+        __syncthreads();
+        const int n = n0 + t;
+        if (t < 256 && n < a.N) {
+            float v = red[t];
+#pragma unroll
+            for (int w = 1; w < 8; ++w) v += red[w * 256 + t];
+            if (a.splitk > 1) a.ws[(long long)a.splitk * a.M * a.N + (long long)ks * a.N + n] = v;
+            else a.colsum[n] = a.colsum_accumulate ? a.colsum[n] + v : v;
+        }
     }
 #pragma unroll
     for (int i = 0; i < 4; ++i)
@@ -662,8 +690,24 @@
         if (a.gate && !(a.gate[(long long)m * a.ldg + n] > 0.f)) v = 0.f;
         *c = v;
     }
-}
-
+    if (a.colsum) {
+        const float* strip = a.ws + (long long)a.splitk * mn;
+        for (long long n = (long long)blockIdx.x * 256 + threadIdx.x; n < a.N; n += (long long)gridDim.x * 256) {
+            float v = a.colsum_accumulate ? a.colsum[n] : 0.f;
+            for (int ks = 0; ks < a.splitk; ++ks) v += strip[(long long)ks * a.N + n];
+            a.colsum[n] = v;
+        }
+    }
+}
+
+}
+
+bool bg_colsum_supported(const BgArgs& a) {
+    return a.bf16 == 3 && a.sam == 1 && a.sbn == 1 && a.nbatch == 1 && !a.gate && a.act == 0;
+}
+
+size_t bg_ws_floats(const BgArgs& a) {
+    return (size_t)a.nbatch * a.splitk * a.M * a.N + (a.colsum ? (size_t)a.splitk * a.N : 0);
 }
 
 int bg_reduce_launch(const BgArgs& a, hipStream_t stream) {
@@ -695,12 +739,12 @@
     hipLaunchKernelGGL((bgh_kernel<BKT, AX, BX>), grid, dim3(512), lds, stream, a, tm, tn);
 }
 
-template <bool AX, bool BX>
+template <bool AX, bool BX, bool CS = false>
 static void bgs_go(const BgArgs& a, dim3 grid, int vecA, int vecB, int tm, int tn, int zmap, hipStream_t stream) {
     static bool done = false;
-    bg_big_lds_once(bgs_kernel<AX, BX>, done);
+    bg_big_lds_once(bgs_kernel<AX, BX, CS>, done);
     const size_t lds = (size_t)4 * (BgsOperand<AX>::SZ + BgsOperand<BX>::SZ);
-    hipLaunchKernelGGL((bgs_kernel<AX, BX>), grid, dim3(512), lds, stream, a, vecA, vecB, tm, tn, zmap);
+    hipLaunchKernelGGL((bgs_kernel<AX, BX, CS>), grid, dim3(512), lds, stream, a, vecA, vecB, tm, tn, zmap);
 }
 
 int bg_to_bf16_launch(const float* x, void* y, long long n, hipStream_t stream) {
@@ -719,6 +763,7 @@
     const bool axc = (a.sam == 1), bxc = (a.sbn == 1);
     if (!axc && a.sak != 1) return PH_ERR_BADARG;
     if (!bxc && a.sbk != 1) return PH_ERR_BADARG;
+    if (a.colsum && !bg_colsum_supported(a)) return PH_ERR_BADARG;
     auto al = [](const float* p, long long stride, long long batch) {
         return (((uintptr_t)p & 15) == 0) && (stride % 4 == 0) && (batch % 4 == 0);
     };
@@ -750,7 +795,8 @@
         const int Z = a.nbatch * a.splitk;
         const int zmap = (Z % 8 == 0) ? 1 : 0;
         const dim3 g = zmap ? dim3(tm * tn * Z) : dim3(tm * tn, Z);
-        if (axc && bxc) bgs_go<true, true>(a, g, vecA, vecB, tm, tn, zmap, stream);
+        if (a.colsum) bgs_go<true, true, true>(a, g, vecA, vecB, tm, tn, zmap, stream);
+        else if (axc && bxc) bgs_go<true, true>(a, g, vecA, vecB, tm, tn, zmap, stream);
         else if (axc) bgs_go<true, false>(a, g, vecA, vecB, tm, tn, zmap, stream);
         else if (bxc) bgs_go<false, true>(a, g, vecA, vecB, tm, tn, zmap, stream);
         else bgs_go<false, false>(a, g, vecA, vecB, tm, tn, zmap, stream);
diff --git a/parrot_amd/csrc/capi.hip b/parrot_amd/csrc/capi.hip
--- a/parrot_amd/csrc/capi.hip
+++ b/parrot_amd/csrc/capi.hip
@@ -94,7 +94,7 @@
     a.ws = nullptr;
     if (a.splitk > 1) {
         if (act != 0) return PARROT_ERR_BADARG;
-        float* ws = bg_workspace.get(st, (size_t)nbatch * a.splitk * M * N);
+        float* ws = bg_workspace.get(st, bg_ws_floats(a));
         if (ws) {
             a.ws = ws;
             a.bias = nullptr;
@@ -124,6 +124,10 @@
 
 static int gemm_mode_in_force() { return t_gemm_bf16 >= 0 ? t_gemm_bf16 : g_gemm_bf16.load(std::memory_order_relaxed); }
 
+static bool gemm_colsum_rides(int route, int transA, int transB, int act, int nbatch, bool has_gate) {
+    return sw_wgrad_fused() && route == PARROT_GEMM_ROUTE_BF16X3 && transA && !transB && act == 0 && nbatch == 1 && !has_gate;
+}
+
 static int gemm_route_bf16(int route) {
     return route == PARROT_GEMM_ROUTE_BF16X3 ? 3 : route == PARROT_GEMM_ROUTE_BF16 ? 1 : 0;
 }
@@ -131,13 +135,14 @@
 static int gemm_impl(const float* A, int lda, int transA, const float* B, int ldb, int transB, float* C, int ldc,
                      int M, int N, int K, const float* bias, float alpha, int accumulate, int act, int nbatch,
                      long long strideA, long long strideB, long long strideC, int split_k, const float* gate, int ldg,
-                     void* stream) {
+                     void* stream, float* colsum = nullptr, int colsum_accumulate = 0) {
     if (!A || !B || !C || M < 1 || N < 1 || K < 1 || nbatch < 1) return PARROT_ERR_BADARG;
     if (gate && (nbatch != 1 || ldg < N)) return PARROT_ERR_BADARG;
     if (act != 0 && accumulate) return PARROT_ERR_BADARG;
     hipStream_t st = (hipStream_t)stream;
     const int route = gemm_pick_kernel(A, lda, transA, B, ldb, transB, M, N, K, alpha, act, nbatch, strideA, strideB, split_k,
                                        gate != nullptr, gemm_mode_in_force());
+    if (colsum && !gemm_colsum_rides(route, transA, transB, act, nbatch, gate != nullptr)) return PARROT_ERR_BADARG;
     if (route == PARROT_GEMM_ROUTE_STEP) {
         SkJob j;
         sk_job_init(j);
@@ -162,6 +167,7 @@
     a.accumulate = accumulate; a.alpha = alpha; a.act = act;
     a.gate = gate; a.ldg = ldg;
     a.bf16 = gemm_route_bf16(route);
+    a.colsum = colsum; a.colsum_accumulate = colsum_accumulate;
     return bg_run(a, split_k, st);
 }
 
@@ -176,6 +182,25 @@
                       int M, int N, int K, const float* gate, int ldg, void* stream) { PH_ENTRY();
     if (!gate) return PARROT_ERR_BADARG;
     return gemm_impl(A, lda, transA, B, ldb, transB, C, ldc, M, N, K, nullptr, 1.0f, 0, 0, 1, 0, 0, 0, 0, gate, ldg, stream);
+}
+
+int parrot_gemm_colsum(const float* A, int lda, int transA, const float* B, int ldb, int transB, float* C, int ldc,
+                       int M, int N, int K, float alpha, int accumulate, int split_k, float* colsum, int colsum_accumulate,
+                       void* stream) { PH_ENTRY();
+    if (!colsum) return PARROT_ERR_BADARG;
+    return gemm_impl(A, lda, transA, B, ldb, transB, C, ldc, M, N, K, nullptr, alpha, accumulate, 0, 1, 0, 0, 0, split_k,
+                     nullptr, 0, stream, colsum, colsum_accumulate);
+}
+
+int parrot_gemm_colsum_fused(const float* A, int lda, int transA, const float* B, int ldb, int transB, int M, int N, int K,
+                             float alpha, int act, int nbatch, long long strideA, long long strideB, int split_k,
+                             int has_gate, int* fused) {
+    if (!A || !B || !fused || M < 1 || N < 1 || K < 1 || nbatch < 1) return PARROT_ERR_BADARG;
+    if (has_gate && nbatch != 1) return PARROT_ERR_BADARG;
+    const int route = gemm_pick_kernel(A, lda, transA, B, ldb, transB, M, N, K, alpha, act, nbatch, strideA, strideB, split_k,
+                                       has_gate != 0, gemm_mode_in_force());
+    *fused = gemm_colsum_rides(route, transA, transB, act, nbatch, has_gate != 0) ? 1 : 0;
+    return 0;
 }
 
 int parrot_gemm_route(const float* A, int lda, int transA, const float* B, int ldb, int transB, int M, int N, int K,
@@ -388,6 +413,10 @@
                             beta2, eps, (hipStream_t)stream);
 }
 
+int parrot_add_fanout(const float* src, float* const* dst, int ndst, size_t n, void* stream) { PH_ENTRY();
+    return add_fanout_launch(src, dst, ndst, n, (hipStream_t)stream);
+}
+
 int parrot_batch_quantize(const float* x, int rows, int n, int ld, double* ws, void* out, int ldo, int mode,
                           int q_levels, void* stream) { PH_ENTRY();
     if (!x || !ws || !out) return PARROT_ERR_BADARG;
diff --git a/parrot_amd/csrc/elementwise.h b/parrot_amd/csrc/elementwise.h
--- a/parrot_amd/csrc/elementwise.h
+++ b/parrot_amd/csrc/elementwise.h
@@ -134,6 +134,9 @@
 int adam_clip_launch(float* p, const float* g, float* m, float* v, size_t n, const float* gnorm_sq,
                      float grad_scale, float threshold, float lr_t, float b1, float b2, float eps,
                      hipStream_t stream);
+constexpr int ADD_FANOUT_MAX = 4;
+struct AddFanoutDst { float* p[ADD_FANOUT_MAX]; };
+int add_fanout_launch(const float* src, float* const* dst, int ndst, size_t n, hipStream_t stream);
 
 int gmm_sample_launch(const float* mu, const float* sig_hat, const float* co_hat, int B, int O, int K, float bias,
                       float eps, const float* unif, const float* noise, float* x, int ldx, float* pi_out,
diff --git a/parrot_amd/csrc/elementwise.hip b/parrot_amd/csrc/elementwise.hip
--- a/parrot_amd/csrc/elementwise.hip
+++ b/parrot_amd/csrc/elementwise.hip
@@ -120,6 +120,15 @@
         m[i] = mi;
         v[i] = vi;
         p[i] -= lr_t * mi / (sqrtf(vi) + eps);
+    }
+}
+
+__global__ __launch_bounds__(256) void add_fanout_kernel(const float* __restrict__ src, AddFanoutDst d, int ndst, size_t n) {
+    for (size_t i = (size_t)blockIdx.x * 256 + threadIdx.x; i < n; i += (size_t)gridDim.x * 256) {
+        const float s = src[i];
+#pragma unroll
+        for (int q = 0; q < ADD_FANOUT_MAX; ++q)
+            if (q < ndst) d.p[q][i] += s;
     }
 }
 
@@ -393,3 +402,17 @@
                        threshold, lr_t, b1, b2, eps);
     return (int)hipGetLastError();
 }
+
+int add_fanout_launch(const float* src, float* const* dst, int ndst, size_t n, hipStream_t stream) {
+    if (!src || !dst || ndst < 1 || ndst > ADD_FANOUT_MAX) return PH_ERR_BADARG;
+    AddFanoutDst d;
+    for (int q = 0; q < ADD_FANOUT_MAX; ++q) {
+        d.p[q] = q < ndst ? dst[q] : nullptr;
+        if (q < ndst && !dst[q]) return PH_ERR_BADARG;
+    }
+    if (n == 0) return 0;
+    int bx = (int)((n + 255) / 256);
+    if (bx > 4096) bx = 4096;
+    hipLaunchKernelGGL(add_fanout_kernel, dim3(bx), dim3(256), 0, stream, src, d, ndst, n);
+    return (int)hipGetLastError();
+}
diff --git a/parrot_amd/csrc/switches.h b/parrot_amd/csrc/switches.h
--- a/parrot_amd/csrc/switches.h
+++ b/parrot_amd/csrc/switches.h
@@ -12,4 +12,5 @@
 static inline int sw_pm_dataflow(int dflt) { return env_int("PARROT_PM_DATAFLOW", dflt); }
 static inline int sw_rg_waves() { return env_int("PARROT_RG_WAVES", 8); }
 static inline int sw_wk() { return env_int("PARROT_WK", 1); }
+static inline int sw_wgrad_fused() { return env_int("PARROT_WGRAD_FUSED", 1); }
 static inline bool sw_pm_dump_plan() { return env_set("PARROT_PM_DUMP_PLAN"); }
diff --git a/parrot_amd/model.py b/parrot_amd/model.py
--- a/parrot_amd/model.py
+++ b/parrot_amd/model.py
@@ -1010,9 +1010,10 @@
                     for j in range(l):
                         self._g(f'/h{j + 1}_to_h{ll}/fork_rnn{ll}_{suf}.b').add_(
                             ops.colsum(ws['ln_y' + key][(l, j)].view(T * B, wd)))
-                db = ops.colsum(dP)
-                for n in self._layer_bias_names(ll, suf):
-                    self._g(n).add_(db)
+                db = save.get('db', {}).get((l, key))
+                if db is None:
+                    db = ops.colsum(dP)
+                ops.add_fanout(db, [self._g(n) for n in self._layer_bias_names(ll, suf)])
                 if ll in self._fb_layers:
                     dPf, dbf = dP, db
                     if self.layer_norm:
@@ -1121,7 +1122,13 @@
                 dP = ws['d' + key.upper()][l][t0:t1].view(R, wd)
                 gW = sg_[f'{mat}{ll}']
                 rec_in = ws['rh'][l][t0:t1].view(R, H) if key == 'c' else hprev
-                ops.gemm(rec_in.t(), dP, out=gW[0:H], accumulate=True)
+                db = None
+                if t0 == 0 and t1 == T:
+                    db = ws.setdefault('db', {}).get((l, key))
+                    if db is None:
+                        db = ws['db'][(l, key)] = torch.empty(wd, device=dP.device, dtype=torch.float32)
+                    save.setdefault('db', {})[(l, key)] = db
+                ops.gemm(rec_in.t(), dP, out=gW[0:H], accumulate=True, colsum_out=db)
                 ops.gemm(wsrc.t(), dP, out=gW[H:H + E], accumulate=True)
                 for j in range(l):
                     r0 = H + E + j * H
diff --git a/parrot_amd/ops.py b/parrot_amd/ops.py
--- a/parrot_amd/ops.py
+++ b/parrot_amd/ops.py
@@ -45,13 +45,23 @@
 
 
 def gemm(a: torch.Tensor, b: torch.Tensor, bias=None, out=None, accumulate=False, act=ACT_NONE,
-         alpha=1.0, split_k=0) -> torch.Tensor:
+         alpha=1.0, split_k=0, colsum_out=None, colsum_accumulate=False) -> torch.Tensor:
     if accumulate and int(act) != ACT_NONE:
         raise ValueError("gemm: accumulate together with an activation is not defined")
     pa, M, K, lda, ta = _mat(a, "a")
     pb, K2, N, ldb, tb = _mat(b, "b")
     if K != K2:
         raise ValueError(f"gemm: inner dimensions differ ({K} vs {K2})")
+    if colsum_out is not None:
+        _chk(colsum_out, "colsum_out")
+        if colsum_out.shape != (N,) or not colsum_out.is_contiguous():
+            raise ValueError("gemm: colsum_out must be a contiguous [N] tensor")
+        fused = (bias is None and M > 0 and N > 0 and K > 0 and
+                 _colsum_fused((pa, lda, ta, pb, ldb, tb, M, N, K, float(alpha), int(act), 1, 0, 0, int(split_k), 0)))
+        if not fused:
+            out = gemm(a, b, bias=bias, out=out, accumulate=accumulate, act=act, alpha=alpha, split_k=split_k)
+            colsum(b, out=colsum_out, accumulate=colsum_accumulate)
+            return out
     if out is None:
         if accumulate:
             out = torch.zeros((M, N), device=a.device, dtype=torch.float32)
@@ -66,10 +76,50 @@
         if not accumulate:
             out.zero_()
         return out
+    if colsum_out is not None:
+        _lib.call("parrot_gemm_colsum", pa, lda, ta, pb, ldb, tb, out.data_ptr(), out.stride(0), M, N, K, float(alpha),
+                  int(bool(accumulate)), int(split_k), colsum_out.data_ptr(), int(bool(colsum_accumulate)), _stream())
+        return out
     _lib.call("parrot_gemm", pa, lda, ta, pb, ldb, tb, out.data_ptr(), out.stride(0), M, N, K,
               ptr(bias, "bias"), float(alpha), int(bool(accumulate)), int(act), 1, 0, 0, 0, int(split_k),
               _stream())
     return out
+
+
+def _colsum_fused(route_args) -> bool:
+    import ctypes as C
+    fused = C.c_int(-1)
+    _lib.call("parrot_gemm_colsum_fused", *route_args, C.byref(fused))
+    return fused.value == 1
+
+
+def gemm_colsum_fused(a: torch.Tensor, b: torch.Tensor, act=ACT_NONE, alpha=1.0, split_k=0, gate=None, nbatch=None,
+                      transA=False, transB=False) -> bool:
+    if nbatch is not None:
+        _chk(a, "a"); _chk(b, "b")
+        M, K = (a.shape[2], a.shape[1]) if transA else (a.shape[1], a.shape[2])
+        N = b.shape[1] if transB else b.shape[2]
+        return _colsum_fused((a.data_ptr(), a.stride(1), int(transA), b.data_ptr(), b.stride(1), int(transB), M, N, K, 1.0,
+                              0, int(nbatch), a.stride(0), b.stride(0), 1, 0))
+    pa, M, K, lda, ta = _mat(a, "a")
+    pb, K2, N, ldb, tb = _mat(b, "b")
+    if K != K2:
+        raise ValueError(f"gemm_colsum_fused: inner dimensions differ ({K} vs {K2})")
+    return _colsum_fused((pa, lda, ta, pb, ldb, tb, M, N, K, float(alpha), int(act), 1, 0, 0, int(split_k),
+                          int(gate is not None)))
+
+
+def add_fanout(src: torch.Tensor, dsts) -> None:
+    import ctypes as C
+    dsts = list(dsts)
+    ps = ptr(src, "src")
+    for d in dsts:
+        if d.numel() != src.numel():
+            raise ValueError("add_fanout: sizes differ")
+    for i in range(0, len(dsts), 4):
+        part = dsts[i:i + 4]
+        arr = (C.c_void_p * len(part))(*[ptr(d, "dst") for d in part])
+        _lib.call("parrot_add_fanout", ps, arr, len(part), src.numel(), _stream())
 
 
 ROUTE_STEP, ROUTE_F32, ROUTE_BF16, ROUTE_BF16X3 = 0, 1, 2, 3
@@ -190,7 +240,7 @@
         return False
 
 
-def gemm_batched(a, b, out, transA=False, transB=False, accumulate=False):
+def gemm_batched(a, b, out, transA=False, transB=False, accumulate=False, colsum_out=None, colsum_accumulate=False):
     _chk(a, "a"); _chk(b, "b"); _chk(out, "out")
     nb = a.shape[0]
     M, K = (a.shape[2], a.shape[1]) if transA else (a.shape[1], a.shape[2])
@@ -199,6 +249,9 @@
     _lib.call("parrot_gemm", a.data_ptr(), a.stride(1), int(transA), b.data_ptr(), b.stride(1), int(transB),
               out.data_ptr(), out.stride(1), M, N, K, None, 1.0, int(bool(accumulate)), 0, nb,
               a.stride(0), b.stride(0), out.stride(0), 1, _stream())
+    if colsum_out is not None:
+        for i in range(nb):
+            colsum(b[i].t() if transB else b[i], out=colsum_out[i], accumulate=colsum_accumulate)
     return out
 
 
@@ -275,7 +328,8 @@
     return _LinearFn.apply(x, W, b, act)
 
 
-def gemm_gated(a: torch.Tensor, b: torch.Tensor, gate: torch.Tensor, out=None) -> torch.Tensor:
+def gemm_gated(a: torch.Tensor, b: torch.Tensor, gate: torch.Tensor, out=None, colsum_out=None,
+               colsum_accumulate=False) -> torch.Tensor:
     pa, M, K, lda, ta = _mat(a, "a")
     pb, K2, N, ldb, tb = _mat(b, "b")
     _chk(gate, "gate")
@@ -288,6 +342,8 @@
         raise ValueError("gemm_gated: bad output tensor")
     _lib.call("parrot_gemm_gated", pa, lda, ta, pb, ldb, tb, out.data_ptr(), out.stride(0), M, N, K,
               gate.data_ptr(), gate.stride(0), _stream())
+    if colsum_out is not None:
+        colsum(b, out=colsum_out, accumulate=colsum_accumulate)
     return out
 
 
```
